# jayleicn/ClipBERT

Measured on NVIDIA H100. Metric: clips/sec fwd+bwd MSRVTT ret (ResNet50+BERT-base), higher is better.
Workload: dtype bf16

## Files before the change

clipbert_b200/_lib.py:

```python
import ctypes
import os

import torch

_HERE = os.path.dirname(os.path.abspath(__file__))
LIB_PATH = os.path.join(_HERE, "lib", "libclipbert_sm90.so")

CB_GEMM_TN, CB_GEMM_WGRAD = 0, 1
ACT_NONE, ACT_RELU, ACT_GELU, ACT_TANH, ACT_GELU_STASH_GRAD = 0, 1, 2, 3, 4
AUX_NONE, AUX_RELU_MASK, AUX_GELU_GRAD, AUX_TANH_GRAD, AUX_MUL = 0, 1, 2, 3, 4
ROWMAP_NONE, ROWMAP_PAD, ROWMAP_UNPAD = 0, 1, 2


class GemmDesc(ctypes.Structure):
    _fields_ = [
        ("mode", ctypes.c_int32),
        ("m", ctypes.c_int32), ("n", ctypes.c_int32), ("k", ctypes.c_int32),
        ("a", ctypes.c_void_p), ("a_rows", ctypes.c_int64), ("a_ld", ctypes.c_int64),
        ("b", ctypes.c_void_p), ("b_rows", ctypes.c_int64), ("b_ld", ctypes.c_int64),
        ("ntaps", ctypes.c_int32), ("tap_w", ctypes.c_int32), ("tap_sign", ctypes.c_int32),
        ("split_k", ctypes.c_int32),
        ("scale", ctypes.c_void_p), ("shift", ctypes.c_void_p),
        ("residual", ctypes.c_void_p), ("res_ld", ctypes.c_int64),
        ("aux", ctypes.c_void_p), ("aux_ld", ctypes.c_int64), ("aux_mode", ctypes.c_int32),
        ("act", ctypes.c_int32),
        ("out", ctypes.c_void_p), ("out_ld", ctypes.c_int64), ("out_fp32", ctypes.c_int32),
        ("out2", ctypes.c_void_p), ("out2_ld", ctypes.c_int64),
        ("rowmap", ctypes.c_int32), ("map_h", ctypes.c_int32), ("map_w", ctypes.c_int32),
        ("dropout_p", ctypes.c_float), ("dropout_seed", ctypes.c_uint64),
        ("block_n", ctypes.c_int32), ("reserved", ctypes.c_int32),
        ("workspace", ctypes.c_void_p), ("workspace_bytes", ctypes.c_int64),
    ]


class NativeLibraryMissing(RuntimeError):
    pass


_lib = None


def lib():
    global _lib
    if _lib is not None:
        return _lib
    if not os.path.exists(LIB_PATH):
        raise NativeLibraryMissing(
            "%s not found: run `python -c 'import __graft_entry__ as g; g.build()'` "
            "(there is no CPU / eager fallback for the ClipBERT hot path)" % LIB_PATH)
    L = ctypes.CDLL(LIB_PATH)
    L.cb_last_error.restype = ctypes.c_char_p
    L.cb_version.restype = ctypes.c_int
    L.cb_sm_arch.restype = ctypes.c_int
    L.cb_launch_count.restype = ctypes.c_int64
    L.cb_gemm.argtypes = [ctypes.POINTER(GemmDesc), ctypes.c_void_p]
    L.cb_gemm.restype = ctypes.c_int
    L.cb_gemm_wgrad_group.argtypes = [ctypes.POINTER(GemmDesc), ctypes.c_int, ctypes.c_void_p]
    L.cb_gemm_wgrad_group.restype = ctypes.c_int
    L.cb_gemm_workspace_bytes.argtypes = [ctypes.POINTER(GemmDesc)]
    L.cb_gemm_workspace_bytes.restype = ctypes.c_int64
    L.cb_gemm_wgrad_group_workspace_bytes.argtypes = [ctypes.POINTER(GemmDesc), ctypes.c_int]
    L.cb_gemm_wgrad_group_workspace_bytes.restype = ctypes.c_int64
    L.cb_set_deterministic.argtypes = [ctypes.c_int]
    L.cb_set_deterministic.restype = ctypes.c_int
    _lib = L
    return L


def check(rc, what="cb call"):
    if rc != 0:
        raise RuntimeError("%s failed (%d): %s" % (what, rc, lib().cb_last_error().decode()))


def stream_ptr():
    return ctypes.c_void_p(torch.cuda.current_stream().cuda_stream)


def ptr(t):
    return None if t is None else t.data_ptr()
```

clipbert_b200/csrc/api.cu:

```cuda
#include <cstdlib>
#include <cstring>
#include <mutex>
#include <unordered_map>
#include <vector>

#include "common.cuh"
#include "host_util.h"

namespace cb {

static thread_local char t_err[512] = "";
std::atomic<int64_t> g_launches{0};
static int pdl_default() {
  const char* e = getenv("CB_PDL");
  return (e && e[0] == '1') ? 1 : ((e && e[0] == '2') ? 2 : 0);
}
std::atomic<int> g_pdl{pdl_default()};
std::atomic<int> g_det{0};
static std::atomic<const uint64_t*> g_drop_offset{nullptr};
const uint64_t* drop_offset_ptr() { return g_drop_offset.load(std::memory_order_relaxed); }

__global__ void drop_offset_advance_kernel(unsigned long long* counter, unsigned long long* snapshot) {
  pdl_wait();
  pdl_trigger();
  const unsigned long long v = *counter + 1ull;
  *counter = v;
  if (snapshot) *snapshot = v;
}

void set_error(const char* fmt, ...) {
  va_list ap;
  va_start(ap, fmt);
  vsnprintf(t_err, sizeof(t_err), fmt, ap);
  va_end(ap);
}

typedef CUresult (*EncodeTiledFn)(CUtensorMap*, CUtensorMapDataType, cuuint32_t, void*,
                                  const cuuint64_t*, const cuuint64_t*, const cuuint32_t*,
                                  const cuuint32_t*, CUtensorMapInterleave, CUtensorMapSwizzle,
                                  CUtensorMapL2promotion, CUtensorMapFloatOOBfill);

static EncodeTiledFn get_encode_fn() {
  static EncodeTiledFn fn = nullptr;
  static std::once_flag once;
  std::call_once(once, [] {
    void* p = nullptr;
    cudaDriverEntryPointQueryResult q;
    cudaError_t e = cudaGetDriverEntryPoint("cuTensorMapEncodeTiled", &p, cudaEnableDefault, &q);
    if (e == cudaSuccess && q == cudaDriverEntryPointSuccess) fn = reinterpret_cast<EncodeTiledFn>(p);
  });
  return fn;
}

struct TmapKey {
  uint64_t base, inner, rows, ld;
  uint32_t box_inner, box_rows;
  bool operator==(const TmapKey& o) const {
    return base == o.base && inner == o.inner && rows == o.rows && ld == o.ld &&
           box_inner == o.box_inner && box_rows == o.box_rows;
  }
};
struct TmapKeyHash {
  size_t operator()(const TmapKey& k) const {
    uint64_t h = k.base * 0x9E3779B97F4A7C15ull;
    h ^= (k.inner + 0x9E3779B97F4A7C15ull + (h << 6) + (h >> 2));
    h ^= (k.rows + 0x9E3779B97F4A7C15ull + (h << 6) + (h >> 2));
    h ^= (k.ld + 0x9E3779B97F4A7C15ull + (h << 6) + (h >> 2));
    h ^= ((static_cast<uint64_t>(k.box_inner) << 32 | k.box_rows) + (h << 6) + (h >> 2));
    return static_cast<size_t>(h);
  }
};

bool get_tmap_2d(CUtensorMap* out, const void* base, uint64_t inner, uint64_t rows, uint64_t ld,
                 uint32_t box_inner, uint32_t box_rows) {
  static std::mutex mu;
  static std::unordered_map<TmapKey, CUtensorMap, TmapKeyHash> cache;
  TmapKey key{reinterpret_cast<uint64_t>(base), inner, rows, ld, box_inner, box_rows};
  std::lock_guard<std::mutex> lock(mu);
  auto it = cache.find(key);
  if (it != cache.end()) {
    *out = it->second;
    return true;
  }

  EncodeTiledFn enc = get_encode_fn();
  if (!enc) {
    set_error("cuTensorMapEncodeTiled driver entry point not available");
    return false;
  }
  if ((reinterpret_cast<uint64_t>(base) & 15) != 0 || ((ld * 2) & 15) != 0) {
    set_error("TMA operand must be 16-byte aligned (base %p, row pitch %llu elements)", base,
              (unsigned long long)ld);
    return false;
  }
  alignas(64) CUtensorMap tm;
  CUtensorMap* m = &tm;
  cuuint64_t dims[2] = {inner, rows};
  cuuint64_t strides[1] = {ld * 2};
  cuuint32_t box[2] = {box_inner, box_rows};
  cuuint32_t estr[2] = {1, 1};
  CUresult r = enc(m, CU_TENSOR_MAP_DATA_TYPE_BFLOAT16, 2, const_cast<void*>(base), dims, strides,
                   box, estr, CU_TENSOR_MAP_INTERLEAVE_NONE, CU_TENSOR_MAP_SWIZZLE_128B,
                   CU_TENSOR_MAP_L2_PROMOTION_L2_256B, CU_TENSOR_MAP_FLOAT_OOB_FILL_NONE);
  if (r != CUDA_SUCCESS) {
    set_error("cuTensorMapEncodeTiled failed (%d) inner=%llu rows=%llu ld=%llu box=%ux%u", (int)r,
              (unsigned long long)inner, (unsigned long long)rows, (unsigned long long)ld, box_inner,
              box_rows);
    return false;
  }
  if (cache.size() > 65536) cache.clear();
  cache.emplace(key, tm);
  *out = tm;
  return true;
}

bool get_tmap_3d_mn(CUtensorMap* out, const void* base, uint64_t cols, uint64_t rows, uint64_t ld, uint32_t box_rows, uint32_t nblk) {
  static std::mutex mu;
  static std::unordered_map<TmapKey, CUtensorMap, TmapKeyHash> cache;
  TmapKey key{reinterpret_cast<uint64_t>(base), cols, rows, ld, 0x80000000u | (nblk << 16) | 64u, box_rows};
  std::lock_guard<std::mutex> lock(mu);
  auto it = cache.find(key);
  if (it != cache.end()) {
    *out = it->second;
    return true;
  }
  EncodeTiledFn enc = get_encode_fn();
  if (!enc) {
    set_error("cuTensorMapEncodeTiled driver entry point not available");
    return false;
  }
  if ((reinterpret_cast<uint64_t>(base) & 15) != 0 || ((ld * 2) & 15) != 0 || (cols & 63) != 0 || nblk == 0 || nblk > 8) {
    set_error("3-D MN-major tensor map: base %p, row pitch %llu, cols %llu (must be a multiple of 64), %u blocks", base,
              (unsigned long long)ld, (unsigned long long)cols, nblk);
    return false;
  }
  alignas(64) CUtensorMap tm;
  CUtensorMap* m = &tm;
  cuuint64_t dims[3] = {64, rows, cols / 64};
  cuuint64_t strides[2] = {ld * 2, 128};
  cuuint32_t box[3] = {64, box_rows, nblk};
  cuuint32_t estr[3] = {1, 1, 1};
  CUresult r = enc(m, CU_TENSOR_MAP_DATA_TYPE_BFLOAT16, 3, const_cast<void*>(base), dims, strides, box, estr,
                   CU_TENSOR_MAP_INTERLEAVE_NONE, CU_TENSOR_MAP_SWIZZLE_128B, CU_TENSOR_MAP_L2_PROMOTION_L2_256B,
                   CU_TENSOR_MAP_FLOAT_OOB_FILL_NONE);
  if (r != CUDA_SUCCESS) {
    set_error("cuTensorMapEncodeTiled (3-D) failed (%d) cols=%llu rows=%llu ld=%llu box=64x%ux%u", (int)r, (unsigned long long)cols,
              (unsigned long long)rows, (unsigned long long)ld, box_rows, nblk);
    return false;
  }
  if (cache.size() > 65536) cache.clear();
  cache.emplace(key, tm);
  *out = tm;
  return true;
}

}

extern "C" {
const char* cb_last_error(void) { return cb::t_err; }
int cb_version(void) { return 100; }
int cb_sm_arch(void) { return 90; }
int64_t cb_launch_count(void) { return cb::g_launches.load(std::memory_order_relaxed); }
int cb_set_pdl(int enable) { return cb::g_pdl.exchange(enable == 2 ? 2 : (enable ? 1 : 0), std::memory_order_relaxed); }
int cb_set_deterministic(int enable) { return cb::g_det.exchange(enable ? 1 : 0, std::memory_order_relaxed); }
int cb_dropout_offset_bind(const uint64_t* device_word) {
  cb::g_drop_offset.store(device_word, std::memory_order_relaxed);
  return CB_OK;
}
int cb_dropout_offset_advance(uint64_t* counter, uint64_t* snapshot, void* stream) {
  CB_REQUIRE(counter != nullptr, "cb_dropout_offset_advance: null counter");
  cb::launch_k(cb::drop_offset_advance_kernel, dim3(1), dim3(1), 0, static_cast<cudaStream_t>(stream),
               reinterpret_cast<unsigned long long*>(counter), reinterpret_cast<unsigned long long*>(snapshot));
  return cb::check_launch("cb_dropout_offset_advance");
}
}
```

clipbert_b200/csrc/common.cuh:

```cuda
#pragma once
#include <cuda.h>
#include <cuda_bf16.h>
#include <cuda_runtime.h>
#include <stdint.h>

#include "drop_cfg.h"

namespace cb {

#ifndef CB_SPIN_LIMIT
#define CB_SPIN_LIMIT (1u << 24)
#endif

__device__ __forceinline__ uint32_t smem_u32(const void* p) {
  return static_cast<uint32_t>(__cvta_generic_to_shared(p));
}

__device__ __forceinline__ void pdl_wait() { asm volatile("griddepcontrol.wait;" ::: "memory"); }
__device__ __forceinline__ void pdl_trigger() { asm volatile("griddepcontrol.launch_dependents;" ::: "memory"); }

__device__ __forceinline__ void mbar_init(uint64_t* bar, uint32_t count) {
  asm volatile("mbarrier.init.shared::cta.b64 [%0], %1;" ::"r"(smem_u32(bar)), "r"(count));
}
__device__ __forceinline__ void fence_mbar_init() {
  asm volatile("fence.mbarrier_init.release.cluster;" ::: "memory");
}
__device__ __forceinline__ void fence_proxy_async_smem() {
  asm volatile("fence.proxy.async.shared::cta;" ::: "memory");
}
__device__ __forceinline__ void mbar_expect_tx(uint64_t* bar, uint32_t bytes) {
  asm volatile("mbarrier.arrive.expect_tx.shared::cta.b64 _, [%0], %1;" ::"r"(smem_u32(bar)),
               "r"(bytes)
               : "memory");
}
__device__ __forceinline__ void mbar_arrive(uint64_t* bar) {
  asm volatile("mbarrier.arrive.shared::cta.b64 _, [%0];" ::"r"(smem_u32(bar)) : "memory");
}
__device__ __forceinline__ void mbar_arrive_if(uint64_t* bar, bool pred) {
  asm volatile("{\n\t.reg .pred p;\n\tsetp.ne.b32 p, %1, 0;\n\t@p mbarrier.arrive.shared::cta.b64 _, [%0];\n\t}" ::"r"(smem_u32(bar)),
               "r"(static_cast<uint32_t>(pred))
               : "memory");
}
__device__ __forceinline__ bool mbar_try_wait(uint64_t* bar, uint32_t parity) {
  uint32_t ok;
  asm volatile(
      "{\n\t.reg .pred p;\n\t"
      "mbarrier.try_wait.parity.shared::cta.b64 p, [%1], %2, %3;\n\t"
      "selp.u32 %0, 1, 0, p;\n\t}"
      : "=r"(ok)
      : "r"(smem_u32(bar)), "r"(parity), "r"(2000u)
      : "memory");
  return ok != 0;
}
__device__ __forceinline__ void mbar_wait(uint64_t* bar, uint32_t parity) {
  uint32_t spins = 0;
  while (!mbar_try_wait(bar, parity)) {
    if (++spins > CB_SPIN_LIMIT) __trap();
  }
}
__device__ __forceinline__ void mbar_wait_unguarded(uint64_t* bar, uint32_t parity) {
  while (!mbar_try_wait(bar, parity)) {
  }
}

__device__ __forceinline__ void tma_prefetch_desc(const CUtensorMap* map) {
  asm volatile("prefetch.tensormap [%0];" ::"l"(map) : "memory");
}
__device__ __forceinline__ void tma_load_2d(void* smem_dst, const CUtensorMap* map, uint64_t* bar,
                                            int c0, int c1) {
  asm volatile(
      "cp.async.bulk.tensor.2d.shared::cluster.global.mbarrier::complete_tx::bytes "
      "[%0], [%1, {%3, %4}], [%2];" ::"r"(smem_u32(smem_dst)),
      "l"(map), "r"(smem_u32(bar)), "r"(c0), "r"(c1)
      : "memory");
}

__device__ __forceinline__ void bulk_load_1d(uint32_t smem_dst, const void* gsrc, uint32_t bytes, uint64_t* bar) {
  asm volatile("cp.async.bulk.shared::cluster.global.mbarrier::complete_tx::bytes [%0], [%1], %2, [%3];" ::"r"(smem_dst), "l"(gsrc),
               "r"(bytes), "r"(smem_u32(bar))
               : "memory");
}

__device__ __forceinline__ void tma_load_2d_s32(uint32_t smem_dst, const CUtensorMap* map, uint64_t* bar, int c0, int c1) {
  asm volatile(
      "cp.async.bulk.tensor.2d.shared::cluster.global.mbarrier::complete_tx::bytes "
      "[%0], [%1, {%3, %4}], [%2];" ::"r"(smem_dst),
      "l"(map), "r"(smem_u32(bar)), "r"(c0), "r"(c1)
      : "memory");
}

__device__ __forceinline__ void tma_load_3d(void* smem_dst, const CUtensorMap* map, uint64_t* bar, int c0, int c1, int c2) {
  asm volatile(
      "cp.async.bulk.tensor.3d.shared::cluster.global.mbarrier::complete_tx::bytes "
      "[%0], [%1, {%3, %4, %5}], [%2];" ::"r"(smem_u32(smem_dst)),
      "l"(map), "r"(smem_u32(bar)), "r"(c0), "r"(c1), "r"(c2)
      : "memory");
}

__device__ __forceinline__ void tma_store_2d(const CUtensorMap* map, const void* smem_src, int c0, int c1) {
  asm volatile("cp.async.bulk.tensor.2d.global.shared::cta.bulk_group [%0, {%2, %3}], [%1];" ::"l"(map),
               "r"(smem_u32(smem_src)), "r"(c0), "r"(c1)
               : "memory");
}
__device__ __forceinline__ void tma_store_2d_s32(const CUtensorMap* map, uint32_t smem_src, int c0, int c1) {
  asm volatile("cp.async.bulk.tensor.2d.global.shared::cta.bulk_group [%0, {%2, %3}], [%1];" ::"l"(map), "r"(smem_src), "r"(c0), "r"(c1)
               : "memory");
}
__device__ __forceinline__ uint4 lds128(uint32_t saddr) {
  uint4 v;
  asm volatile("ld.shared.v4.u32 {%0, %1, %2, %3}, [%4];" : "=r"(v.x), "=r"(v.y), "=r"(v.z), "=r"(v.w) : "r"(saddr));
  return v;
}
__device__ __forceinline__ void sts128(uint32_t saddr, uint4 v) {
  asm volatile("st.shared.v4.u32 [%0], {%1, %2, %3, %4};" ::"r"(saddr), "r"(v.x), "r"(v.y), "r"(v.z), "r"(v.w) : "memory");
}
__device__ __forceinline__ void tma_store_commit() { asm volatile("cp.async.bulk.commit_group;" ::: "memory"); }
template <int N>
__device__ __forceinline__ void tma_store_wait_read() {
  asm volatile("cp.async.bulk.wait_group.read %0;" ::"n"(N) : "memory");
}
template <int N>
__device__ __forceinline__ void tma_store_wait_all() {
  asm volatile("cp.async.bulk.wait_group %0;" ::"n"(N) : "memory");
}
__device__ __forceinline__ void named_bar_sync(uint32_t id, uint32_t nthreads) {
  asm volatile("bar.sync %0, %1;" ::"r"(id), "r"(nthreads) : "memory");
}
__device__ __forceinline__ void named_bar_arrive(uint32_t id, uint32_t nthreads) {
  asm volatile("bar.arrive %0, %1;" ::"r"(id), "r"(nthreads) : "memory");
}
template <uint32_t NREG>
__device__ __forceinline__ void setmaxnreg_dec() {
  asm volatile("setmaxnreg.dec.sync.aligned.u32 %0;" ::"n"(NREG));
}
template <uint32_t NREG>
__device__ __forceinline__ void setmaxnreg_inc() {
  asm volatile("setmaxnreg.inc.sync.aligned.u32 %0;" ::"n"(NREG));
}

__device__ __forceinline__ void wgmma_fence() { asm volatile("wgmma.fence.sync.aligned;" ::: "memory"); }
__device__ __forceinline__ void wgmma_commit() { asm volatile("wgmma.commit_group.sync.aligned;" ::: "memory"); }
template <int N>
__device__ __forceinline__ void wgmma_wait() {
  asm volatile("wgmma.wait_group.sync.aligned %0;" ::"n"(N) : "memory");
}
template <int R>
__device__ __forceinline__ void wgmma_fence_acc(float (&d)[R]) {
#pragma unroll
  for (int i = 0; i < R; ++i) asm volatile("" : "+f"(d[i])::"memory");
}

__device__ __forceinline__ uint64_t gmma_desc(uint32_t smem_addr, uint32_t lbo, uint32_t sbo) {
  uint64_t d = 0;
  d |= static_cast<uint64_t>((smem_addr & 0x3FFFFu) >> 4);
  d |= static_cast<uint64_t>((lbo >> 4) & 0x3FFFu) << 16;
  d |= static_cast<uint64_t>((sbo >> 4) & 0x3FFFu) << 32;
  d |= 1ull << 62;
  return d;
}

template <int TA, int TB>
__device__ __forceinline__ void wgmma_bf16_n64(float (&d)[32], uint64_t adesc, uint64_t bdesc, uint32_t accumulate) {
  asm volatile(
      "{\n\t.reg .pred p;\n\t"
      "setp.ne.b32 p, %34, 0;\n\t"
      "wgmma.mma_async.sync.aligned.m64n64k16.f32.bf16.bf16 "
      "{"
      "%0, %1, %2, %3, %4, %5, %6, %7, %8, %9, %10, %11, %12, %13, %14, %15, "
      "%16, %17, %18, %19, %20, %21, %22, %23, %24, %25, %26, %27, %28, %29, %30, %31"
      "}, %32, %33, p, 1, 1, %35, %36;\n\t}"
      : "+f"(d[0]), "+f"(d[1]), "+f"(d[2]), "+f"(d[3]), "+f"(d[4]), "+f"(d[5]), "+f"(d[6]), "+f"(d[7]),
        "+f"(d[8]), "+f"(d[9]), "+f"(d[10]), "+f"(d[11]), "+f"(d[12]), "+f"(d[13]), "+f"(d[14]), "+f"(d[15]),
        "+f"(d[16]), "+f"(d[17]), "+f"(d[18]), "+f"(d[19]), "+f"(d[20]), "+f"(d[21]), "+f"(d[22]), "+f"(d[23]),
        "+f"(d[24]), "+f"(d[25]), "+f"(d[26]), "+f"(d[27]), "+f"(d[28]), "+f"(d[29]), "+f"(d[30]), "+f"(d[31])
      : "l"(adesc), "l"(bdesc), "r"(accumulate), "n"(TA), "n"(TB));
}
template <int TA, int TB>
__device__ __forceinline__ void wgmma_bf16_n128(float (&d)[64], uint64_t adesc, uint64_t bdesc, uint32_t accumulate) {
  asm volatile(
      "{\n\t.reg .pred p;\n\t"
      "setp.ne.b32 p, %66, 0;\n\t"
      "wgmma.mma_async.sync.aligned.m64n128k16.f32.bf16.bf16 "
      "{"
      "%0, %1, %2, %3, %4, %5, %6, %7, %8, %9, %10, %11, %12, %13, %14, %15, "
      "%16, %17, %18, %19, %20, %21, %22, %23, %24, %25, %26, %27, %28, %29, %30, %31, "
      "%32, %33, %34, %35, %36, %37, %38, %39, %40, %41, %42, %43, %44, %45, %46, %47, "
      "%48, %49, %50, %51, %52, %53, %54, %55, %56, %57, %58, %59, %60, %61, %62, %63"
      "}, %64, %65, p, 1, 1, %67, %68;\n\t}"
      : "+f"(d[0]), "+f"(d[1]), "+f"(d[2]), "+f"(d[3]), "+f"(d[4]), "+f"(d[5]), "+f"(d[6]), "+f"(d[7]),
        "+f"(d[8]), "+f"(d[9]), "+f"(d[10]), "+f"(d[11]), "+f"(d[12]), "+f"(d[13]), "+f"(d[14]), "+f"(d[15]),
        "+f"(d[16]), "+f"(d[17]), "+f"(d[18]), "+f"(d[19]), "+f"(d[20]), "+f"(d[21]), "+f"(d[22]), "+f"(d[23]),
        "+f"(d[24]), "+f"(d[25]), "+f"(d[26]), "+f"(d[27]), "+f"(d[28]), "+f"(d[29]), "+f"(d[30]), "+f"(d[31]),
        "+f"(d[32]), "+f"(d[33]), "+f"(d[34]), "+f"(d[35]), "+f"(d[36]), "+f"(d[37]), "+f"(d[38]), "+f"(d[39]),
        "+f"(d[40]), "+f"(d[41]), "+f"(d[42]), "+f"(d[43]), "+f"(d[44]), "+f"(d[45]), "+f"(d[46]), "+f"(d[47]),
        "+f"(d[48]), "+f"(d[49]), "+f"(d[50]), "+f"(d[51]), "+f"(d[52]), "+f"(d[53]), "+f"(d[54]), "+f"(d[55]),
        "+f"(d[56]), "+f"(d[57]), "+f"(d[58]), "+f"(d[59]), "+f"(d[60]), "+f"(d[61]), "+f"(d[62]), "+f"(d[63])
      : "l"(adesc), "l"(bdesc), "r"(accumulate), "n"(TA), "n"(TB));
}
template <int TA, int TB>
__device__ __forceinline__ void wgmma_bf16_n256(float (&d)[128], uint64_t adesc, uint64_t bdesc, uint32_t accumulate) {
  asm volatile(
      "{\n\t.reg .pred p;\n\t"
      "setp.ne.b32 p, %130, 0;\n\t"
      "wgmma.mma_async.sync.aligned.m64n256k16.f32.bf16.bf16 "
      "{"
      "%0, %1, %2, %3, %4, %5, %6, %7, %8, %9, %10, %11, %12, %13, %14, %15, "
      "%16, %17, %18, %19, %20, %21, %22, %23, %24, %25, %26, %27, %28, %29, %30, %31, "
      "%32, %33, %34, %35, %36, %37, %38, %39, %40, %41, %42, %43, %44, %45, %46, %47, "
      "%48, %49, %50, %51, %52, %53, %54, %55, %56, %57, %58, %59, %60, %61, %62, %63, "
      "%64, %65, %66, %67, %68, %69, %70, %71, %72, %73, %74, %75, %76, %77, %78, %79, "
      "%80, %81, %82, %83, %84, %85, %86, %87, %88, %89, %90, %91, %92, %93, %94, %95, "
      "%96, %97, %98, %99, %100, %101, %102, %103, %104, %105, %106, %107, %108, %109, %110, %111, "
      "%112, %113, %114, %115, %116, %117, %118, %119, %120, %121, %122, %123, %124, %125, %126, %127"
      "}, %128, %129, p, 1, 1, %131, %132;\n\t}"
      : "+f"(d[0]), "+f"(d[1]), "+f"(d[2]), "+f"(d[3]), "+f"(d[4]), "+f"(d[5]), "+f"(d[6]), "+f"(d[7]),
        "+f"(d[8]), "+f"(d[9]), "+f"(d[10]), "+f"(d[11]), "+f"(d[12]), "+f"(d[13]), "+f"(d[14]), "+f"(d[15]),
        "+f"(d[16]), "+f"(d[17]), "+f"(d[18]), "+f"(d[19]), "+f"(d[20]), "+f"(d[21]), "+f"(d[22]), "+f"(d[23]),
        "+f"(d[24]), "+f"(d[25]), "+f"(d[26]), "+f"(d[27]), "+f"(d[28]), "+f"(d[29]), "+f"(d[30]), "+f"(d[31]),
        "+f"(d[32]), "+f"(d[33]), "+f"(d[34]), "+f"(d[35]), "+f"(d[36]), "+f"(d[37]), "+f"(d[38]), "+f"(d[39]),
        "+f"(d[40]), "+f"(d[41]), "+f"(d[42]), "+f"(d[43]), "+f"(d[44]), "+f"(d[45]), "+f"(d[46]), "+f"(d[47]),
        "+f"(d[48]), "+f"(d[49]), "+f"(d[50]), "+f"(d[51]), "+f"(d[52]), "+f"(d[53]), "+f"(d[54]), "+f"(d[55]),
        "+f"(d[56]), "+f"(d[57]), "+f"(d[58]), "+f"(d[59]), "+f"(d[60]), "+f"(d[61]), "+f"(d[62]), "+f"(d[63]),
        "+f"(d[64]), "+f"(d[65]), "+f"(d[66]), "+f"(d[67]), "+f"(d[68]), "+f"(d[69]), "+f"(d[70]), "+f"(d[71]),
        "+f"(d[72]), "+f"(d[73]), "+f"(d[74]), "+f"(d[75]), "+f"(d[76]), "+f"(d[77]), "+f"(d[78]), "+f"(d[79]),
        "+f"(d[80]), "+f"(d[81]), "+f"(d[82]), "+f"(d[83]), "+f"(d[84]), "+f"(d[85]), "+f"(d[86]), "+f"(d[87]),
        "+f"(d[88]), "+f"(d[89]), "+f"(d[90]), "+f"(d[91]), "+f"(d[92]), "+f"(d[93]), "+f"(d[94]), "+f"(d[95]),
        "+f"(d[96]), "+f"(d[97]), "+f"(d[98]), "+f"(d[99]), "+f"(d[100]), "+f"(d[101]), "+f"(d[102]), "+f"(d[103]),
        "+f"(d[104]), "+f"(d[105]), "+f"(d[106]), "+f"(d[107]), "+f"(d[108]), "+f"(d[109]), "+f"(d[110]), "+f"(d[111]),
        "+f"(d[112]), "+f"(d[113]), "+f"(d[114]), "+f"(d[115]), "+f"(d[116]), "+f"(d[117]), "+f"(d[118]), "+f"(d[119]),
        "+f"(d[120]), "+f"(d[121]), "+f"(d[122]), "+f"(d[123]), "+f"(d[124]), "+f"(d[125]), "+f"(d[126]), "+f"(d[127])
      : "l"(adesc), "l"(bdesc), "r"(accumulate), "n"(TA), "n"(TB));
}

template <int N, int TA, int TB>
__device__ __forceinline__ void wgmma_bf16(float (&d)[N / 2], uint64_t adesc, uint64_t bdesc, uint32_t accumulate) {
  if constexpr (N == 64) wgmma_bf16_n64<TA, TB>(d, adesc, bdesc, accumulate);
  else if constexpr (N == 128) wgmma_bf16_n128<TA, TB>(d, adesc, bdesc, accumulate);
  else wgmma_bf16_n256<TA, TB>(d, adesc, bdesc, accumulate);
}

__device__ __forceinline__ float warp_sum(float v) {
#pragma unroll
  for (int o = 16; o > 0; o >>= 1) v += __shfl_xor_sync(0xffffffffu, v, o);
  return v;
}
__device__ __forceinline__ float warp_max(float v) {
#pragma unroll
  for (int o = 16; o > 0; o >>= 1) v = fmaxf(v, __shfl_xor_sync(0xffffffffu, v, o));
  return v;
}

__device__ __forceinline__ void red_add_f32x4(float* addr, float4 v) {
  asm volatile("red.global.add.v4.f32 [%0], {%1, %2, %3, %4};" ::"l"(addr), "f"(v.x), "f"(v.y), "f"(v.z),
               "f"(v.w)
               : "memory");
}

__device__ __forceinline__ void red_add_f32x2(float* addr, float x, float y) {
  asm volatile("red.global.add.v2.f32 [%0], {%1, %2};" ::"l"(addr), "f"(x), "f"(y) : "memory");
}

__device__ __forceinline__ float fast_rcp(float x) {
  float r;
  asm("rcp.approx.ftz.f32 %0, %1;" : "=f"(r) : "f"(x));
  return r;
}

__device__ __forceinline__ float fast_erf(float x) {
  const float ax = fabsf(x);
  const float t = fast_rcp(fmaf(0.3275911f, ax, 1.0f));
  float p = fmaf(1.061405429f, t, -1.453152027f);
  p = fmaf(p, t, 1.421413741f);
  p = fmaf(p, t, -0.284496736f);
  p = fmaf(p, t, 0.254829592f);
  const float r = 1.0f - p * t * __expf(-ax * ax);
  return copysignf(r, x);
}
__device__ __forceinline__ float gelu_erf(float x) {
  return 0.5f * x * (1.0f + fast_erf(x * 0.70710678118654752f));
}
__device__ __forceinline__ void gelu_erf_and_grad(float x, float& y, float& g) {
  const float az = fabsf(x) * 0.70710678118654752f;
  const float t = fast_rcp(fmaf(0.3275911f, az, 1.0f));
  float p = fmaf(1.061405429f, t, -1.453152027f);
  p = fmaf(p, t, 1.421413741f);
  p = fmaf(p, t, -0.284496736f);
  p = fmaf(p, t, 0.254829592f);
  const float e = __expf(-az * az);
  const float cdf = 0.5f * (1.0f + copysignf(1.0f - p * t * e, x));
  y = x * cdf;
  g = fmaf(x * 0.3989422804014327f, e, cdf);
}
__device__ __forceinline__ float gelu_erf_grad(float x) {
  const float cdf = 0.5f * (1.0f + fast_erf(x * 0.70710678118654752f));
  const float pdf = 0.3989422804014327f * __expf(-0.5f * x * x);
  return cdf + x * pdf;
}

__device__ __forceinline__ uint64_t drop_seed(uint64_t seed, const uint64_t* offset) {
  return offset ? seed + __ldg(reinterpret_cast<const unsigned long long*>(offset)) * 0xD1342543DE82EF95ull : seed;
}
__device__ __forceinline__ DropCfg drop_resolve(DropCfg dc) {
  if (dc.thresh) dc.seed = drop_seed(dc.seed, dc.offset);
  dc.offset = nullptr;
  return dc;
}
__device__ __forceinline__ uint64_t drop_hash(uint64_t seed, uint64_t group) {
  uint64_t z = group * 0x9E3779B97F4A7C15ull + seed;
  z = (z ^ (z >> 30)) * 0xBF58476D1CE4E5B9ull;
  z = (z ^ (z >> 27)) * 0x94D049BB133111EBull;
  return z ^ (z >> 31);
}
__device__ __forceinline__ float drop_lane(uint64_t h, int lane, uint32_t thresh, float inv_keep) {
  return (static_cast<uint32_t>(h >> (16 * lane)) & 0xFFFFu) >= thresh ? inv_keep : 0.0f;
}
__device__ __forceinline__ float dropout_mult(uint64_t seed, uint64_t idx, uint32_t thresh, float inv_keep) {
  return drop_lane(drop_hash(seed, idx >> 2), static_cast<int>(idx & 3), thresh, inv_keep);
}
__device__ __forceinline__ void dropout_mult4(uint64_t seed, uint64_t idx, uint32_t thresh, float inv_keep, float (&m)[4]) {
  const uint64_t h = drop_hash(seed, idx >> 2);
#pragma unroll
  for (int j = 0; j < 4; ++j) m[j] = drop_lane(h, j, thresh, inv_keep);
}
__device__ __forceinline__ void dropout_mult2(uint64_t seed, uint64_t idx, uint32_t thresh, float inv_keep, float& m0, float& m1) {
  const uint64_t h0 = drop_hash(seed, idx >> 2);
  const int l0 = static_cast<int>(idx & 3);
  m0 = drop_lane(h0, l0, thresh, inv_keep);
  m1 = l0 == 3 ? drop_lane(drop_hash(seed, (idx >> 2) + 1), 0, thresh, inv_keep) : drop_lane(h0, l0 + 1, thresh, inv_keep);
}

__device__ __forceinline__ uint32_t pack_bf16x2(float lo, float hi) {
  __nv_bfloat162 h = __floats2bfloat162_rn(lo, hi);
  return *reinterpret_cast<uint32_t*>(&h);
}
__device__ __forceinline__ float2 unpack_bf16x2(uint32_t u) {
  __nv_bfloat162 h = *reinterpret_cast<__nv_bfloat162*>(&u);
  return __bfloat1622float2(h);
}

}
```

clipbert_b200/csrc/gemm.cu:

```cuda
#include <algorithm>

#include "common.cuh"
#include "host_util.h"

namespace cb {

constexpr int BM = 128;
constexpr int BK = 64;
constexpr int CONSUMER_WARPS = 8;
constexpr int GEMM_THREADS = (CONSUMER_WARPS + 1) * 32;
constexpr int PP_THREADS = 3 * 128;
constexpr int PP_PRODUCER_REGS = 40;
constexpr int PP_CONSUMER_REGS = 232;
constexpr int PP_BAR_TURN = 1;
constexpr int MAX_STAGES = 8;
constexpr int SMEM_LIMIT = 232448;
constexpr int STG_PITCH = 36;
constexpr int STG_WARP_FLOATS = 16 * STG_PITCH;
constexpr int EPI_BYTES = CONSUMER_WARPS * STG_WARP_FLOATS * 4;
constexpr int IN_BOX_BYTES = BM * 64 * 2;

struct GemmEpi {
  const float* scale;
  const float* shift;
  const __nv_bfloat16* residual;
  const __nv_bfloat16* aux;
  int aux_mode;
  int act;
  void* out;
  int64_t out_ld;
  int out_fp32;
  __nv_bfloat16* out2;
  int64_t out2_ld;
  int rowmap, H, W;
  uint32_t drop_thresh;
  float drop_inv_keep;
  uint64_t seed;
  const uint64_t* seed_off;
  int mn3d;
  long long* dbg;
};

__device__ __forceinline__ void dbg_stamp(const GemmEpi& epi, int slot) {
  if (epi.dbg) {
    epi.dbg[blockIdx.x * 32 + slot] = clock64();
    if (slot == 0 || slot == 11) {
      unsigned long long ns;
      asm volatile("mov.u64 %0, %%globaltimer;" : "=l"(ns));
      epi.dbg[blockIdx.x * 32 + (slot == 0 ? 12 : 13)] = static_cast<long long>(ns);
    }
  }
}

template <int BN>
struct GemmCfg {
  static constexpr int A_BYTES = BM * BK * 2;
  static constexpr int B_BYTES = BN * BK * 2;
  static constexpr int STAGE_BYTES = A_BYTES + B_BYTES;
  static constexpr int BAR_BYTES = 256;
};

enum { EK_GENERIC = 0, EK_SHIFT_ACT = 1, EK_RELU_MASK = 2, EK_DROP_RES = 3, EK_GELU_STASH = 4, EK_AUX_MUL = 5 };

__device__ __forceinline__ float relu_nan(float v) { return !(v <= 0.0f) ? v : 0.0f; }
__device__ __forceinline__ bool bf16_relu_pos(uint32_t x, bool lo) {
  const uint32_t b = lo ? (x & 0xffffu) : (x >> 16);
  return b - 0x0080u <= 0x7f80u - 0x0080u;
}

template <int NC>
__device__ __forceinline__ void add_shift(float (&f)[NC], const float (&shv)[NC]) {
#pragma unroll
  for (int j = 0; j < NC; ++j) f[j] += shv[j];
}
template <int NC>
__device__ __forceinline__ void add_residual(float (&f)[NC], const uint32_t (&res16)[NC / 2]) {
#pragma unroll
  for (int j = 0; j < NC / 2; ++j) {
    const float2 r2 = unpack_bf16x2(res16[j]);
    f[2 * j] += r2.x;
    f[2 * j + 1] += r2.y;
  }
}
template <int NC>
__device__ __forceinline__ void epilogue_shift_act(float (&f)[NC], const float (&shv)[NC], bool has_shift, const uint32_t (&res16)[NC / 2], bool has_res,
                                                   bool relu) {
  if (has_shift) add_shift<NC>(f, shv);
  if (has_res) add_residual<NC>(f, res16);
  if (relu) {
#pragma unroll
    for (int j = 0; j < NC; ++j) f[j] = relu_nan(f[j]);
  }
}
template <int NC>
__device__ __forceinline__ void epilogue_relu_mask(float (&f)[NC], const uint32_t (&res16)[NC / 2], bool has_res, const uint32_t (&aux16)[NC / 2]) {
  if (has_res) add_residual<NC>(f, res16);
#pragma unroll
  for (int j = 0; j < NC / 2; ++j) {
    f[2 * j] = bf16_relu_pos(aux16[j], true) ? f[2 * j] : 0.0f;
    f[2 * j + 1] = bf16_relu_pos(aux16[j], false) ? f[2 * j + 1] : 0.0f;
  }
}
template <int NC>
__device__ __forceinline__ void epilogue_drop_res(float (&f)[NC], const float (&shv)[NC], bool has_shift, const uint32_t (&res16)[NC / 2], bool has_res,
                                                  uint64_t dseed, uint64_t didx, uint32_t thresh, float inv_keep) {
  if (has_shift) add_shift<NC>(f, shv);
#pragma unroll
  for (int j = 0; j < NC; j += 4) {
    float m[4];
    dropout_mult4(dseed, didx + j, thresh, inv_keep, m);
    f[j] *= m[0]; f[j + 1] *= m[1]; f[j + 2] *= m[2]; f[j + 3] *= m[3];
  }
  if (has_res) add_residual<NC>(f, res16);
}
template <int NC>
__device__ __forceinline__ void epilogue_gelu_stash(float (&f)[NC], const float (&shv)[NC], bool has_shift, uint32_t (&o2_16)[NC / 2]) {
  if (has_shift) add_shift<NC>(f, shv);
#pragma unroll
  for (int j = 0; j < NC / 2; ++j) {
    float y0, g0, y1, g1;
    gelu_erf_and_grad(f[2 * j], y0, g0);
    gelu_erf_and_grad(f[2 * j + 1], y1, g1);
    f[2 * j] = y0;
    f[2 * j + 1] = y1;
    o2_16[j] = pack_bf16x2(g0, g1);
  }
}
template <int NC>
__device__ __forceinline__ void epilogue_aux_mul(float (&f)[NC], const uint32_t (&res16)[NC / 2], bool has_res, const uint32_t (&aux16)[NC / 2]) {
  if (has_res) add_residual<NC>(f, res16);
#pragma unroll
  for (int j = 0; j < NC / 2; ++j) {
    const float2 a2 = unpack_bf16x2(aux16[j]);
    f[2 * j] *= a2.x;
    f[2 * j + 1] *= a2.y;
  }
}
template <int NC, bool GUARD>
__device__ __forceinline__ void epilogue_math(float (&f)[NC], const GemmEpi& epi, const float (&shv)[NC], bool has_shift, uint64_t dseed, int nb, int N,
                                              int64_t orow, const uint32_t (&res16)[NC / 2], bool has_res, const uint32_t (&aux16)[NC / 2], bool has_aux,
                                              uint32_t (&o2_16)[NC / 2], bool has_out2) {
  if (GUARD && nb >= N) return;
  if (epi.scale) {
#pragma unroll
    for (int j = 0; j < NC; j += 4) {
      if (!GUARD || nb + j + 4 <= N) {
        const float4 s4 = __ldg(reinterpret_cast<const float4*>(epi.scale + nb + j));
        f[j] *= s4.x; f[j + 1] *= s4.y; f[j + 2] *= s4.z; f[j + 3] *= s4.w;
      }
    }
  }
  if (has_shift) add_shift<NC>(f, shv);
  if (epi.drop_thresh) {
    const uint64_t base = static_cast<uint64_t>(orow) * static_cast<uint64_t>(N) + nb;
#pragma unroll
    for (int j = 0; j < NC; j += 4) {
      float m[4];
      dropout_mult4(dseed, base + j, epi.drop_thresh, epi.drop_inv_keep, m);
      f[j] *= m[0]; f[j + 1] *= m[1]; f[j + 2] *= m[2]; f[j + 3] *= m[3];
    }
  }
  if (has_res) add_residual<NC>(f, res16);
  if (epi.act == CB_ACT_GELU_STASH_GRAD) {
#pragma unroll
    for (int j = 0; j < NC / 2; ++j) {
      float y0, g0, y1, g1;
      gelu_erf_and_grad(f[2 * j], y0, g0);
      gelu_erf_and_grad(f[2 * j + 1], y1, g1);
      f[2 * j] = y0;
      f[2 * j + 1] = y1;
      if (has_out2) o2_16[j] = pack_bf16x2(g0, g1);
    }
  } else if (has_out2) {
#pragma unroll
    for (int j = 0; j < NC / 2; ++j) o2_16[j] = pack_bf16x2(f[2 * j], f[2 * j + 1]);
  }
  switch (epi.act) {
    case CB_ACT_RELU:
#pragma unroll
      for (int j = 0; j < NC; ++j) f[j] = relu_nan(f[j]);
      break;
    case CB_ACT_GELU:
#pragma unroll
      for (int j = 0; j < NC; ++j) f[j] = gelu_erf(f[j]);
      break;
    case CB_ACT_TANH:
#pragma unroll
      for (int j = 0; j < NC; ++j) f[j] = tanhf(f[j]);
      break;
    default: break;
  }
  if (has_aux) {
    switch (epi.aux_mode) {
      case CB_AUX_RELU_MASK:
#pragma unroll
        for (int j = 0; j < NC / 2; ++j) {
          f[2 * j] = bf16_relu_pos(aux16[j], true) ? f[2 * j] : 0.0f;
          f[2 * j + 1] = bf16_relu_pos(aux16[j], false) ? f[2 * j + 1] : 0.0f;
        }
        break;
      case CB_AUX_GELU_GRAD:
#pragma unroll
        for (int j = 0; j < NC / 2; ++j) {
          const float2 a2 = unpack_bf16x2(aux16[j]);
          f[2 * j] *= gelu_erf_grad(a2.x);
          f[2 * j + 1] *= gelu_erf_grad(a2.y);
        }
        break;
      case CB_AUX_TANH_GRAD:
#pragma unroll
        for (int j = 0; j < NC / 2; ++j) {
          const float2 a2 = unpack_bf16x2(aux16[j]);
          f[2 * j] *= (1.0f - a2.x * a2.x);
          f[2 * j + 1] *= (1.0f - a2.y * a2.y);
        }
        break;
      case CB_AUX_MUL:
#pragma unroll
        for (int j = 0; j < NC / 2; ++j) {
          const float2 a2 = unpack_bf16x2(aux16[j]);
          f[2 * j] *= a2.x;
          f[2 * j + 1] *= a2.y;
        }
        break;
      default: break;
    }
  }
}

struct TileInfo {
  int m0, n0;
};

template <int BN>
__device__ __forceinline__ TileInfo decode_tile(int tile, int tiles_m, int tiles_n) {
  TileInfo t;
  t.m0 = (tile / tiles_n) % tiles_m * BM;
  t.n0 = tile % tiles_n * BN;
  return t;
}

template <int BN, int TA, int TB>
__device__ __forceinline__ void mma_tile(float (&acc)[BN / 2], uint32_t smem0, int stage_bytes, int KCH, int STAGES, int n_iters, int wg,
                                         int lane, int& s, uint32_t& ph, uint64_t* full_bar, uint64_t* empty_bar) {
  using Cfg = GemmCfg<BN>;
  int prev = -1;
  for (int i = 0; i < n_iters; i += KCH) {
    const int nch = min(KCH, n_iters - i);
    mbar_wait(&full_bar[s], ph);
    __syncwarp();
    wgmma_fence();
    wgmma_fence_acc(acc);
    for (int ch = 0; ch < nch; ++ch) {
      const uint32_t a_addr = smem0 + s * stage_bytes + ch * Cfg::STAGE_BYTES + wg * (64 * 128);
      const uint32_t b_addr = smem0 + s * stage_bytes + ch * Cfg::STAGE_BYTES + Cfg::A_BYTES;
#pragma unroll
      for (int k = 0; k < BK / 16; ++k) {
        const uint64_t ad = TA ? gmma_desc(a_addr + k * 2048, BK * 128, 1024) : gmma_desc(a_addr + k * 32, 16, 1024);
        const uint64_t bd = TB ? gmma_desc(b_addr + k * 2048, BK * 128, 1024) : gmma_desc(b_addr + k * 32, 16, 1024);
        wgmma_bf16<BN, TA, TB>(acc, ad, bd, (i > 0 || ch > 0 || k > 0) ? 1u : 0u);
      }
    }
    wgmma_commit();
    wgmma_wait<1>();
    wgmma_fence_acc(acc);
    if (prev >= 0) {
      __syncwarp();
      if (lane == 0) mbar_arrive(&empty_bar[prev]);
    }
    prev = s;
    if (++s == STAGES) { s = 0; ph ^= 1; }
  }
  wgmma_wait<0>();
  wgmma_fence_acc(acc);
  if (prev >= 0) {
    __syncwarp();
    if (lane == 0) mbar_arrive(&empty_bar[prev]);
  }
}

template <int BN, int TB>
__device__ __forceinline__ void mma_tile_pp(float (&acc)[2][BN / 2], uint32_t smem0, int stage_bytes, int KCH, int STAGES, int n_iters,
                                            int lane, int& s, uint32_t& ph, uint64_t* full_bar, uint64_t* empty_bar, int pass_bar,
                                            bool in_stage) {
  using Cfg = GemmCfg<BN>;
  int prev = -1;
  for (int i = 0; i < n_iters; i += KCH) {
    const int nch = min(KCH, n_iters - i);
    mbar_wait_unguarded(&full_bar[s], ph);
    __syncwarp();
    wgmma_fence();
    wgmma_fence_acc(acc[0]);
    wgmma_fence_acc(acc[1]);
    for (int ch = 0; ch < nch; ++ch) {
      const uint32_t a_addr = smem0 + s * stage_bytes + ch * Cfg::STAGE_BYTES;
      const uint32_t b_addr = a_addr + Cfg::A_BYTES;
#pragma unroll
      for (int k = 0; k < BK / 16; ++k) {
        const uint64_t bd = TB ? gmma_desc(b_addr + k * 2048, BK * 128, 1024) : gmma_desc(b_addr + k * 32, 16, 1024);
        const uint32_t accum = (i > 0 || ch > 0 || k > 0) ? 1u : 0u;
#pragma unroll
        for (int h = 0; h < 2; ++h) wgmma_bf16<BN, 0, TB>(acc[h], gmma_desc(a_addr + h * (64 * 128) + k * 32, 16, 1024), bd, accum);
      }
    }
    wgmma_commit();
    wgmma_wait<1>();
    wgmma_fence_acc(acc[0]);
    wgmma_fence_acc(acc[1]);
    if (prev >= 0) {
      __syncwarp();
      mbar_arrive_if(&empty_bar[prev], lane == 0);
    }
    prev = s;
    if (++s == STAGES) { s = 0; ph ^= 1; }
    if (pass_bar && i + KCH >= n_iters) {
      if (in_stage) mbar_wait_unguarded(&full_bar[s], ph);
      named_bar_arrive(pass_bar, 2 * 128);
    }
  }
  wgmma_wait<0>();
  wgmma_fence_acc(acc[0]);
  wgmma_fence_acc(acc[1]);
  if (prev >= 0) {
    __syncwarp();
    mbar_arrive_if(&empty_bar[prev], lane == 0);
  }
}

template <int BN, bool STORE = false>
__device__ __forceinline__ void wgrad_epilogue(const float (&acc)[BN / 2], float* obase, int64_t out_ld, const float* scale, int M, int N, int r0,
                                               int n0, int lane) {
  const int r1 = r0 + 8;
  const float rs0 = (r0 < M && scale) ? scale[r0] : 1.0f;
  const float rs1 = (r1 < M && scale) ? scale[r1] : 1.0f;
#pragma unroll
  for (int j = 0; j < BN / 8; ++j) {
    const int n = n0 + j * 8 + 2 * (lane & 3);
    if (n < N) {
      if constexpr (STORE) {
        if (r0 < M) *reinterpret_cast<float2*>(obase + static_cast<int64_t>(r0) * out_ld + n) = make_float2(acc[4 * j] * rs0, acc[4 * j + 1] * rs0);
        if (r1 < M) *reinterpret_cast<float2*>(obase + static_cast<int64_t>(r1) * out_ld + n) = make_float2(acc[4 * j + 2] * rs1, acc[4 * j + 3] * rs1);
      } else {
        if (r0 < M) red_add_f32x2(obase + static_cast<int64_t>(r0) * out_ld + n, acc[4 * j] * rs0, acc[4 * j + 1] * rs0);
        if (r1 < M) red_add_f32x2(obase + static_cast<int64_t>(r1) * out_ld + n, acc[4 * j + 2] * rs1, acc[4 * j + 3] * rs1);
      }
    }
  }
}

__device__ __forceinline__ uint32_t swz128(uint32_t box, int r, int q) { return box + r * 128 + ((q ^ (r & 7)) << 4); }

template <int BN, int MODE>
__global__ void __launch_bounds__(PP_THREADS, 1)
    gemm_pingpong_kernel(const __grid_constant__ CUtensorMap tmA, const __grid_constant__ CUtensorMap tmB, const __grid_constant__ CUtensorMap tmR,
                         const __grid_constant__ CUtensorMap tmX, int M, int N, int K, int ntaps, int tap_w, int tap_sign, int tiles_m,
                         int tiles_n, int total_tiles, int STAGES, int KCH, int N_IN, GemmEpi epi) {
  static_assert(MODE != 1 && BN <= 128, "TN / NN tiles of 128 x 64 or 128 x 128");
  using Cfg = GemmCfg<BN>;
  extern __shared__ uint8_t smem_raw[];
  uint8_t* smem = reinterpret_cast<uint8_t*>((reinterpret_cast<uintptr_t>(smem_raw) + 1023) & ~static_cast<uintptr_t>(1023));
  const int stage_bytes = KCH * Cfg::STAGE_BYTES;
  const bool has_res = epi.residual != nullptr, has_aux = epi.aux != nullptr;
  constexpr int IN_TILE_BYTES = (BN / 64) * IN_BOX_BYTES;
  const int in_bytes = (has_res + has_aux) * IN_TILE_BYTES;
  uint8_t* in_base = smem + STAGES * stage_bytes;
  uint8_t* stg_base = in_base + N_IN * in_bytes;
  uint64_t* full_bar = reinterpret_cast<uint64_t*>(stg_base + EPI_BYTES);
  uint64_t* empty_bar = full_bar + MAX_STAGES;
  uint64_t* in_full = empty_bar + MAX_STAGES;
  uint64_t* in_empty = in_full + 2;

  const int warp = __shfl_sync(0xffffffffu, static_cast<int>(threadIdx.x >> 5), 0);
  const int lane = threadIdx.x & 31;
  const int unit = blockIdx.x;
  const int n_units = gridDim.x;
  if (threadIdx.x == 0) dbg_stamp(epi, 0);
  pdl_trigger();
  if (threadIdx.x == 0) {
    tma_prefetch_desc(&tmA);
    tma_prefetch_desc(&tmB);
    if (has_res) tma_prefetch_desc(&tmR);
    if (has_aux) tma_prefetch_desc(&tmX);
    for (int s = 0; s < STAGES; ++s) {
      mbar_init(&full_bar[s], 1);
      mbar_init(&empty_bar[s], 4);
    }
    for (int b = 0; b < 2; ++b) {
      mbar_init(&in_full[b], 1);
      mbar_init(&in_empty[b], 4);
    }
    fence_mbar_init();
  }
  __syncthreads();
  const int kc_per_tap = (K + BK - 1) / BK;
  const int n_iters = ntaps * kc_per_tap;
  const bool in_stage = in_bytes && !N_IN;
  const int tile_stages = (n_iters + KCH - 1) / KCH + (in_stage ? 1 : 0);
  pdl_wait();
  if (threadIdx.x == 0) dbg_stamp(epi, 1);

  if (warp < 4) {
    setmaxnreg_dec<PP_PRODUCER_REGS>();
    if (warp == 0 && lane == 0) {
      constexpr int B_BOXES = (MODE == 0) ? 1 : BN / 64;
      int s = 0;
      uint32_t ph = 0;
      auto load_inputs = [&](int tile) {
        const TileInfo t = decode_tile<BN>(tile, tiles_m, tiles_n);
        uint64_t* bar;
        uint8_t* dst;
        if (N_IN) {
          const int local = (tile - unit) / n_units;
          const int b = N_IN == 2 ? (local & 1) : 0;
          const int uses = N_IN == 2 ? (local >> 1) : local;
          mbar_wait(&in_empty[b], (static_cast<uint32_t>(uses) & 1u) ^ 1u);
          bar = &in_full[local & 1];
          dst = in_base + b * in_bytes;
        } else {
          mbar_wait(&empty_bar[s], ph ^ 1);
          bar = &full_bar[s];
          dst = smem + s * stage_bytes;
          if (++s == STAGES) { s = 0; ph ^= 1; }
        }
        mbar_expect_tx(bar, in_bytes);
        if (has_res) {
#pragma unroll
          for (int j = 0; j < BN / 64; ++j) tma_load_2d(dst + j * IN_BOX_BYTES, &tmR, bar, t.n0 + j * 64, t.m0);
          dst += IN_TILE_BYTES;
        }
        if (has_aux) {
#pragma unroll
          for (int j = 0; j < BN / 64; ++j) tma_load_2d(dst + j * IN_BOX_BYTES, &tmX, bar, t.n0 + j * 64, t.m0);
        }
      };
      int pend = -1;
      for (int tile = unit; tile < total_tiles; tile += n_units) {
        const TileInfo t = decode_tile<BN>(tile, tiles_m, tiles_n);
        const bool inputs_first = tile < unit + N_IN * n_units;
        if (in_bytes && N_IN && inputs_first) load_inputs(tile);
        for (int i = 0; i < n_iters; i += KCH) {
          const int nch = min(KCH, n_iters - i);
          mbar_wait(&empty_bar[s], ph ^ 1);
          mbar_expect_tx(&full_bar[s], nch * Cfg::STAGE_BYTES);
          int tp = 0, kc = i;
          if (ntaps > 1) { tp = i / kc_per_tap; kc = i - tp * kc_per_tap; }
          for (int ch = 0; ch < nch; ++ch) {
            uint8_t* sa = smem + s * stage_bytes + ch * Cfg::STAGE_BYTES;
            uint8_t* sb = sa + Cfg::A_BYTES;
            int shift = 0;
            if (ntaps == 9) shift = tap_sign * ((tp / 3 - 1) * tap_w + (tp % 3 - 1));
            else if (ntaps > 1) shift = tap_sign * tp * tap_w;
            tma_load_2d(sa, &tmA, &full_bar[s], kc * BK, t.m0 + shift);
            if (MODE == 0) {
              tma_load_2d(sb, &tmB, &full_bar[s], tp * K + kc * BK, t.n0);
            } else if (epi.mn3d) {
              tma_load_3d(sb, &tmB, &full_bar[s], 0, kc * BK, (tp * N + t.n0) >> 6);
            } else {
#pragma unroll
              for (int j = 0; j < B_BOXES; ++j) tma_load_2d(sb + j * (BK * 128), &tmB, &full_bar[s], tp * N + t.n0 + j * 64, kc * BK);
            }
            if (++kc == kc_per_tap) { kc = 0; ++tp; }
          }
          if (++s == STAGES) { s = 0; ph ^= 1; }
          if (i == 0 && tile == unit) dbg_stamp(epi, 2);
        }
        if (in_stage) load_inputs(tile);
        if (pend >= 0) load_inputs(pend);
        pend = (in_bytes && N_IN && !inputs_first) ? tile : -1;
      }
      if (pend >= 0) load_inputs(pend);
      dbg_stamp(epi, 3);
    }
    return;
  }

  setmaxnreg_inc<PP_CONSUMER_REGS>();
  const int wg = (warp >> 2) - 1;
  const int wq = warp & 3;
  const uint32_t smem0 = smem_u32(smem);
  const uint64_t dseed = epi.drop_thresh ? drop_seed(epi.seed, epi.seed_off) : 0ull;
  float acc[2][BN / 2];
  int s = 0;
  uint32_t ph = 0;
  auto ring_skip = [&](int n) {
    s += n;
    while (s >= STAGES) { s -= STAGES; ph ^= 1; }
  };
  if (wg == 1) ring_skip(tile_stages);

  const int er = lane & 15, eh = lane >> 4;
  float* stg = reinterpret_cast<float*>(stg_base) + (warp - 4) * STG_WARP_FLOATS;
  const bool has_out2 = epi.out2 != nullptr;
  const bool has_shift = epi.shift != nullptr;
  const bool full = (N & 15) == 0 && epi.scale == nullptr;
  const bool drop = epi.drop_thresh != 0;
  int kind = EK_GENERIC;
  if (full) {
    if (!drop && !has_out2 && !has_aux && (epi.act == CB_ACT_NONE || epi.act == CB_ACT_RELU)) kind = EK_SHIFT_ACT;
    else if (!drop && !has_out2 && !has_shift && has_aux && epi.aux_mode == CB_AUX_RELU_MASK && epi.act == CB_ACT_NONE) kind = EK_RELU_MASK;
    else if (drop && !has_out2 && !has_aux && epi.act == CB_ACT_NONE) kind = EK_DROP_RES;
    else if (!drop && has_out2 && !has_aux && !has_res && epi.act == CB_ACT_GELU_STASH_GRAD) kind = EK_GELU_STASH;
    else if (!drop && !has_out2 && !has_shift && has_aux && epi.aux_mode == CB_AUX_MUL && epi.act == CB_ACT_NONE) kind = EK_AUX_MUL;
  }
  const bool kind_relu = epi.act == CB_ACT_RELU;
  const bool guard = (N & 15) != 0;

  for (int local = wg, tile = unit + wg * n_units; tile < total_tiles; local += 2, tile += 2 * n_units) {
    const TileInfo t = decode_tile<BN>(tile, tiles_m, tiles_n);
    if (local > 0) named_bar_sync(PP_BAR_TURN + wg, 2 * 128);
    const int pass = tile + n_units < total_tiles ? PP_BAR_TURN + (wg ^ 1) : 0;
    mma_tile_pp<BN, MODE != 0>(acc, smem0, stage_bytes, KCH, STAGES, n_iters, lane, s, ph, full_bar, empty_bar, pass, in_stage);

    const uint32_t in_buf = N_IN ? smem_u32(in_base) + (N_IN == 2 ? wg : 0) * in_bytes : smem0 + s * stage_bytes;
    if (in_bytes) {
      if (N_IN) mbar_wait_unguarded(&in_full[wg], static_cast<uint32_t>(local >> 1) & 1u);
      else mbar_wait_unguarded(&full_bar[s], ph);
    }
    int orow_half[2];
#pragma unroll
    for (int h = 0; h < 2; ++h) {
      const int m = t.m0 + h * 64 + wq * 16 + er;
      bool row_ok = m < M;
      int64_t orow = m;
      if (epi.rowmap == CB_ROWMAP_PAD) {
        const int hw = epi.H * epi.W;
        const int img = m / hw;
        const int r = m - img * hw;
        const int y = r / epi.W, x = r - y * epi.W;
        orow = (static_cast<int64_t>(img) * (epi.H + 2) + y + 1) * (epi.W + 2) + x + 1;
      } else if (epi.rowmap == CB_ROWMAP_UNPAD) {
        const int wp = epi.W + 2, hp = epi.H + 2;
        const int img = m / (hp * wp);
        const int r = m - img * (hp * wp);
        const int y = r / wp, x = r - y * wp;
        row_ok = row_ok && y >= 1 && y <= epi.H && x >= 1 && x <= epi.W;
        orow = (static_cast<int64_t>(img) * epi.H + (y - 1)) * epi.W + (x - 1);
      }
      orow_half[h] = row_ok ? static_cast<int>(orow) : -1;
    }
#pragma unroll
    for (int sc = 0; sc < BN / 32; ++sc) {
#pragma unroll 1
      for (int h = 0; h < 2; ++h) {
        const int wrow = h * 64 + wq * 16;
        __syncwarp();
#pragma unroll
        for (int jj = 0; jj < 4; ++jj) {
          const int j = sc * 4 + jj;
          float* p = stg + (lane >> 2) * STG_PITCH + jj * 8 + 2 * (lane & 3);
          const bool h1 = h != 0;
          *reinterpret_cast<float2*>(p) = make_float2(h1 ? acc[1][4 * j] : acc[0][4 * j], h1 ? acc[1][4 * j + 1] : acc[0][4 * j + 1]);
          *reinterpret_cast<float2*>(p + 8 * STG_PITCH) =
              make_float2(h1 ? acc[1][4 * j + 2] : acc[0][4 * j + 2], h1 ? acc[1][4 * j + 3] : acc[0][4 * j + 3]);
        }
        __syncwarp();
        const int nb = t.n0 + sc * 32 + eh * 16;
        const int64_t orow = h ? orow_half[1] : orow_half[0];
        if (orow < 0 || nb >= N) continue;
        constexpr int NC = 16;
        float f[NC];
        const uint32_t srow = smem_u32(stg + er * STG_PITCH + eh * 16);
#pragma unroll
        for (int j = 0; j < NC / 4; ++j) {
          const uint4 u = lds128(srow + j * 16);
          f[4 * j] = __uint_as_float(u.x); f[4 * j + 1] = __uint_as_float(u.y);
          f[4 * j + 2] = __uint_as_float(u.z); f[4 * j + 3] = __uint_as_float(u.w);
        }
        uint32_t res16[NC / 2], aux16[NC / 2];
        const int tc = sc * 32 + eh * 16;
        const int q = (tc & 63) >> 3;
        if (has_res) {
#pragma unroll
          for (int j = 0; j < 2; ++j) {
            const uint4 u = lds128(swz128(in_buf + (tc >> 6) * IN_BOX_BYTES, wrow + er, q + j));
            res16[4 * j] = u.x; res16[4 * j + 1] = u.y; res16[4 * j + 2] = u.z; res16[4 * j + 3] = u.w;
          }
        }
        if (has_aux) {
#pragma unroll
          for (int j = 0; j < 2; ++j) {
            const uint4 u = lds128(swz128(in_buf + (has_res ? IN_TILE_BYTES : 0) + (tc >> 6) * IN_BOX_BYTES, wrow + er, q + j));
            aux16[4 * j] = u.x; aux16[4 * j + 1] = u.y; aux16[4 * j + 2] = u.z; aux16[4 * j + 3] = u.w;
          }
        }
        float shv[NC];
        if (has_shift) {
#pragma unroll
          for (int j = 0; j < NC; j += 4) {
            float4 s4 = make_float4(0.f, 0.f, 0.f, 0.f);
            if (nb + j + 4 <= N) s4 = __ldg(reinterpret_cast<const float4*>(epi.shift + nb + j));
            shv[j] = s4.x; shv[j + 1] = s4.y; shv[j + 2] = s4.z; shv[j + 3] = s4.w;
          }
        }
        uint32_t o2_16[NC / 2];
        switch (kind) {
          case EK_SHIFT_ACT: epilogue_shift_act<NC>(f, shv, has_shift, res16, has_res, kind_relu); break;
          case EK_RELU_MASK: epilogue_relu_mask<NC>(f, res16, has_res, aux16); break;
          case EK_DROP_RES:
            epilogue_drop_res<NC>(f, shv, has_shift, res16, has_res, dseed, static_cast<uint64_t>(orow) * static_cast<uint64_t>(N) + nb,
                                  epi.drop_thresh, epi.drop_inv_keep);
            break;
          case EK_GELU_STASH: epilogue_gelu_stash<NC>(f, shv, has_shift, o2_16); break;
          case EK_AUX_MUL: epilogue_aux_mul<NC>(f, res16, has_res, aux16); break;
          default:
            if (guard) epilogue_math<NC, true>(f, epi, shv, has_shift, dseed, nb, N, orow, res16, has_res, aux16, has_aux, o2_16, has_out2);
            else epilogue_math<NC, false>(f, epi, shv, has_shift, dseed, nb, N, orow, res16, has_res, aux16, has_aux, o2_16, has_out2);
        }
        if (epi.out_fp32) {
          float* o = reinterpret_cast<float*>(epi.out) + orow * epi.out_ld + nb;
#pragma unroll
          for (int j = 0; j < NC; j += 4)
            if (nb + j + 4 <= N) *reinterpret_cast<float4*>(o + j) = make_float4(f[j], f[j + 1], f[j + 2], f[j + 3]);
        } else {
          __nv_bfloat16* o = reinterpret_cast<__nv_bfloat16*>(epi.out) + orow * epi.out_ld + nb;
#pragma unroll
          for (int j = 0; j < 2; ++j)
            if (nb + 8 * j + 8 <= N)
              *reinterpret_cast<uint4*>(o + 8 * j) = make_uint4(pack_bf16x2(f[8 * j], f[8 * j + 1]), pack_bf16x2(f[8 * j + 2], f[8 * j + 3]),
                                                                pack_bf16x2(f[8 * j + 4], f[8 * j + 5]), pack_bf16x2(f[8 * j + 6], f[8 * j + 7]));
        }
        if (has_out2) {
          __nv_bfloat16* o = epi.out2 + orow * epi.out2_ld + nb;
#pragma unroll
          for (int j = 0; j < 2; ++j)
            if (nb + 8 * j + 8 <= N) *reinterpret_cast<uint4*>(o + 8 * j) = make_uint4(o2_16[4 * j], o2_16[4 * j + 1], o2_16[4 * j + 2], o2_16[4 * j + 3]);
        }
      }
    }
    if (in_bytes) {
      __syncwarp();
      if (lane == 0) mbar_arrive(N_IN ? &in_empty[N_IN == 2 ? wg : 0] : &empty_bar[s]);
      if (!N_IN && ++s == STAGES) { s = 0; ph ^= 1; }
    }
    ring_skip(tile_stages);
  }
  if (threadIdx.x == 4 * 32) dbg_stamp(epi, 11);
}

static int g_sm_limit = 0;
static int sm_count_device() {
  static int n = 0;
  if (n == 0) {
    int dev = 0;
    cudaGetDevice(&dev);
    cudaDeviceGetAttribute(&n, cudaDevAttrMultiProcessorCount, dev);
    if (n <= 0) n = 132;
  }
  return n;
}
static int sm_count() {
  const int n = sm_count_device();
  return (g_sm_limit > 0 && g_sm_limit < n) ? g_sm_limit : n;
}
static int plan_sm_count() { return g_det.load(std::memory_order_relaxed) ? sm_count_device() : sm_count(); }

static long long* g_gemm_timeline = nullptr;
static int g_mn3d = 1;


struct SmemPlan {
  int epi_bytes, kch, stages, chunk_bytes, n_in;
};
static SmemPlan plan_ring(int bn, bool staging, int kiters, int force_kch, int in_bytes, int n_in) {
  SmemPlan p;
  const int limit = SMEM_LIMIT;
  p.chunk_bytes = BM * BK * 2 + bn * BK * 2;
  p.epi_bytes = staging ? EPI_BYTES : 0;
  p.n_in = n_in;
  const int chunks_fit = (limit - 1024 - GemmCfg<64>::BAR_BYTES - p.epi_bytes - n_in * in_bytes) / p.chunk_bytes;
  const int min_stages = kiters > chunks_fit ? 3 : 2;
  p.kch = 1;
  if (force_kch > 0) p.kch = force_kch;
  else if (kiters >= 4 && chunks_fit >= 4 * min_stages) p.kch = 4;
  else if (kiters >= 2 && chunks_fit >= 2 * min_stages) p.kch = 2;
  if (p.kch > kiters) p.kch = kiters;
  if (p.kch > 1 && chunks_fit / p.kch < 2) p.kch = 1;
  p.stages = chunks_fit / p.kch;
  if (p.stages > MAX_STAGES) p.stages = MAX_STAGES;
  const int stage_iters = ceil_div(kiters, p.kch);
  const int cap = staging ? 2 * stage_iters + 1 : (stage_iters + 1 > 2 ? stage_iters + 1 : 2);
  if (p.stages > cap) p.stages = cap;
  return p;
}
static SmemPlan plan_smem(int bn, bool staging, int kiters, int force_kch = 0, int in_bytes = 0) {
  const SmemPlan none = plan_ring(bn, staging, kiters, force_kch, 0, 0);
  if (in_bytes == 0) return none;
  const SmemPlan two = plan_ring(bn, staging, kiters, force_kch, in_bytes, 2);
  if (two.stages >= 2 && two.stages * two.kch >= kiters) return two;
  if (kiters > 4 && none.stages >= 2 && none.kch * none.chunk_bytes >= in_bytes) return none;
  return plan_ring(bn, staging, kiters, force_kch, in_bytes, 1);
}
static int epi_in_bytes(const cb_gemm_desc& d, int bn) {
  return d.mode == CB_GEMM_WGRAD ? 0 : ((d.residual != nullptr) + (d.aux != nullptr)) * (bn / 64) * IN_BOX_BYTES;
}

static int real_splits(int kc, int want) {
  const int sp = want < 1 ? 1 : (want > kc ? kc : want);
  return ceil_div(kc, ceil_div(kc, sp));
}

struct SplitReduceJob {
  float* out;
  const float* ws;
  int64_t out_ld;
  int M, W, S;
};
struct SplitReduce {
  int njobs;
  SplitReduceJob j[8];
};
__global__ void __launch_bounds__(256) wgrad_split_reduce_kernel(const __grid_constant__ SplitReduce r) {
  pdl_wait();
  pdl_trigger();
  const SplitReduceJob& J = r.j[blockIdx.y];
  const int w4 = J.W / 4;
  const int64_t total = static_cast<int64_t>(J.M) * w4, plane = static_cast<int64_t>(J.M) * J.W;
  for (int64_t i = static_cast<int64_t>(blockIdx.x) * 256 + threadIdx.x; i < total; i += static_cast<int64_t>(gridDim.x) * 256) {
    const int64_t m = i / w4;
    const int c = static_cast<int>(i - m * w4) * 4;
    float4* o = reinterpret_cast<float4*>(J.out + m * J.out_ld + c);
    float4 v = *o;
    const float* p = J.ws + m * J.W + c;
    for (int s = 0; s < J.S; ++s) {
      const float4 a = *reinterpret_cast<const float4*>(p + s * plane);
      v.x += a.x; v.y += a.y; v.z += a.z; v.w += a.w;
    }
    *o = v;
  }
}
static int launch_split_reduce(const SplitReduce& r, cudaStream_t stream, const char* what) {
  int64_t most = 0;
  for (int i = 0; i < r.njobs; ++i) most = std::max(most, static_cast<int64_t>(r.j[i].M) * (r.j[i].W / 4));
  const int gx = static_cast<int>(std::min<int64_t>(1024, (most + 255) / 256));
  launch_k(wgrad_split_reduce_kernel, dim3(gx, r.njobs), 256, 0, stream, r);
  return check_launch(what);
}

template <int BN, int MODE>
static int launch_gemm(const cb_gemm_desc& d, const GemmEpi& epi_in, cudaStream_t stream) {
  GemmEpi epi = epi_in;
  using Cfg = GemmCfg<BN>;
  static bool attr_set = false;
  auto kern = gemm_pingpong_kernel<BN, MODE>;
  if (!attr_set) {
    cudaError_t e = cudaFuncSetAttribute(kern, cudaFuncAttributeMaxDynamicSharedMemorySize, SMEM_LIMIT);
    if (e != cudaSuccess) {
      set_error("cudaFuncSetAttribute(smem=%d): %s", SMEM_LIMIT, cudaGetErrorString(e));
      return CB_ERR_CUDA;
    }
    attr_set = true;
  }
  alignas(64) CUtensorMap ta, tb, tr, tx;
  bool mn3d = false;
  const int tiles_m = ceil_div(d.m, BM), tiles_n = ceil_div(d.n, BN);
  const int total = tiles_m * tiles_n;
  const int kiters = ceil_div(d.k, BK) * d.ntaps;
  bool ok = get_tmap_2d(&ta, d.a, d.k, d.a_rows, d.a_ld, BK, BM);
  if (MODE == 0) {
    ok = ok && get_tmap_2d(&tb, d.b, static_cast<uint64_t>(d.k) * d.ntaps, d.b_rows, d.b_ld, BK, BN);
  } else {
    mn3d = g_mn3d && d.n % 64 == 0 &&
           get_tmap_3d_mn(&tb, d.b, static_cast<uint64_t>(d.n) * d.ntaps, d.b_rows, d.b_ld, BK, BN / 64);
    if (!mn3d) ok = ok && get_tmap_2d(&tb, d.b, static_cast<uint64_t>(d.n) * d.ntaps, d.b_rows, d.b_ld, 64, BK);
  }
  tr = ta;
  tx = ta;
  if (d.residual) ok = ok && get_tmap_2d(&tr, d.residual, d.n, d.m, d.res_ld, 64, BM);
  if (d.aux) ok = ok && get_tmap_2d(&tx, d.aux, d.n, d.m, d.aux_ld, 64, BM);
  if (!ok) return CB_ERR_CUDA;
  epi.mn3d = mn3d ? 1 : 0;
  const int units = sm_count();
  const int grid = total < units ? total : units;
  const int in_bytes = epi_in_bytes(d, BN);
  const SmemPlan sp = plan_smem(BN, true, kiters, (d.reserved >> 8) & 15, in_bytes);
  const int kch = sp.kch, stages = sp.stages;
  if (stages < 2) {
    set_error("cb_gemm: not enough shared memory for a 2-stage pipeline (BN=%d, epilogue %d B + inputs %d B)", BN, sp.epi_bytes,
              in_bytes);
    return CB_ERR_INVALID;
  }
  const int smem_bytes = stages * kch * Cfg::STAGE_BYTES + sp.n_in * in_bytes + sp.epi_bytes + Cfg::BAR_BYTES + 1024;
  launch_gemm_k(kern, grid, PP_THREADS, smem_bytes, stream, ta, tb, tr, tx, d.m, d.n, d.k, d.ntaps, d.tap_w, d.tap_sign, tiles_m,
                tiles_n, total, stages, kch, sp.n_in, epi);
  return check_launch("cb_gemm");
}

struct LaunchCfg {
  int bn, splits;
};

static LaunchCfg choose_config(const cb_gemm_desc& d, int units) {
  const int kc = ceil_div(d.k, BK);
  const bool wgrad = d.mode == CB_GEMM_WGRAD;
  const int block_n = (!wgrad && d.block_n == 256) ? 128 : d.block_n;
  static const int cand[3] = {64, 128, 256};
  LaunchCfg best = {64, 1};
  double best_cost = 1e30;
  for (int c = 0; c < 3; ++c) {
    const int bn = cand[c];
    if (block_n && bn != block_n) continue;
    if (!wgrad && bn == 256) continue;
    if (bn > 64 && d.n <= bn / 2) continue;
    const int64_t base = static_cast<int64_t>(ceil_div(d.m, BM)) * ceil_div(d.n, bn) * (wgrad ? d.ntaps : 1);
    const int max_split = wgrad ? (d.split_k > 0 ? d.split_k : (kc < 32 ? kc : 32)) : 1;
    for (int sp = (wgrad && d.split_k > 0) ? d.split_k : 1; sp <= max_split; ++sp) {
      const int ips = ceil_div(wgrad ? kc : kc * d.ntaps, sp);
      const int real_sp = wgrad ? ceil_div(kc, ips) : 1;
      const int64_t tiles = base * real_sp;
      const double rounds = static_cast<double>((tiles + units - 1) / units);
      const SmemPlan pl = plan_smem(bn, !wgrad, ips, (d.reserved >> 8) & 15, epi_in_bytes(d, bn));
      if (pl.stages < 2) continue;
      const double shallow = (pl.stages * pl.kch < 3 && ips > 2) ? 3.0 : 1.0;
      const double stage_cost = 450.0 + pl.kch * pl.chunk_bytes / 60.0;
      const double main_loop = ceil_div(ips, pl.kch) * stage_cost * shallow;
      double cost;
      if (wgrad) {
        cost = rounds * (main_loop + bn * 24.0) + 2500.0;
      } else {
        const double epi = bn * 30.0;
        const double per_tile = main_loop > 0.5 * (main_loop + epi) ? main_loop : 0.5 * (main_loop + epi);
        cost = rounds * per_tile + 0.5 * epi + 2500.0;
      }
      if (cost < best_cost) {
        best_cost = cost;
        best = {bn, real_sp};
      }
    }
  }
  return best;
}

constexpr int WG_MAX_PROBLEMS = 8;
struct WgradProblem {
  CUtensorMap tmA, tmB;
  float* out;
  const float* scale;
  int64_t out_ld;
  int M, N, K;
  int ntaps, tap_w, tap_sign;
  int iters_per_split, tiles_m, tiles_n;
  int tile_begin;
  int mn3d;
};
struct WgradGroup {
  int nprob, total_tiles;
  WgradProblem p[WG_MAX_PROBLEMS];
};
struct WgradWorkspace {
  float* p[WG_MAX_PROBLEMS];
};
struct WgTile {
  int pi, m0, n0, tap, it_begin, n_iters;
};
__device__ __forceinline__ WgTile wg_decode(const WgradGroup& g, int tile) {
  WgTile t;
  int pi = 0;
  while (pi + 1 < g.nprob && tile >= g.p[pi + 1].tile_begin) ++pi;
  const WgradProblem& P = g.p[pi];
  int r = tile - P.tile_begin;
  const int nt = r % P.tiles_n;
  r /= P.tiles_n;
  const int mt = r % P.tiles_m;
  r /= P.tiles_m;
  t.pi = pi;
  t.m0 = mt * BM;
  t.tap = r % P.ntaps;
  const int split = r / P.ntaps;
  const int kc = (P.K + BK - 1) / BK;
  t.it_begin = split * P.iters_per_split;
  t.n_iters = min(kc, t.it_begin + P.iters_per_split) - t.it_begin;
  t.n0 = nt;
  return t;
}

template <int BN, bool DET = false>
__global__ void __launch_bounds__(GEMM_THREADS, 1)
    wgrad_group_kernel(const __grid_constant__ WgradGroup g, int STAGES, int KCH, const __grid_constant__ WgradWorkspace ws) {
  using Cfg = GemmCfg<BN>;
  extern __shared__ uint8_t smem_raw[];
  uint8_t* smem = reinterpret_cast<uint8_t*>((reinterpret_cast<uintptr_t>(smem_raw) + 1023) & ~static_cast<uintptr_t>(1023));
  const int stage_bytes = KCH * Cfg::STAGE_BYTES;
  uint64_t* full_bar = reinterpret_cast<uint64_t*>(smem + STAGES * stage_bytes);
  uint64_t* empty_bar = full_bar + MAX_STAGES;
  const int warp = __shfl_sync(0xffffffffu, static_cast<int>(threadIdx.x >> 5), 0);
  const int lane = threadIdx.x & 31;
  const int unit = blockIdx.x, n_units = gridDim.x;
  pdl_trigger();
  if (threadIdx.x == 0) {
    for (int i = 0; i < g.nprob; ++i) {
      tma_prefetch_desc(&g.p[i].tmA);
      tma_prefetch_desc(&g.p[i].tmB);
    }
    for (int s = 0; s < STAGES; ++s) {
      mbar_init(&full_bar[s], 1);
      mbar_init(&empty_bar[s], CONSUMER_WARPS);
    }
    fence_mbar_init();
  }
  __syncthreads();
  pdl_wait();

  if (warp >= CONSUMER_WARPS) {
    if (warp == CONSUMER_WARPS && lane == 0) {
      int s = 0;
      uint32_t ph = 0;
      for (int tile = unit; tile < g.total_tiles; tile += n_units) {
        const WgTile t = wg_decode(g, tile);
        const WgradProblem& P = g.p[t.pi];
        const int n0 = t.n0 * BN;
        int shift = 0;
        if (P.ntaps == 9) shift = P.tap_sign * ((t.tap / 3 - 1) * P.tap_w + (t.tap % 3 - 1));
        for (int i = 0; i < t.n_iters; i += KCH) {
          const int nch = min(KCH, t.n_iters - i);
          mbar_wait(&empty_bar[s], ph ^ 1);
          mbar_expect_tx(&full_bar[s], nch * Cfg::STAGE_BYTES);
          int kit = t.it_begin + i;
          for (int ch = 0; ch < nch; ++ch, ++kit) {
            uint8_t* sa = smem + s * stage_bytes + ch * Cfg::STAGE_BYTES;
            uint8_t* sb = sa + Cfg::A_BYTES;
            const int p = kit * BK;
            if (P.mn3d) {
              tma_load_3d(sa, &P.tmA, &full_bar[s], 0, p, t.m0 >> 6);
              tma_load_3d(sb, &P.tmB, &full_bar[s], 0, p + shift, n0 >> 6);
            } else {
#pragma unroll
              for (int j = 0; j < BM / 64; ++j) tma_load_2d(sa + j * (BK * 128), &P.tmA, &full_bar[s], t.m0 + j * 64, p);
#pragma unroll
              for (int j = 0; j < BN / 64; ++j) tma_load_2d(sb + j * (BK * 128), &P.tmB, &full_bar[s], n0 + j * 64, p + shift);
            }
          }
          if (++s == STAGES) { s = 0; ph ^= 1; }
        }
      }
    }
    return;
  }

  const int wg = warp >> 2;
  const int wrow = wg * 64 + (warp & 3) * 16;
  const uint32_t smem0 = smem_u32(smem);
  float acc[BN / 2];
  int s = 0;
  uint32_t ph = 0;
  for (int tile = unit; tile < g.total_tiles; tile += n_units) {
    const WgTile t = wg_decode(g, tile);
    const WgradProblem& P = g.p[t.pi];
    mma_tile<BN, 1, 1>(acc, smem0, stage_bytes, KCH, STAGES, t.n_iters, wg, lane, s, ph, full_bar, empty_bar);
    if (DET && ws.p[t.pi] != nullptr)
      wgrad_epilogue<BN, true>(acc, ws.p[t.pi] + static_cast<int64_t>(t.it_begin / P.iters_per_split) * P.M * P.ntaps * P.N +
                                        static_cast<int64_t>(t.tap) * P.N,
                               static_cast<int64_t>(P.ntaps) * P.N, P.scale, P.M, P.N, t.m0 + wrow + (lane >> 2), t.n0 * BN, lane);
    else
      wgrad_epilogue<BN>(acc, P.out + static_cast<int64_t>(t.tap) * P.N, P.out_ld, P.scale, P.M, P.N, t.m0 + wrow + (lane >> 2), t.n0 * BN, lane);
  }
}

template <int BN, bool DET>
static int launch_wgrad_group(const cb_gemm_desc* descs, int n, int splits, float* ws, cudaStream_t stream, const char* what) {
  using Cfg = GemmCfg<BN>;
  static bool attr_set = false;
  auto kern = wgrad_group_kernel<BN, DET>;
  if (!attr_set) {
    cudaError_t e = cudaFuncSetAttribute(kern, cudaFuncAttributeMaxDynamicSharedMemorySize, SMEM_LIMIT);
    if (e != cudaSuccess) {
      set_error("cudaFuncSetAttribute(smem=%d): %s", SMEM_LIMIT, cudaGetErrorString(e));
      return CB_ERR_CUDA;
    }
    attr_set = true;
  }
  alignas(64) WgradGroup g;
  g.nprob = n;
  SplitReduce red;
  red.njobs = 0;
  WgradWorkspace wsp;
  int total = 0, max_iters = 0;
  for (int i = 0; i < n; ++i) {
    const cb_gemm_desc& d = descs[i];
    WgradProblem& P = g.p[i];
    const bool mn3d = g_mn3d && d.m % 64 == 0 && d.n % 64 == 0 && get_tmap_3d_mn(&P.tmA, d.a, d.m, d.a_rows, d.a_ld, BK, BM / 64) &&
                      get_tmap_3d_mn(&P.tmB, d.b, d.n, d.b_rows, d.b_ld, BK, BN / 64);
    if (!mn3d && !(get_tmap_2d(&P.tmA, d.a, d.m, d.a_rows, d.a_ld, 64, BK) && get_tmap_2d(&P.tmB, d.b, d.n, d.b_rows, d.b_ld, 64, BK)))
      return CB_ERR_CUDA;
    P.mn3d = mn3d ? 1 : 0;
    P.out = static_cast<float*>(d.out);
    P.scale = d.scale;
    P.out_ld = d.out_ld;
    P.M = d.m; P.N = d.n; P.K = d.k;
    P.ntaps = d.ntaps; P.tap_w = d.tap_w; P.tap_sign = d.tap_sign;
    const int kc = ceil_div(d.k, BK);
    const int sp = real_splits(kc, splits);
    P.iters_per_split = ceil_div(kc, sp);
    wsp.p[i] = nullptr;
    if (DET && sp > 1) {
      wsp.p[i] = ws;
      red.j[red.njobs++] = {static_cast<float*>(d.out), ws, d.out_ld, d.m, d.ntaps * d.n, sp};
      ws += static_cast<int64_t>(sp) * d.m * d.ntaps * d.n;
    }
    P.tiles_m = ceil_div(d.m, BM);
    P.tiles_n = ceil_div(d.n, BN);
    P.tile_begin = total;
    total += P.tiles_m * P.tiles_n * d.ntaps * sp;
    if (P.iters_per_split > max_iters) max_iters = P.iters_per_split;
  }
  g.total_tiles = total;
  const SmemPlan sp = plan_smem(BN, false, max_iters, (descs[0].reserved >> 8) & 15);
  if (sp.stages < 2) {
    set_error("%s: not enough shared memory for a 2-stage pipeline (BN=%d)", what, BN);
    return CB_ERR_INVALID;
  }
  const int smem_bytes = sp.stages * sp.kch * Cfg::STAGE_BYTES + Cfg::BAR_BYTES + 1024;
  const int units = sm_count();
  launch_gemm_k(kern, total < units ? total : units, GEMM_THREADS, smem_bytes, stream, g, sp.stages, sp.kch, wsp);
  const int rc = check_launch(what);
  if (rc != CB_OK || red.njobs == 0) return rc;
  return launch_split_reduce(red, stream, what);
}

struct GroupPlan {
  bool groupable;
  int bn, split;
};
static GroupPlan group_plan(const cb_gemm_desc* descs, int n, int sms) {
  GroupPlan gp = {n >= 2 && n <= WG_MAX_PROBLEMS, 64, 1};
  for (int i = 0; i < n; ++i)
    if (descs[i].k * 2 < descs[0].k || descs[0].k * 2 < descs[i].k) gp.groupable = false;
  if (!gp.groupable) return gp;
  int min_n = descs[0].n;
  for (int i = 1; i < n; ++i) min_n = descs[i].n < min_n ? descs[i].n : min_n;
  gp.bn = descs[0].block_n ? descs[0].block_n : (min_n >= 192 ? 256 : (min_n >= 96 ? 128 : 64));
  int64_t base = 0;
  int kc_min = 1 << 30, kc_max = 0;
  for (int i = 0; i < n; ++i) {
    base += static_cast<int64_t>(ceil_div(descs[i].m, BM)) * ceil_div(descs[i].n, gp.bn) * descs[i].ntaps;
    const int kc = ceil_div(descs[i].k, BK);
    kc_min = kc < kc_min ? kc : kc_min;
    kc_max = kc > kc_max ? kc : kc_max;
  }
  double best_cost = 1e30;
  for (int sp = 1; sp <= 8 && sp <= kc_min; ++sp) {
    const double waves = static_cast<double>((base * sp + sms - 1) / sms);
    const double cost = waves * (ceil_div(kc_max, sp) + 8.0);
    if (cost < best_cost) { best_cost = cost; gp.split = sp; }
  }
  if (descs[0].split_k > 0) gp.split = descs[0].split_k;
  return gp;
}

static int64_t wgrad_ws_bytes(const cb_gemm_desc& d, int splits) {
  return splits > 1 ? static_cast<int64_t>(splits) * d.m * d.ntaps * d.n * 4 : 0;
}
static int64_t group_ws_bytes(const cb_gemm_desc* descs, int n) {
  const GroupPlan gp = group_plan(descs, n, sm_count_device());
  int64_t bytes = 0;
  for (int i = 0; i < n; ++i) {
    const int64_t b = gp.groupable ? wgrad_ws_bytes(descs[i], real_splits(ceil_div(descs[i].k, BK), gp.split))
                                   : wgrad_ws_bytes(descs[i], choose_config(descs[i], sm_count_device()).splits);
    bytes = gp.groupable ? bytes + b : std::max(bytes, b);
  }
  return bytes;
}

static int check_wgrad_desc(const cb_gemm_desc& d, const char* who) {
  CB_REQUIRE(d.mode == CB_GEMM_WGRAD && d.out_fp32 == 1, "%s: not an fp32 WGRAD descriptor", who);
  CB_REQUIRE(d.a && d.b && d.out && d.m > 0 && d.n > 0 && d.k > 0, "%s: null operand / empty shape", who);
  CB_REQUIRE(d.m % 8 == 0 && d.n % 8 == 0, "%s: m, n must be multiples of 8 (got %d, %d)", who, d.m, d.n);
  CB_REQUIRE(d.out_ld % 4 == 0, "%s: out_ld must be a multiple of 4", who);
  CB_REQUIRE((reinterpret_cast<uintptr_t>(d.out) & 15) == 0, "%s: out must be 16-byte aligned", who);
  CB_REQUIRE((reinterpret_cast<uintptr_t>(d.a) & 15) == 0 && (reinterpret_cast<uintptr_t>(d.b) & 15) == 0,
             "%s: a and b must be 16-byte aligned (TMA)", who);
  CB_REQUIRE(d.ntaps == 1 || d.ntaps == 9, "%s: ntaps must be 1 or 9 (got %d)", who, d.ntaps);
  return CB_OK;
}

static int launch_wgrad(const cb_gemm_desc* descs, int n, int bn, int splits, cudaStream_t stream, const char* what) {
  int64_t need = 0;
  if (g_det.load(std::memory_order_relaxed))
    for (int i = 0; i < n; ++i) need += wgrad_ws_bytes(descs[i], real_splits(ceil_div(descs[i].k, BK), splits));
  const cb_gemm_desc& d0 = descs[0];
  CB_REQUIRE(need == 0 || (d0.workspace != nullptr && d0.workspace_bytes >= need && (reinterpret_cast<uintptr_t>(d0.workspace) & 15) == 0),
             "%s: deterministic mode needs a 16-byte aligned workspace of %lld bytes in descs[0] (%s_workspace_bytes), got %lld", what,
             static_cast<long long>(need), what, static_cast<long long>(d0.workspace ? d0.workspace_bytes : 0));
  float* ws = static_cast<float*>(d0.workspace);
  switch (bn) {
    case 64: return need ? launch_wgrad_group<64, true>(descs, n, splits, ws, stream, what)
                         : launch_wgrad_group<64, false>(descs, n, splits, ws, stream, what);
    case 128: return need ? launch_wgrad_group<128, true>(descs, n, splits, ws, stream, what)
                          : launch_wgrad_group<128, false>(descs, n, splits, ws, stream, what);
    case 256: return need ? launch_wgrad_group<256, true>(descs, n, splits, ws, stream, what)
                          : launch_wgrad_group<256, false>(descs, n, splits, ws, stream, what);
    default: set_error("%s: block_n must be 0, 64, 128 or 256 (got %d)", what, bn); return CB_ERR_INVALID;
  }
}

}

extern "C" void cb_debug_gemm_timeline(void* device_buf) { cb::g_gemm_timeline = static_cast<long long*>(device_buf); }
extern "C" void cb_debug_gemm_mn3d(int on) { cb::g_mn3d = on ? 1 : 0; }
extern "C" void cb_debug_gemm_occ2(int, double) {}
extern "C" void cb_debug_gemm_sm_limit(int n) { cb::g_sm_limit = n > 0 ? n : 0; }

extern "C" int cb_gemm(const cb_gemm_desc* dp, void* stream_v) {
  using namespace cb;
  CB_REQUIRE(dp != nullptr, "cb_gemm: null descriptor");
  const cb_gemm_desc& d = *dp;
  cudaStream_t stream = static_cast<cudaStream_t>(stream_v);
  CB_REQUIRE(d.a && d.b && d.out, "cb_gemm: null operand pointer");
  CB_REQUIRE(d.m > 0 && d.n > 0 && d.k > 0, "cb_gemm: empty problem m=%d n=%d k=%d", d.m, d.n, d.k);
  CB_REQUIRE(d.ntaps == 1 || d.ntaps == 9 || (d.ntaps == 4 && d.mode == CB_GEMM_TN),
             "cb_gemm: ntaps must be 1, 9 (3x3 conv) or 4 (row taps, TN only) (got %d)", d.ntaps);
  CB_REQUIRE(d.mode == CB_GEMM_TN || d.mode == CB_GEMM_WGRAD || d.mode == CB_GEMM_NN, "cb_gemm: bad mode %d", d.mode);
  CB_REQUIRE(d.dropout_p >= 0.0f && d.dropout_p <= 1.0f, "cb_gemm: dropout_p %g outside [0, 1]", d.dropout_p);

  GemmEpi epi;
  epi.scale = d.scale;
  epi.shift = d.shift;
  epi.residual = static_cast<const __nv_bfloat16*>(d.residual);
  epi.aux = static_cast<const __nv_bfloat16*>(d.aux);
  epi.aux_mode = d.aux ? d.aux_mode : CB_AUX_NONE;
  epi.act = d.act;
  epi.out = d.out;
  epi.out_ld = d.out_ld;
  epi.out_fp32 = d.out_fp32;
  epi.out2 = static_cast<__nv_bfloat16*>(d.out2);
  epi.out2_ld = d.out2_ld;
  epi.rowmap = d.rowmap;
  epi.H = d.map_h;
  epi.W = d.map_w;
  epi.seed = d.dropout_seed;
  epi.dbg = g_gemm_timeline;
  epi.mn3d = 0;
  {
    const DropCfg dc = make_drop(d.dropout_p, d.dropout_seed);
    epi.drop_thresh = dc.thresh;
    epi.drop_inv_keep = dc.inv_keep;
    epi.seed_off = dc.offset;
  }

  if (d.mode == CB_GEMM_TN || d.mode == CB_GEMM_NN) {
    const bool nn = d.mode == CB_GEMM_NN;
    CB_REQUIRE(d.n % 8 == 0, "cb_gemm(TN): n must be a multiple of 8 (got %d)", d.n);
    CB_REQUIRE(d.k % 8 == 0, "cb_gemm(TN): k must be a multiple of 8 (got %d)", d.k);
    CB_REQUIRE(d.out_ld % 8 == 0, "cb_gemm(TN): out_ld must be a multiple of 8");
    CB_REQUIRE(!d.residual || d.res_ld % 8 == 0, "cb_gemm(TN): res_ld must be a multiple of 8");
    CB_REQUIRE(!d.aux || d.aux_ld % 8 == 0, "cb_gemm(TN): aux_ld must be a multiple of 8");
    CB_REQUIRE((reinterpret_cast<uintptr_t>(d.residual) & 15) == 0, "cb_gemm(TN): residual must be 16-byte aligned");
    CB_REQUIRE((reinterpret_cast<uintptr_t>(d.aux) & 15) == 0, "cb_gemm(TN): aux must be 16-byte aligned");
    CB_REQUIRE((reinterpret_cast<uintptr_t>(d.a) & 15) == 0, "cb_gemm(TN): a must be 16-byte aligned");
    CB_REQUIRE((reinterpret_cast<uintptr_t>(d.b) & 15) == 0, "cb_gemm(TN): b must be 16-byte aligned");
    CB_REQUIRE((reinterpret_cast<uintptr_t>(d.out) & 15) == 0, "cb_gemm(TN): out must be 16-byte aligned");
    CB_REQUIRE((reinterpret_cast<uintptr_t>(d.out2) & 15) == 0, "cb_gemm(TN): out2 must be 16-byte aligned");
    CB_REQUIRE(!d.out2 || d.out2_ld % 8 == 0, "cb_gemm(TN): out2_ld must be a multiple of 8");
    CB_REQUIRE(!(d.out2 && d.out_fp32), "cb_gemm(TN): out2 requires a bf16 primary output");
    CB_REQUIRE(d.rowmap == CB_ROWMAP_NONE || (d.map_h > 0 && d.map_w > 0), "cb_gemm: rowmap needs map_h/map_w");
    CB_REQUIRE(d.ntaps == 1 || d.tap_w > 2, "cb_gemm: tap modes need tap_w (padded row pitch in pixels)");
    CB_REQUIRE(d.block_n == 0 || d.block_n == 64 || d.block_n == 128 || d.block_n == 256, "cb_gemm: block_n must be 0, 64, 128 or 256 (got %d)",
               d.block_n);
    const LaunchCfg lc = choose_config(d, sm_count());
    switch (lc.bn) {
      case 64: return nn ? launch_gemm<64, 2>(d, epi, stream) : launch_gemm<64, 0>(d, epi, stream);
      case 128: return nn ? launch_gemm<128, 2>(d, epi, stream) : launch_gemm<128, 0>(d, epi, stream);
      default: CB_REQUIRE(false, "cb_gemm: no tile width for block_n %d", d.block_n);
    }
  } else {
    const int rc = check_wgrad_desc(d, "cb_gemm(WGRAD)");
    if (rc != CB_OK) return rc;
    const LaunchCfg lc = choose_config(d, plan_sm_count());
    return launch_wgrad(&d, 1, lc.bn, lc.splits, stream, "cb_gemm");
  }
  return CB_ERR_INVALID;
}

extern "C" int cb_gemm_wgrad_group(const cb_gemm_desc* descs, int n, void* stream_v) {
  using namespace cb;
  CB_REQUIRE(descs != nullptr && n >= 1, "cb_gemm_wgrad_group: no problems");
  for (int i = 0; i < n; ++i) {
    char who[48];
    snprintf(who, sizeof(who), "cb_gemm_wgrad_group: problem %d", i);
    const int rc = check_wgrad_desc(descs[i], who);
    if (rc != CB_OK) return rc;
  }
  const GroupPlan gp = group_plan(descs, n, plan_sm_count());
  if (!gp.groupable) {
    for (int i = 0; i < n; ++i) {
      cb_gemm_desc d = descs[i];
      d.workspace = descs[0].workspace;
      d.workspace_bytes = descs[0].workspace_bytes;
      const int rc = cb_gemm(&d, stream_v);
      if (rc != CB_OK) return rc;
    }
    return CB_OK;
  }
  return launch_wgrad(descs, n, gp.bn, gp.split, static_cast<cudaStream_t>(stream_v), "cb_gemm_wgrad_group");
}

extern "C" int64_t cb_gemm_workspace_bytes(const cb_gemm_desc* d) {
  using namespace cb;
  if (d == nullptr || d->mode != CB_GEMM_WGRAD || d->m <= 0 || d->n <= 0 || d->k <= 0) return 0;
  return wgrad_ws_bytes(*d, choose_config(*d, sm_count_device()).splits);
}

extern "C" int64_t cb_gemm_wgrad_group_workspace_bytes(const cb_gemm_desc* descs, int n) {
  using namespace cb;
  if (descs == nullptr || n < 1) return 0;
  for (int i = 0; i < n; ++i)
    if (descs[i].mode != CB_GEMM_WGRAD || descs[i].m <= 0 || descs[i].n <= 0 || descs[i].k <= 0) return 0;
  return group_ws_bytes(descs, n);
}
```

clipbert_b200/csrc/host_util.h:

```cpp
#pragma once
#include <cuda.h>
#include <cuda_runtime.h>
#include <stdint.h>

#include <atomic>
#include <cstdarg>
#include <cstdio>
#include <utility>

#include "../../include/clipbert_b200.h"

namespace cb {

void set_error(const char* fmt, ...);
extern std::atomic<int64_t> g_launches;

inline int check_launch(const char* what) {
  cudaError_t e = cudaGetLastError();
  if (e != cudaSuccess) {
    set_error("%s: launch failed: %s", what, cudaGetErrorString(e));
    return CB_ERR_CUDA;
  }
  g_launches.fetch_add(1, std::memory_order_relaxed);
  return CB_OK;
}

extern std::atomic<int> g_pdl;

extern std::atomic<int> g_det;
int launch_ordered_sum(const float* part, int n, float* out, cudaStream_t stream, const char* what);

template <bool kGemm, typename... KArgs, typename... Args>
inline void launch_k_impl(void (*kern)(KArgs...), dim3 grid, dim3 block, size_t smem, cudaStream_t stream, Args&&... args) {
  cudaLaunchConfig_t cfg = {};
  cfg.gridDim = grid;
  cfg.blockDim = block;
  cfg.dynamicSmemBytes = smem;
  cfg.stream = stream;
  cudaLaunchAttribute attr[1];
  attr[0].id = cudaLaunchAttributeProgrammaticStreamSerialization;
  attr[0].val.programmaticStreamSerializationAllowed = 1;
  cfg.attrs = attr;
  const int mode = g_pdl.load(std::memory_order_relaxed);
  cfg.numAttrs = (mode == 1 || (mode == 2 && !kGemm)) ? 1 : 0;
  (void)cudaLaunchKernelEx(&cfg, kern, std::forward<Args>(args)...);
}
template <typename... KArgs, typename... Args>
inline void launch_k(void (*kern)(KArgs...), dim3 grid, dim3 block, size_t smem, cudaStream_t stream, Args&&... args) {
  launch_k_impl<false>(kern, grid, block, smem, stream, std::forward<Args>(args)...);
}
template <typename... KArgs, typename... Args>
inline void launch_gemm_k(void (*kern)(KArgs...), dim3 grid, dim3 block, size_t smem, cudaStream_t stream, Args&&... args) {
  launch_k_impl<true>(kern, grid, block, smem, stream, std::forward<Args>(args)...);
}

bool get_tmap_2d(CUtensorMap* out, const void* base, uint64_t inner, uint64_t rows, uint64_t ld,
                 uint32_t box_inner, uint32_t box_rows);

bool get_tmap_3d_mn(CUtensorMap* out, const void* base, uint64_t cols, uint64_t rows, uint64_t ld, uint32_t box_rows, uint32_t nblk);

#define CB_REQUIRE(cond, ...)        \
  do {                               \
    if (!(cond)) {                   \
      cb::set_error(__VA_ARGS__);    \
      return CB_ERR_INVALID;         \
    }                                \
  } while (0)

inline int ceil_div(int64_t a, int64_t b) { return static_cast<int>((a + b - 1) / b); }

}
```

clipbert_b200/grid_feat.py:

```python
import math

import torch
from torch import nn

from . import ops
from .params import FlatGroup

RESNET50_STAGES = (("res2", 3, 64, 256, 1), ("res3", 4, 128, 512, 2), ("res4", 6, 256, 1024, 2), ("res5", 3, 512, 2048, 2))
FROZEN_BN_EPS = 1e-5
STEM_KP = 152

_D2_CONFIG_TEXT = """MODEL:
  META_ARCHITECTURE: GeneralizedRCNN
  BACKBONE: {NAME: build_resnet_backbone, FREEZE_AT: %d}
  RESNETS: {DEPTH: 50, OUT_FEATURES: [res5], RES5_DILATION: 1, STRIDE_IN_1X1: true, NORM: FrozenBN}
  WEIGHTS: detectron2://ImageNetPretrained/MSRA/R-50.pkl
"""


def _require_cuda(t):
    assert t.is_cuda, "GridFeatBackbone runs on CUDA only (no CPU fallback)"


class FrozenBatchNorm2d(nn.Module):

    def __init__(self, c):
        super().__init__()
        self.register_buffer("weight", torch.ones(c))
        self.register_buffer("bias", torch.zeros(c))
        self.register_buffer("running_mean", torch.zeros(c))
        self.register_buffer("running_var", torch.ones(c))


class ConvBN(nn.Module):

    def __init__(self, cin, cout, k, norm=True):
        super().__init__()
        self.weight = nn.Parameter(torch.empty(cout, cin, k, k))
        nn.init.kaiming_normal_(self.weight, mode="fan_out", nonlinearity="relu")
        if norm:
            self.norm = FrozenBatchNorm2d(cout)
        self.cin, self.cout, self.k = cin, cout, k


class BottleneckBlock(nn.Module):
    def __init__(self, cin, mid, cout, stride, has_shortcut):
        super().__init__()
        if has_shortcut:
            self.shortcut = ConvBN(cin, cout, 1)
        self.conv1 = ConvBN(cin, mid, 1)
        self.conv2 = ConvBN(mid, mid, 3)
        self.conv3 = ConvBN(mid, cout, 1)
        self.stride, self.has_shortcut = stride, has_shortcut
        self.cin, self.mid, self.cout = cin, mid, cout


class _Stem(nn.Module):
    def __init__(self):
        super().__init__()
        self.conv1 = ConvBN(3, 64, 7)


class _Backbone(nn.Module):
    def __init__(self):
        super().__init__()
        self.stem = _Stem()
        cin = 64
        for name, nblocks, mid, cout, stride in RESNET50_STAGES:
            blocks = []
            for b in range(nblocks):
                blocks.append(BottleneckBlock(cin, mid, cout, stride if b == 0 else 1, b == 0))
                cin = cout
            setattr(self, name, nn.Sequential(*blocks))


class _Feature(nn.Module):

    def __init__(self):
        super().__init__()
        self.backbone = _Backbone()


class _GridEncoderConv(nn.Module):
    def __init__(self, cin, cout):
        super().__init__()
        self.weight = nn.Parameter(torch.empty(cout, cin, 3, 3))
        nn.init.kaiming_uniform_(self.weight, a=math.sqrt(5))
        self.cin, self.cout, self.k = cin, cout, 3


class _CnnFn(torch.autograd.Function):
    @staticmethod
    def forward(ctx, module, images, anchor):
        grid, stash = module._forward_impl(images, need_backward=True)
        module._pending_backward += 1
        ctx.module = module
        ctx.stash = stash
        return grid

    @staticmethod
    def backward(ctx, dgrid):
        stash, ctx.stash = ctx.stash, None
        m = ctx.module
        m._pending_backward = max(0, m._pending_backward - 1)
        if stash is not None:
            m._backward_impl(stash, dgrid, last=m._pending_backward == 0)
        return None, None, None


class GridFeatBackbone(nn.Module):
    def __init__(self, detectron2_model_cfg=None, config=None, input_format="BGR", freeze_at=2):
        super().__init__()
        assert input_format == "BGR", "detectron 2 image input format should be BGR"
        hidden = getattr(config, "hidden_size", 768) if config is not None else 768
        cin = getattr(config, "backbone_channel_in_size", 2048) if config is not None else 2048
        self.feature = _Feature()
        self.grid_encoder = nn.Sequential(_GridEncoderConv(cin, hidden))
        self.input_format = input_format
        self.config = config
        self.freeze_at = freeze_at
        self.detectron2_model_cfg = detectron2_model_cfg
        self._flat = None
        self._bn = None
        self._dirty = True
        self._capture = None
        self._inject = None
        self._pending_backward = 0
        self._bucket_hook = None
        self._segments = None
        self._pad_pool = {}
        self.pixel_mean = None
        self.raw_float_inputs = False
        self.pixel_std = None
        self.stem_mode = "s2d"
        self._s2d_ld = 16
        self._optimizer_emits_packed = False
        if freeze_at < 1:
            raise NotImplementedError("GridFeatBackbone: FREEZE_AT = 0 (trainable stem) is not supported on the H100 path")
        bb = self.feature.backbone
        if freeze_at >= 1:
            for p in bb.stem.parameters():
                p.requires_grad = False
        for si, (name, *_r) in enumerate(RESNET50_STAGES):
            if freeze_at >= si + 2:
                for p in getattr(bb, name).parameters():
                    p.requires_grad = False

    @property
    def config_file(self):
        return _D2_CONFIG_TEXT % self.freeze_at

    def load_state_dict(self, state_dict, strict=False, **kw):
        import os

        from . import load_save
        if isinstance(state_dict, (str, bytes, os.PathLike)):
            if not os.path.exists(state_dict):
                raise FileNotFoundError("GridFeatBackbone.load_state_dict: checkpoint %r does not exist (the reference falls back to the d2 "
                                        "config's MODEL.WEIGHTS URL, which this offline path cannot download)" % (state_dict,))
        loaded, ignored = load_save.load_detectron2_checkpoint(self, state_dict)
        self._dirty = True
        missing = sorted(k for k in self.state_dict() if k not in loaded)
        if strict and missing:
            raise RuntimeError("GridFeatBackbone.load_state_dict: missing keys %s" % missing[:8])
        return torch.nn.modules.module._IncompatibleKeys(missing, ignored)

    def mark_weights_updated(self):
        self._dirty = True

    def _convs(self):
        bb = self.feature.backbone
        out = [("stem.conv1", bb.stem.conv1)]
        for name, *_r in RESNET50_STAGES:
            for bi, blk in enumerate(getattr(bb, name)):
                if blk.has_shortcut:
                    out.append(("%s.%d.shortcut" % (name, bi), blk.shortcut))
                out.append(("%s.%d.conv1" % (name, bi), blk.conv1))
                out.append(("%s.%d.conv2" % (name, bi), blk.conv2))
                out.append(("%s.%d.conv3" % (name, bi), blk.conv3))
        out.append(("grid_encoder.0", self.grid_encoder[0]))
        return out

    def _any_trainable(self):
        return any(m.weight.requires_grad for _, m in self._convs())

    def _ensure_ready(self, device):
        if self._flat is None or not self._flat.is_current() or self._flat.device != device:
            flat = FlatGroup(device)
            for name, m in self._convs():
                m._e = flat.add(name, m.weight, kind="conv")
            flat.materialize()
            self._flat = flat
            convs = [m for _, m in self._convs() if hasattr(m, "norm")]
            ctot = sum(m.cout for m in convs)
            bufs = {k: torch.empty(ctot, dtype=torch.float32, device=device) for k in ("weight", "bias", "running_mean", "running_var")}
            off = 0
            for m in convs:
                for k in bufs:
                    v = bufs[k][off: off + m.cout]
                    v.copy_(getattr(m.norm, k).to(device))
                    setattr(m.norm, k, v)
                m._bn_off = off
                off += m.cout
            self._bn = bufs
            self._bn_scale = torch.empty(ctot, dtype=torch.float32, device=device)
            self._bn_shift = torch.empty(ctot, dtype=torch.float32, device=device)
            self._stem_w = torch.zeros(64, STEM_KP, dtype=torch.bfloat16, device=device)
            self._stem_w_s2d = torch.zeros(64, 256, dtype=torch.bfloat16, device=device)
            self._segments = None
            self._pad_pool = {}
            self._dirty = True
        if self._dirty or self._flat.needs_repack():
            self._repack()
            self._dirty = False
            self._flat.needs_repack()

    @torch.no_grad()
    def _repack(self):
        b = self._bn
        torch.rsqrt(b["running_var"] + FROZEN_BN_EPS, out=self._bn_scale)
        self._bn_scale.mul_(b["weight"])
        torch.addcmul(b["bias"], b["running_mean"], self._bn_scale, value=-1.0, out=self._bn_shift)
        flat = self._flat
        if self._segments is None:
            rows = []
            for name, m in self._convs():
                e = m._e
                rows.append([e["offset"], e["numel"], m.k * m.k * m.cin, m._bn_off if hasattr(m, "norm") else -1])
            self._segments = torch.tensor(rows, dtype=torch.int64, device=flat.master.device)
        ops.cast_scale_segments(flat.master, flat.packed, self._segments, self._bn_scale)
        for name, m in self._convs():
            e = m._e
            n = e["numel"]
            row_len = m.k * m.k * m.cin
            if hasattr(m, "norm"):
                m._scale, m._shift = self._bn_scale[m._bn_off: m._bn_off + m.cout], self._bn_shift[m._bn_off: m._bn_off + m.cout]
            else:
                m._scale = m._shift = None
            m._w = flat.packed[e["offset"]: e["offset"] + n].view(m.cout, row_len)
            m._gw = flat.grad[e["offset"]: e["offset"] + n].view(m.cout, row_len)
        stem = self.feature.backbone.stem.conv1
        if self.pixel_std is not None and any(float(v) != 1.0 for v in self.pixel_std):
            e = stem._e
            w32 = flat.master[e["offset"]: e["offset"] + e["numel"]].view(64, 49, 3) * self._bn_scale[stem._bn_off: stem._bn_off + 64].view(64, 1, 1)
            r, g, b_ = (float(v) for v in self.pixel_std)
            inv = torch.tensor([1.0 / b_, 1.0 / g, 1.0 / r], dtype=torch.float32, device=w32.device)
            stem._w.copy_((w32 * inv).reshape(64, 147))
        self._stem_w[:, :147] = stem._w
        self._pack_stem_s2d(stem._w)
        stem._w = self._stem_w

    def optimizer_segments(self):
        return [dict(param=m.weight, row_len=m.k * m.k * m.cin, scale_off=m._bn_off if hasattr(m, "norm") else -1, emit=True)
                for _, m in self._convs()]

    def optimizer_scales(self):
        return self._bn_scale

    def packed_written_by_optimizer(self):
        stem = self.feature.backbone.stem.conv1
        if stem.weight.requires_grad:
            e = stem._e
            self._stem_w[:, :147] = self._flat.packed[e["offset"]: e["offset"] + e["numel"]].view(64, 147)
            self._pack_stem_s2d(self._stem_w[:, :147])
        self._dirty = False
        self._flat.needs_repack()

    def _pack_stem_s2d(self, w147):
        w = torch.zeros(64, 8, 8, 4, dtype=w147.dtype, device=w147.device)
        w[:, :7, :7, :3] = w147.reshape(64, 7, 7, 3)
        self._stem_w_s2d.copy_(w.view(64, 4, 2, 4, 2, 4).permute(0, 1, 3, 2, 4, 5).reshape(64, 256))

    def _pad_get(self, rows, ch, device):
        lst = self._pad_pool.setdefault((rows, ch), [])
        return lst.pop() if lst else torch.zeros(rows, ch, dtype=torch.bfloat16, device=device)

    def _pad_put(self, t):
        if t is not None:
            self._pad_pool.setdefault((t.shape[0], t.shape[1]), []).append(t)

    def forward(self, x):
        _require_cuda(x)
        self._ensure_ready(x.device)
        if not (torch.is_grad_enabled() and self._any_trainable()):
            return self._forward_impl(x, need_backward=False)[0]
        anchor = next(m.weight for _, m in self._convs() if m.weight.requires_grad)
        return _CnnFn.apply(self, x, anchor)

    def _conv1x1(self, m, x, rows, act, residual=None, rowmap=ops.ROWMAP_NONE, hw=None, out=None):
        if out is None:
            out = torch.empty(rows, m.cout, dtype=torch.bfloat16, device=x.device)
        kw = dict(mode=ops.CB_GEMM_TN, m=rows, n=m.cout, k=m.cin, a=x, a_rows=rows, a_ld=m.cin, b=m._w, b_rows=m.cout,
                  b_ld=m.cin, shift=m._shift, act=act, out=out, out_ld=m.cout, rowmap=rowmap)
        if residual is not None:
            kw.update(residual=residual, res_ld=m.cout)
        if hw is not None:
            kw.update(map_h=hw[0], map_w=hw[1])
        ops.gemm(**kw)
        return out

    def _conv3x3(self, m, x_pad, n, h, w, act):
        p = n * (h + 2) * (w + 2)
        out = torch.empty(n * h * w, m.cout, dtype=torch.bfloat16, device=x_pad.device)
        ops.gemm(mode=ops.CB_GEMM_TN, m=p, n=m.cout, k=m.cin, a=x_pad, a_rows=p, a_ld=m.cin, b=m._w, b_rows=m.cout,
                 b_ld=9 * m.cin, ntaps=9, tap_w=w + 2, tap_sign=1, shift=m._shift, act=act, out=out, out_ld=m.cout,
                 rowmap=ops.ROWMAP_UNPAD, map_h=h, map_w=w)
        return out

    def _forward_impl(self, images, need_backward):
        dev = images.device
        bsz, n_frms, c, h, w = images.shape
        assert c == 3
        n = bsz * n_frms
        x = images.reshape(n, c, h, w)
        if x.dtype == torch.uint8 or self.raw_float_inputs:
            assert self.pixel_mean is not None, "raw frames need pixel_mean (fused ImageNorm)"
            mean = tuple(float(v) for v in self.pixel_mean)
            x = x if x.dtype in (torch.uint8, torch.float32) else x.float()
        else:
            x = x.float() if x.dtype != torch.float32 else x
            mean = (0.0, 0.0, 0.0)
        x = x.contiguous()
        bb = self.feature.backbone
        bf16 = torch.bfloat16
        ho, wo = (h - 1) // 2 + 1, (w - 1) // 2 + 1
        hh, ww = (ho - 1) // 2 + 1, (wo - 1) // 2 + 1
        stem = bb.stem.conv1
        cur = torch.empty(n * hh * ww, 64, dtype=bf16, device=dev)
        mode = self.stem_mode
        if mode == "s2d":
            hs, ws = ho + 3, wo + 3
            rows = n * hs * ws
            ld = self._s2d_ld
            s2d = torch.empty((rows + 4) * ld, dtype=bf16, device=dev)
            ops.stem_s2d(x, s2d, n, h, w, ld, mean)
            c1 = torch.empty(rows, 64, dtype=bf16, device=dev)
            kw = dict(mode=ops.CB_GEMM_TN, m=rows, n=64, k=64, a=s2d, a_rows=rows, a_ld=ld, b=self._stem_w_s2d, b_rows=64, b_ld=256,
                      ntaps=4, tap_w=ws, tap_sign=1, shift=stem._shift, act=ops.ACT_RELU, out=c1, out_ld=64)
            try:
                ops.gemm(**kw)
            except RuntimeError as e:
                if ld == 64 or "cuTensorMapEncodeTiled" not in str(e):
                    raise
                self._s2d_ld = ld = 64
                s2d = torch.empty((rows + 4) * ld, dtype=bf16, device=dev)
                ops.stem_s2d(x, s2d, n, h, w, ld, mean)
                ops.gemm(**dict(kw, a=s2d, a_ld=ld))
            del s2d
            ops.maxpool3x3s2(c1, cur, n, ho, wo, 64, row_pitch=ws, img_pitch=hs * ws)
        else:
            col = torch.empty(n * ho * wo, STEM_KP, dtype=bf16, device=dev)
            ops.stem_im2col(x, col, n, h, w, STEM_KP, mean)
            c1 = torch.empty(n * ho * wo, 64, dtype=bf16, device=dev)
            ops.gemm(mode=ops.CB_GEMM_TN, m=n * ho * wo, n=64, k=STEM_KP, a=col, a_rows=n * ho * wo, a_ld=STEM_KP, b=stem._w,
                     b_rows=64, b_ld=STEM_KP, shift=stem._shift, act=ops.ACT_RELU, out=c1, out_ld=64)
            del col
            ops.maxpool3x3s2(c1, cur, n, ho, wo, 64)
        del c1
        if self._capture is not None:
            self._capture["stem"] = cur.view(n, hh, ww, 64)
        blocks = []
        stage_names = [s[0] for s in RESNET50_STAGES]
        for si, name in enumerate(stage_names):
            stage = getattr(bb, name)
            for bi, blk in enumerate(stage):
                last = (si == len(stage_names) - 1) and (bi == len(stage) - 1)
                if self._inject is not None and ("%s.%d" % (name, bi)) in self._inject:
                    cur = self._inject["%s.%d" % (name, bi)].to(device=dev, dtype=bf16).reshape(n * hh * ww, -1).contiguous()
                x_in, h_in, w_in = cur, hh, ww
                if blk.stride == 2:
                    hh, ww = (hh - 1) // 2 + 1, (ww - 1) // 2 + 1
                    xs = torch.empty(n * hh * ww, blk.cin, dtype=bf16, device=dev)
                    ops.subsample2(x_in, xs, n, h_in, w_in, blk.cin)
                else:
                    xs = x_in
                rows = n * hh * ww
                sc = self._conv1x1(blk.shortcut, xs, rows, ops.ACT_NONE) if blk.has_shortcut else xs
                a_pad = self._pad_get(n * (hh + 2) * (ww + 2), blk.mid, dev)
                self._conv1x1(blk.conv1, xs, rows, ops.ACT_RELU, rowmap=ops.ROWMAP_PAD, hw=(hh, ww), out=a_pad)
                b = self._conv3x3(blk.conv2, a_pad, n, hh, ww, ops.ACT_RELU)
                if last:
                    y = self._pad_get(n * (hh + 2) * (ww + 2), blk.cout, dev)
                    self._conv1x1(blk.conv3, b, rows, ops.ACT_RELU, residual=sc, rowmap=ops.ROWMAP_PAD, hw=(hh, ww), out=y)
                else:
                    y = self._conv1x1(blk.conv3, b, rows, ops.ACT_RELU, residual=sc)
                trainable = blk.conv1.weight.requires_grad
                if not (need_backward and trainable):
                    self._pad_put(a_pad)
                if need_backward and trainable:
                    blocks.append(dict(name="%s.%d" % (name, bi), blk=blk, x_in=x_in, xs=xs, a_pad=a_pad, b=b, y=y, h=hh, w=ww, h_in=h_in, w_in=w_in,
                                       first_trainable=not blocks))
                cur = y
            if self._capture is not None:
                self._capture[name] = (cur.view(n, hh + 2, ww + 2, -1)[:, 1:-1, 1:-1] if name == "res5" else cur.view(n, hh, ww, -1))
        ge = self.grid_encoder[0]
        gconv = self._conv3x3(ge, cur, n, hh, ww, ops.ACT_NONE)
        gh, gw = hh // 2, ww // 2
        grid = torch.empty(bsz, n_frms, gh, gw, ge.cout, dtype=bf16, device=dev)
        ops.maxpool2x2_relu_fwd(gconv, grid, n, hh, ww, ge.cout)
        stash = None
        if not need_backward:
            self._pad_put(cur)
        if need_backward:
            stash = dict(n=n, h=hh, w=ww, res5_pad=cur, gconv=gconv, blocks=blocks)
            if self._capture is not None:
                self._capture["stash"] = stash
        return grid, stash

    def _wgrad_kw(self, m, dy, x, p, ntaps=1, tap_w=0):
        return dict(mode=ops.CB_GEMM_WGRAD, m=m.cout, n=m.cin, k=p, a=dy, a_rows=p, a_ld=m.cout, b=x, b_rows=p, b_ld=m.cin,
                    ntaps=ntaps, tap_w=tap_w, tap_sign=1, scale=m._scale, out=m._gw, out_ld=ntaps * m.cin, out_fp32=1)

    def _wgrad(self, m, dy, x, p, ntaps=1, tap_w=0):
        ops.gemm(**self._wgrad_kw(m, dy, x, p, ntaps, tap_w))

    def _dgrad1x1(self, m, dy, rows, residual=None, aux=None, rowmap=ops.ROWMAP_NONE, hw=None, out=None):
        if out is None:
            out = torch.empty(rows, m.cin, dtype=torch.bfloat16, device=dy.device)
        kw = dict(mode=ops.CB_GEMM_NN, m=rows, n=m.cin, k=m.cout, a=dy, a_rows=rows, a_ld=m.cout, b=m._w, b_rows=m.cout,
                  b_ld=m.cin, out=out, out_ld=m.cin, rowmap=rowmap)
        if residual is not None:
            kw.update(residual=residual, res_ld=m.cin)
        if aux is not None:
            kw.update(aux=aux, aux_ld=m.cin, aux_mode=ops.AUX_RELU_MASK)
        if hw is not None:
            kw.update(map_h=hw[0], map_w=hw[1])
        ops.gemm(**kw)
        return out

    def _dgrad3x3(self, m, dy_pad, n, h, w, aux_pad):
        p = n * (h + 2) * (w + 2)
        out = torch.empty(n * h * w, m.cin, dtype=torch.bfloat16, device=dy_pad.device)
        ops.gemm(mode=ops.CB_GEMM_NN, m=p, n=m.cin, k=m.cout, a=dy_pad, a_rows=p, a_ld=m.cout, b=m._w, b_rows=m.cout,
                 b_ld=9 * m.cin, ntaps=9, tap_w=w + 2, tap_sign=-1, aux=aux_pad, aux_ld=m.cin, aux_mode=ops.AUX_RELU_MASK,
                 out=out, out_ld=m.cin, rowmap=ops.ROWMAP_UNPAD, map_h=h, map_w=w)
        return out

    def _backward_impl(self, stash, dgrid, last=True):
        self._flat.attach_grads()
        dev = dgrid.device
        bf16 = torch.bfloat16
        n, h, w = stash["n"], stash["h"], stash["w"]
        ge = self.grid_encoder[0]
        dgrid = dgrid.to(bf16).contiguous()
        p = n * (h + 2) * (w + 2)
        sq = ops.SideQueue()
        recycle = []
        dg_pad = torch.empty(p, ge.cout, dtype=bf16, device=dev)
        ops.maxpool2x2_relu_bwd(dgrid, stash["gconv"], dg_pad, n, h, w, ge.cout)
        res5_pad = stash["res5_pad"]
        recycle.append(res5_pad)
        if ge.weight.requires_grad:
            sq.run(lambda: self._wgrad(ge, dg_pad, res5_pad, p, ntaps=9, tap_w=w + 2), dg_pad, res5_pad)
        blocks = stash["blocks"]
        if blocks:
            g = self._dgrad3x3(ge, dg_pad, n, h, w, res5_pad)
        del dg_pad
        for st in (reversed(blocks) if blocks else ()):
            blk, hh, ww = st["blk"], st["h"], st["w"]
            rows = n * hh * ww
            pp = n * (hh + 2) * (ww + 2)
            wg = [self._wgrad_kw(blk.conv3, g, st["b"], rows)]
            db_pad = self._pad_get(pp, blk.mid, dev)
            recycle += [db_pad, st["a_pad"]]
            self._dgrad1x1(blk.conv3, g, rows, aux=st["b"], rowmap=ops.ROWMAP_PAD, hw=(hh, ww), out=db_pad)
            wg.append(self._wgrad_kw(blk.conv2, db_pad, st["a_pad"], pp, ntaps=9, tap_w=ww + 2))
            da = self._dgrad3x3(blk.conv2, db_pad, n, hh, ww, st["a_pad"])
            wg.append(self._wgrad_kw(blk.conv1, da, st["xs"], rows))
            if blk.has_shortcut:
                wg.append(self._wgrad_kw(blk.shortcut, g, st["xs"], rows))
            if ops.group_wgrad in (1, 2, 4):
                sq.run(lambda: ops.gemm_wgrad_group(wg), g, st["b"], db_pad, st["a_pad"], da, st["xs"])
            else:
                sq.run(lambda: [ops.gemm(**kw) for kw in wg], g, st["b"], db_pad, st["a_pad"], da, st["xs"])
            if blk.has_shortcut:
                if last and self._bucket_hook is not None and st["name"] == "res5.0":
                    self._bucket_hook(self._flat.grad, blk.shortcut._e["offset"], sq.side if sq.forked else None)
                if st["first_trainable"]:
                    break
                dxs = self._dgrad1x1(blk.shortcut, g, rows)
                dxs = self._dgrad1x1(blk.conv1, da, rows, residual=dxs)
                g = torch.empty(n * st["h_in"] * st["w_in"], blk.cin, dtype=bf16, device=dev)
                if blk.stride == 2:
                    ops.unsubsample2_mask(dxs, st["x_in"], g, n, st["h_in"], st["w_in"], blk.cin)
                else:
                    ops.relu_mask(dxs, st["x_in"], g)
            else:
                if st["first_trainable"]:
                    break
                g = self._dgrad1x1(blk.conv1, da, rows, residual=g, aux=st["x_in"])
        sq.join()
        for t in recycle:
            self._pad_put(t)
        if not self._optimizer_emits_packed:
            self._dirty = True
```

clipbert_b200/ops.py:

```python
import ctypes

import torch

from . import _lib as L
from ._lib import (ACT_GELU, ACT_GELU_STASH_GRAD, ACT_NONE, ACT_RELU, ACT_TANH, AUX_GELU_GRAD, AUX_MUL, AUX_NONE,
                   AUX_RELU_MASK, AUX_TANH_GRAD, CB_GEMM_TN, CB_GEMM_WGRAD, ROWMAP_NONE, ROWMAP_PAD, ROWMAP_UNPAD)

CB_GEMM_NN = 2
_c = ctypes
_vp, _i, _i64, _f, _u64 = _c.c_void_p, _c.c_int, _c.c_int64, _c.c_float, _c.c_uint64

_SIGS = {
    "cb_layernorm_fwd": [_vp, _vp, _vp, _vp, _vp, _i, _i, _f, _vp],
    "cb_layernorm_bwd": [_vp, _vp, _vp, _vp, _vp, _vp, _vp, _vp, _vp, _i, _i, _f, _u64, _vp],
    "cb_embed_text_fwd": [_vp, _vp, _vp, _vp, _vp, _vp, _vp, _vp, _i, _i, _i, _i, _i, _f, _f, _u64, _vp],
    "cb_embed_text_bwd": [_vp] * 12 + [_i, _i, _i, _i, _i, _f, _u64, _vp],
    "cb_embed_visual_fwd": [_vp, _vp, _i, _vp, _vp, _vp, _vp, _vp, _vp, _vp, _i, _i, _i, _i, _i, _i, _i, _f, _f, _u64, _vp],
    "cb_embed_visual_bwd": [_vp, _vp, _vp, _vp, _i] + [_vp] * 12 + [_i, _i, _i, _i, _i, _i, _i, _i, _f, _u64, _vp],
    "cb_colsum": [_vp, _i64, _vp, _i, _i, _vp],
    "cb_dropout": [_vp, _vp, _i64, _f, _u64, _vp],
    "cb_dropout_offset_advance": [_vp, _vp, _vp],
    "cb_gelu_bwd": [_vp, _vp, _vp, _i64, _vp],
    "cb_pad_cast": [_vp, _i64, _vp, _i, _i, _i, _vp],
    "cb_cast_scale": [_vp, _vp, _i64, _vp, _i64, _vp],
    "cb_cast_bf16_f32": [_vp, _vp, _i64, _vp],
    "cb_cast_scale_segments": [_vp, _vp, _vp, _i, _vp, _vp],
    "cb_nvls_allreduce_f32": [_vp, _i64, _i, _i, _f, _i, _vp],
    "cb_clip_lse_loss": [_vp, _vp, _vp, _vp, _i, _i, _i, _f, _vp],
    "cb_clip_pool_ce_loss": [_vp, _vp, _vp, _vp, _i, _i, _i, _i, _f, _vp],
    "cb_cross_entropy_fwd": [_vp, _i64, _vp, _vp, _vp, _i64, _i, _i64, _vp],
    "cb_cross_entropy_bwd": [_vp, _i64, _vp, _vp, _vp, _vp, _i64, _i64, _i, _i64, _vp],
    "cb_attention_fwd": [_vp, _i64, _vp, _vp, _i64, _vp, _i, _i, _i, _i, _i, _f, _u64, _vp],
    "cb_attention_bwd": [_vp, _i64, _vp, _vp, _vp, _i64, _vp, _vp, _i64, _i, _i, _i, _i, _i, _f, _u64, _vp],
    "cb_attention_probs": [_vp, _i64, _vp, _vp, _vp, _i, _i, _i, _i, _i, _f, _u64, _vp],
    "cb_stem_im2col": [_vp, _i, _vp, _i, _i, _i, _i, _f, _f, _f, _vp],
    "cb_maxpool3x3s2": [_vp, _vp, _i, _i, _i, _i, _vp],
    "cb_maxpool3x3s2_strided": [_vp, _vp, _i, _i, _i, _i, _i64, _i64, _vp],
    "cb_stem_s2d": [_vp, _i, _vp, _i, _i, _i, _i, _f, _f, _f, _vp],
    "cb_resize_pad": [_vp, _i, _vp, _i, _i, _i, _i, _i, _i, _vp],
    "cb_subsample2": [_vp, _vp, _i, _i, _i, _i, _vp],
    "cb_unsubsample2_mask": [_vp, _vp, _vp, _i, _i, _i, _i, _vp],
    "cb_maxpool2x2_relu_fwd": [_vp, _vp, _i, _i, _i, _i, _vp],
    "cb_maxpool2x2_relu_bwd": [_vp, _vp, _vp, _i, _i, _i, _i, _vp],
    "cb_relu_mask": [_vp, _vp, _vp, _i64, _vp],
    "cb_layernorm_bwd_det": [_vp, _vp, _vp, _vp, _vp, _vp, _vp, _vp, _vp, _i, _i, _f, _u64, _vp, _i64, _vp],
    "cb_embed_text_bwd_det": [_vp] * 12 + [_i, _i, _i, _i, _i, _f, _u64, _vp, _i64, _vp],
    "cb_embed_visual_bwd_det": [_vp, _vp, _vp, _vp, _i] + [_vp] * 12 + [_i, _i, _i, _i, _i, _i, _i, _i, _f, _u64, _vp, _i64, _vp],
    "cb_colsum_det": [_vp, _i64, _vp, _i, _i, _vp, _i64, _vp],
    "cb_clip_lse_loss_det": [_vp, _vp, _vp, _vp, _i, _i, _i, _f, _vp, _i64, _vp],
    "cb_clip_pool_ce_loss_det": [_vp, _vp, _vp, _vp, _i, _i, _i, _i, _f, _vp, _i64, _vp],
    "cb_sumsq_det": [_vp, _i64, _vp, _i, _vp, _vp, _i64, _vp],
    "cb_layernorm_bwd_scratch_bytes": [_i],
    "cb_embed_text_bwd_scratch_bytes": [_i, _i],
    "cb_embed_visual_bwd_scratch_bytes": [_i, _i, _i],
    "cb_colsum_scratch_bytes": [_i, _i],
    "cb_clip_loss_scratch_bytes": [_i],
    "cb_sumsq_scratch_bytes": [_i64, _vp, _i],
}
_bound = {}


def _fn(name):
    f = _bound.get(name)
    if f is None:
        f = getattr(L.lib(), name)
        f.argtypes = _SIGS[name]
        f.restype = _c.c_int64 if name.endswith("_scratch_bytes") else _c.c_int
        _bound[name] = f
    return f


def _p(t):
    return None if t is None else t.data_ptr()


def _s():
    return torch.cuda.current_stream().cuda_stream


_op_timing = None


def set_op_timing(events):
    global _op_timing
    _op_timing = events


def _call(name, *args):
    if _op_timing is not None:
        e0, e1 = torch.cuda.Event(enable_timing=True), torch.cuda.Event(enable_timing=True)
        e0.record()
    rc = _fn(name)(*args)
    if rc != 0:
        raise RuntimeError("%s failed (%d): %s" % (name, rc, L.lib().cb_last_error().decode()))
    if _op_timing is not None:
        e1.record()
        _op_timing.append((name, e0, e1))


def launch_count():
    return int(L.lib().cb_launch_count())


def set_attention_flash(on):
    L.lib().cb_debug_attention_flash(int(bool(on)))


def set_attention_flash_pipe(on):
    L.lib().cb_debug_attention_flash_pipe(int(bool(on)))


def set_attention_rows48(on):
    L.lib().cb_debug_attention_rows48(int(bool(on)))


def set_mn3d(on):
    L.lib().cb_debug_gemm_mn3d(int(bool(on)))


def set_occ2(mode, max_gflop=0.0):
    f = L.lib().cb_debug_gemm_occ2
    f.argtypes = [ctypes.c_int, ctypes.c_double]
    f.restype = None
    f(int(mode), float(max_gflop))


def dropout_offset_bind(word):
    f = L.lib().cb_dropout_offset_bind
    f.argtypes = [_vp]
    f.restype = _c.c_int
    f(None if word is None else word.data_ptr())


def dropout_offset_advance(counter, snapshot=None):
    _call("cb_dropout_offset_advance", _p(counter), _p(snapshot), _s())


def set_sm_limit(n):
    L.lib().cb_debug_gemm_sm_limit(int(n))


def set_pdl(enable):
    return int(L.lib().cb_set_pdl(2 if int(enable) == 2 else int(bool(enable))))


_lib_deterministic = False


def set_deterministic(on):
    return bool(L.lib().cb_set_deterministic(int(bool(on))))


def deterministic():
    global _lib_deterministic
    on = torch.are_deterministic_algorithms_enabled()
    if on != _lib_deterministic:
        set_deterministic(on)
        _lib_deterministic = on
    return on


def _scratch(nbytes, like):
    return torch.empty(max(4, (int(nbytes) + 3) // 4), dtype=torch.float32, device=like.device)


def _scratch_args(nbytes, like):
    t = _scratch(nbytes, like)
    return t, t.numel() * 4


class SideQueue:
    _streams = {}

    def __init__(self, enabled=True):
        self.enabled = bool(enabled) and overlap_wgrad
        self.keep = []
        self.side = None
        self.forked = False

    def _side_stream(self):
        dev = torch.cuda.current_device()
        st = SideQueue._streams.get(dev)
        if st is None:
            st = SideQueue._streams[dev] = torch.cuda.Stream(device=dev)
        return st

    def run(self, fn, *keep):
        if not self.enabled:
            fn()
            return
        if self.side is None:
            self.side = self._side_stream()
        main = torch.cuda.current_stream()
        ev = torch.cuda.Event()
        ev.record(main)
        self.side.wait_event(ev)
        with torch.cuda.stream(self.side):
            fn()
        self.keep.extend(keep)
        self.forked = True

    def join(self):
        if self.forked:
            torch.cuda.current_stream().wait_stream(self.side)
            self.forked = False
        self.keep.clear()


overlap_wgrad = True


_GEMM_PTR_FIELDS = ("a", "b", "scale", "shift", "residual", "aux", "out", "out2", "workspace")
_gemm_timing = None


def set_gemm_timing(events):
    global _gemm_timing
    _gemm_timing = events


_tuning = None
_gemm_record = None


def gemm_key(kw):
    return "m%d n%d k%d mode%d t%d r%d a%d o%d f%d rm%d act%d" % (
        kw["m"], kw["n"], kw["k"], kw.get("mode", 0), kw.get("ntaps", 1), kw.get("residual") is not None, kw.get("aux") is not None,
        kw.get("out2") is not None, kw.get("out_fp32", 0), kw.get("rowmap", 0), kw.get("act", 0))


def _load_tuning():
    global _tuning
    import json
    import os
    path = os.path.join(os.path.dirname(os.path.abspath(__file__)), "gemm_tuning.json")
    _tuning = {}
    if os.path.exists(path) and not os.environ.get("CB_NO_TUNING"):
        try:
            _tuning = json.load(open(path)).get("configs", {})
        except Exception:
            _tuning = {}


def _gemm_descs(kws):
    arr = (L.GemmDesc * len(kws))()
    for d, kw in zip(arr, kws):
        d.ntaps = 1
        d.tap_sign = 1
        d.split_k = 0
        for k, v in kw.items():
            if k in _GEMM_PTR_FIELDS:
                v = _p(v) if isinstance(v, torch.Tensor) else v
            setattr(d, k, v)
    return arr


def gemm_workspace_bytes(kw):
    return int(L.lib().cb_gemm_workspace_bytes(_gemm_descs([kw])))


def gemm_wgrad_group_workspace_bytes(kws):
    return int(L.lib().cb_gemm_wgrad_group_workspace_bytes(_gemm_descs(kws), len(kws)))


def _with_workspace(kw, nbytes):
    if nbytes <= 0:
        return kw
    ws, nb = _scratch_args(nbytes, kw["out"])
    return dict(kw, workspace=ws, workspace_bytes=nb)


def _launch_gemm(name, kws):
    arr = _gemm_descs(kws)
    timing = _gemm_timing is not None or _op_timing is not None
    if timing:
        e0, e1 = torch.cuda.Event(enable_timing=True), torch.cuda.Event(enable_timing=True)
        e0.record()
    if name == "cb_gemm":
        rc = L.lib().cb_gemm(arr, _s())
    else:
        rc = L.lib().cb_gemm_wgrad_group(arr, len(kws), _s())
    if rc != 0:
        raise RuntimeError("%s failed (%d): %s" % (name, rc, L.lib().cb_last_error().decode()))
    if timing:
        e1.record()
        if _gemm_timing is not None:
            _gemm_timing.append((e0, e1))
        if _op_timing is not None:
            d = arr[0]
            label = ("gemm mode=%d m=%d n=%d k=%d taps=%d res=%d aux=%d o2=%d f32=%d rm=%d" % (
                d.mode, d.m, d.n, d.k, d.ntaps, bool(d.residual), bool(d.aux), bool(d.out2), d.out_fp32, d.rowmap)
                if name == "cb_gemm" else "gemm wgrad group x%d" % len(kws))
            _op_timing.append((label, e0, e1))


def gemm(**kw):
    if _tuning is None:
        _load_tuning()
    if _gemm_record is not None:
        _gemm_record.append(dict(kw))
    if _tuning and "block_n" not in kw and "reserved" not in kw:
        t = _tuning.get(gemm_key(kw))
        if t is not None:
            kw = dict(kw, block_n=t[0], split_k=t[1], reserved=(t[2] << 8) | (32 if (len(t) > 3 and t[3]) else 0))
    if kw.get("mode", CB_GEMM_TN) == CB_GEMM_WGRAD and deterministic():
        kw = _with_workspace(kw, gemm_workspace_bytes(kw))
    _launch_gemm("cb_gemm", [kw])


group_wgrad = 3


def gemm_wgrad_group(kws):
    if not kws:
        return
    if len(kws) == 1:
        for kw in kws:
            gemm(**kw)
        return
    if _gemm_record is not None:
        _gemm_record.append(dict(group=[dict(kw) for kw in kws]))
    kws = list(kws)
    if deterministic():
        kws[0] = _with_workspace(kws[0], gemm_wgrad_group_workspace_bytes(kws))
    _launch_gemm("cb_gemm_wgrad_group", kws)


def layernorm_fwd(x, gamma, beta, y, stats, eps):
    _call("cb_layernorm_fwd", _p(x), _p(gamma), _p(beta), _p(y), _p(stats), x.shape[0], x.shape[1], eps, _s())


def layernorm_bwd(dy, x, stats, gamma, dx, dx_drop, dgamma, dbeta, dbias_drop, p, seed):
    if (dgamma is not None or dbeta is not None or dbias_drop is not None) and deterministic():
        layernorm_bwd_det(dy, x, stats, gamma, dx, dx_drop, dgamma, dbeta, dbias_drop, p, seed,
                          _scratch(layernorm_bwd_scratch_bytes(x.shape[0]), x))
        return
    _call("cb_layernorm_bwd", _p(dy), _p(x), _p(stats), _p(gamma), _p(dx), _p(dx_drop), _p(dgamma), _p(dbeta),
          _p(dbias_drop), x.shape[0], x.shape[1], p, seed, _s())


def layernorm_bwd_scratch_bytes(m):
    return int(_fn("cb_layernorm_bwd_scratch_bytes")(m))


def layernorm_bwd_det(dy, x, stats, gamma, dx, dx_drop, dgamma, dbeta, dbias_drop, p, seed, scratch):
    _call("cb_layernorm_bwd_det", _p(dy), _p(x), _p(stats), _p(gamma), _p(dx), _p(dx_drop), _p(dgamma), _p(dbeta),
          _p(dbias_drop), x.shape[0], x.shape[1], p, seed, _p(scratch), scratch.numel() * 4, _s())


def embed_text_fwd(ids, word, pos, type0, gamma, beta, out, stats, nseq, lt, l, eps, p, seed):
    _call("cb_embed_text_fwd", _p(ids), _p(word), _p(pos), _p(type0), _p(gamma), _p(beta), _p(out), _p(stats), nseq, lt, l,
          word.shape[0], word.shape[1], eps, p, seed, _s())


def embed_text_bwd(dh, ids, word, pos, type0, gamma, stats, dword, dpos, dtype0, dgamma, dbeta, nseq, lt, l, p, seed):
    if deterministic():
        embed_text_bwd_det(dh, ids, word, pos, type0, gamma, stats, dword, dpos, dtype0, dgamma, dbeta, nseq, lt, l, p, seed,
                           _scratch(embed_text_bwd_scratch_bytes(nseq, lt), dh))
        return
    _call("cb_embed_text_bwd", _p(dh), _p(ids), _p(word), _p(pos), _p(type0), _p(gamma), _p(stats), _p(dword), _p(dpos),
          _p(dtype0), _p(dgamma), _p(dbeta), nseq, lt, l, word.shape[0], word.shape[1], p, seed, _s())


def embed_text_bwd_scratch_bytes(nseq, lt):
    return int(_fn("cb_embed_text_bwd_scratch_bytes")(nseq, lt))


def embed_text_bwd_det(dh, ids, word, pos, type0, gamma, stats, dword, dpos, dtype0, dgamma, dbeta, nseq, lt, l, p, seed, scratch):
    _call("cb_embed_text_bwd_det", _p(dh), _p(ids), _p(word), _p(pos), _p(type0), _p(gamma), _p(stats), _p(dword), _p(dpos),
          _p(dtype0), _p(dgamma), _p(dbeta), nseq, lt, l, word.shape[0], word.shape[1], p, seed, _p(scratch), scratch.numel() * 4,
          _s())


def embed_visual_fwd(grid, seq2vid, n_ex, rowemb, colemb, type0, gamma, beta, out, stats, nseq, t, gh, gw, lt, l, eps, p,
                     seed):
    _call("cb_embed_visual_fwd", _p(grid), _p(seq2vid), n_ex, _p(rowemb), _p(colemb), _p(type0), _p(gamma), _p(beta), _p(out),
          _p(stats), nseq, t, gh, gw, lt, l, rowemb.shape[1], eps, p, seed, _s())


def embed_visual_bwd(dh, grid, seq2vid, vid_start, n_ex, rowemb, colemb, type0, gamma, stats, dv_tmp, dgrid, drow, dcol,
                     dtype0, dgamma, dbeta, nseq, nvid, t, gh, gw, lt, l, p, seed):
    if deterministic():
        embed_visual_bwd_det(dh, grid, seq2vid, vid_start, n_ex, rowemb, colemb, type0, gamma, stats, dv_tmp, dgrid, drow, dcol,
                             dtype0, dgamma, dbeta, nseq, nvid, t, gh, gw, lt, l, p, seed,
                             _scratch(embed_visual_bwd_scratch_bytes(nseq, gh, gw), dh))
        return
    _call("cb_embed_visual_bwd", _p(dh), _p(grid), _p(seq2vid), _p(vid_start), n_ex, _p(rowemb), _p(colemb), _p(type0),
          _p(gamma), _p(stats), _p(dv_tmp), _p(dgrid), _p(drow), _p(dcol), _p(dtype0), _p(dgamma), _p(dbeta), nseq, nvid, t,
          gh, gw, lt, l, rowemb.shape[1], p, seed, _s())


def embed_visual_bwd_scratch_bytes(nseq, gh, gw):
    return int(_fn("cb_embed_visual_bwd_scratch_bytes")(nseq, gh, gw))


def embed_visual_bwd_det(dh, grid, seq2vid, vid_start, n_ex, rowemb, colemb, type0, gamma, stats, dv_tmp, dgrid, drow, dcol,
                         dtype0, dgamma, dbeta, nseq, nvid, t, gh, gw, lt, l, p, seed, scratch):
    _call("cb_embed_visual_bwd_det", _p(dh), _p(grid), _p(seq2vid), _p(vid_start), n_ex, _p(rowemb), _p(colemb), _p(type0),
          _p(gamma), _p(stats), _p(dv_tmp), _p(dgrid), _p(drow), _p(dcol), _p(dtype0), _p(dgamma), _p(dbeta), nseq, nvid, t,
          gh, gw, lt, l, rowemb.shape[1], p, seed, _p(scratch), scratch.numel() * 4, _s())


def nvls_allreduce(multicast_ptr, n, rank, world, scale, max_ctas=0):
    _call("cb_nvls_allreduce_f32", multicast_ptr, n, rank, world, scale, max_ctas, _s())


def clip_lse_loss(logits, labels, loss, dlogits, n_clips, nseq, ncls, grad_scale=1.0):
    if deterministic():
        clip_lse_loss_det(logits, labels, loss, dlogits, n_clips, nseq, ncls, grad_scale, _scratch(clip_loss_scratch_bytes(nseq), logits))
        return
    _call("cb_clip_lse_loss", _p(logits), _p(labels), _p(loss), _p(dlogits), n_clips, nseq, ncls, grad_scale, _s())


def clip_pool_ce_loss(logits, labels, loss, dlogits, n_clips, nseq, ncls, pool, grad_scale=1.0):
    if deterministic():
        clip_pool_ce_loss_det(logits, labels, loss, dlogits, n_clips, nseq, ncls, pool, grad_scale,
                              _scratch(clip_loss_scratch_bytes(nseq), logits))
        return
    _call("cb_clip_pool_ce_loss", _p(logits), _p(labels), _p(loss), _p(dlogits), n_clips, nseq, ncls, pool, grad_scale, _s())


def clip_loss_scratch_bytes(nseq):
    return int(_fn("cb_clip_loss_scratch_bytes")(nseq))


def clip_lse_loss_det(logits, labels, loss, dlogits, n_clips, nseq, ncls, grad_scale, scratch):
    _call("cb_clip_lse_loss_det", _p(logits), _p(labels), _p(loss), _p(dlogits), n_clips, nseq, ncls, grad_scale, _p(scratch),
          scratch.numel() * 4, _s())


def clip_pool_ce_loss_det(logits, labels, loss, dlogits, n_clips, nseq, ncls, pool, grad_scale, scratch):
    _call("cb_clip_pool_ce_loss_det", _p(logits), _p(labels), _p(loss), _p(dlogits), n_clips, nseq, ncls, pool, grad_scale,
          _p(scratch), scratch.numel() * 4, _s())


def cross_entropy_fwd(logits, labels, loss, lse, ignore_index=-100):
    _call("cb_cross_entropy_fwd", _p(logits), logits.stride(0), _p(labels), _p(loss), _p(lse), logits.shape[0], logits.shape[1], ignore_index, _s())


def cross_entropy_bwd(logits, labels, lse, grad_loss, dlogits, ignore_index=-100):
    _call("cb_cross_entropy_bwd", _p(logits), logits.stride(0), _p(labels), _p(lse), _p(grad_loss), _p(dlogits), dlogits.stride(0), logits.shape[0],
          logits.shape[1], ignore_index, _s())


def colsum(x, out, m, n, ld=None):
    if deterministic():
        colsum_det(x, out, m, n, ld, _scratch(colsum_scratch_bytes(m, n), x))
        return
    _call("cb_colsum", _p(x), n if ld is None else ld, _p(out), m, n, _s())


def colsum_scratch_bytes(m, n):
    return int(_fn("cb_colsum_scratch_bytes")(m, n))


def colsum_det(x, out, m, n, ld, scratch):
    _call("cb_colsum_det", _p(x), n if ld is None else ld, _p(out), m, n, _p(scratch), scratch.numel() * 4, _s())


def sumsq_scratch_bytes(n, chunks, nchunks):
    return int(_fn("cb_sumsq_scratch_bytes")(n, _p(chunks), nchunks))


def sumsq_det(x, n, chunks, nchunks, out, scratch):
    _call("cb_sumsq_det", _p(x), n, _p(chunks), nchunks, _p(out), _p(scratch), scratch.numel() * 4, _s())


def dropout(x, y, p, seed):
    _call("cb_dropout", _p(x), _p(y), x.numel(), p, seed, _s())


def gelu_bwd(dy, u, dx):
    _call("cb_gelu_bwd", _p(dy), _p(u), _p(dx), dy.numel(), _s())


def pad_cast(src, dst):
    _call("cb_pad_cast", _p(src), src.stride(0), _p(dst), src.shape[0], src.shape[1], dst.shape[1], _s())


def cast_scale(src, dst, rowscale=None, row_len=1):
    _call("cb_cast_scale", _p(src), _p(rowscale), row_len, _p(dst), src.numel(), _s())


def cast_bf16_f32(src, dst):
    _call("cb_cast_bf16_f32", _p(src), _p(dst), src.numel(), _s())


def cast_scale_segments(master, packed, segments, scales):
    _call("cb_cast_scale_segments", _p(master), _p(packed), _p(segments), segments.shape[0], _p(scales), _s())


def attention_fwd(qkv, text_mask, ctx, lse, nseq, l, lt, heads, p, seed):
    _call("cb_attention_fwd", _p(qkv), qkv.shape[1], _p(text_mask), _p(ctx), ctx.shape[1], _p(lse), nseq, l, lt, heads, 64, p,
          seed, _s())


def attention_bwd(qkv, text_mask, ctx, dctx, lse, dqkv, nseq, l, lt, heads, p, seed):
    _call("cb_attention_bwd", _p(qkv), qkv.shape[1], _p(text_mask), _p(ctx), _p(dctx), ctx.shape[1], _p(lse), _p(dqkv),
          dqkv.shape[1], nseq, l, lt, heads, 64, p, seed, _s())


def attention_probs(qkv, text_mask, lse, probs, nseq, l, lt, heads, p, seed):
    assert probs.dtype == torch.float32 and probs.is_contiguous() and probs.numel() == nseq * heads * l * l
    _call("cb_attention_probs", _p(qkv), qkv.shape[1], _p(text_mask), _p(lse), _p(probs), nseq, l, lt, heads, 64, p, seed, _s())


def stem_im2col(x, out, n, h, w, kp, mean=(0.0, 0.0, 0.0)):
    dt = 0 if x.dtype == torch.float32 else 1
    _call("cb_stem_im2col", _p(x), dt, _p(out), n, h, w, kp, mean[0], mean[1], mean[2], _s())


def stem_s2d(x, out, n, h, w, ld, mean=(0.0, 0.0, 0.0)):
    dt = 0 if x.dtype == torch.float32 else 1
    _call("cb_stem_s2d", _p(x), dt, _p(out), n, h, w, ld, mean[0], mean[1], mean[2], _s())


def resize_pad(x, y, new_h, new_w):
    dt = 0 if x.dtype == torch.float32 else 1
    _call("cb_resize_pad", _p(x), dt, _p(y), x.numel() // (x.shape[-1] * x.shape[-2]), x.shape[-2], x.shape[-1], new_h, new_w, y.shape[-1], _s())


def maxpool3x3s2(x, y, n, h, w, c, row_pitch=None, img_pitch=None):
    if row_pitch is None:
        _call("cb_maxpool3x3s2", _p(x), _p(y), n, h, w, c, _s())
    else:
        _call("cb_maxpool3x3s2_strided", _p(x), _p(y), n, h, w, c, row_pitch, img_pitch, _s())


def subsample2(x, y, n, h, w, c):
    _call("cb_subsample2", _p(x), _p(y), n, h, w, c, _s())


def unsubsample2_mask(dsub, act, dx, n, h, w, c):
    _call("cb_unsubsample2_mask", _p(dsub), _p(act), _p(dx), n, h, w, c, _s())


def maxpool2x2_relu_fwd(x, y, n, h, w, c):
    _call("cb_maxpool2x2_relu_fwd", _p(x), _p(y), n, h, w, c, _s())


def maxpool2x2_relu_bwd(dy, x, dx_pad, n, h, w, c):
    _call("cb_maxpool2x2_relu_bwd", _p(dy), _p(x), _p(dx_pad), n, h, w, c, _s())


def relu_mask(dy, act, dx):
    _call("cb_relu_mask", _p(dy), _p(act), _p(dx), dy.numel(), _s())
```

include/clipbert_b200.h:

```cpp
#ifndef CLIPBERT_B200_H_
#define CLIPBERT_B200_H_

#include <stddef.h>
#include <stdint.h>

#ifdef __cplusplus
extern "C" {
#endif

typedef enum cb_status {
  CB_OK = 0,
  CB_ERR_INVALID = -1,
  CB_ERR_CUDA = -2,
  CB_ERR_UNSUPPORTED = -3
} cb_status;

const char* cb_last_error(void);
int cb_version(void);
int cb_sm_arch(void);
int64_t cb_launch_count(void);
int cb_set_pdl(int enable);

int cb_set_deterministic(int enable);

int cb_dropout_offset_bind(const uint64_t* device_word);
int cb_dropout_offset_advance(uint64_t* counter, uint64_t* snapshot, void* stream);

enum { CB_GEMM_TN = 0, CB_GEMM_WGRAD = 1, CB_GEMM_NN = 2 };
enum {
  CB_ACT_NONE = 0, CB_ACT_RELU = 1, CB_ACT_GELU = 2, CB_ACT_TANH = 3,
  CB_ACT_GELU_STASH_GRAD = 4
};
enum {
  CB_AUX_NONE = 0,
  CB_AUX_RELU_MASK = 1,
  CB_AUX_GELU_GRAD = 2,
  CB_AUX_TANH_GRAD = 3,
  CB_AUX_MUL = 4
};
enum {
  CB_ROWMAP_NONE = 0,
  CB_ROWMAP_PAD = 1,
  CB_ROWMAP_UNPAD = 2
};

typedef struct cb_gemm_desc {
  int32_t mode;
  int32_t m, n, k;
  const void* a;
  int64_t a_rows, a_ld;
  const void* b;
  int64_t b_rows, b_ld;
  int32_t ntaps, tap_w, tap_sign;
  int32_t split_k;
  const float* scale;
  const float* shift;
  const void* residual;
  int64_t res_ld;
  const void* aux;
  int64_t aux_ld;
  int32_t aux_mode;
  int32_t act;
  void* out;
  int64_t out_ld;
  int32_t out_fp32;
  void* out2;
  int64_t out2_ld;
  int32_t rowmap, map_h, map_w;
  float dropout_p;
  uint64_t dropout_seed;
  int32_t block_n;
  int32_t reserved;
  void* workspace;
  int64_t workspace_bytes;
} cb_gemm_desc;

int cb_gemm(const cb_gemm_desc* desc, void* stream);
int64_t cb_gemm_workspace_bytes(const cb_gemm_desc* desc);
int cb_gemm_wgrad_group(const cb_gemm_desc* descs, int n, void* stream);
int64_t cb_gemm_wgrad_group_workspace_bytes(const cb_gemm_desc* descs, int n);

int cb_layernorm_fwd(const void* x, const float* gamma, const float* beta, void* y, float* stats, int m, int hidden,
                     float eps, void* stream);
int cb_layernorm_bwd(const void* dy, const void* x, const float* stats, const float* gamma, void* dx, void* dx_drop,
                     float* dgamma, float* dbeta, float* dbias_drop, int m, int hidden, float dropout_p,
                     uint64_t dropout_seed, void* stream);
int64_t cb_layernorm_bwd_scratch_bytes(int m);
int cb_layernorm_bwd_det(const void* dy, const void* x, const float* stats, const float* gamma, void* dx, void* dx_drop,
                         float* dgamma, float* dbeta, float* dbias_drop, int m, int hidden, float dropout_p,
                         uint64_t dropout_seed, float* scratch, int64_t scratch_bytes, void* stream);

int cb_embed_text_fwd(const int64_t* ids, const float* word, const float* pos, const float* type0, const float* gamma,
                      const float* beta, void* out, float* stats, int nseq, int lt, int l, int vocab, int hidden,
                      float eps, float dropout_p, uint64_t seed, void* stream);
int cb_embed_text_bwd(const void* dh, const int64_t* ids, const float* word, const float* pos, const float* type0,
                      const float* gamma, const float* stats, float* dword, float* dpos, float* dtype0, float* dgamma,
                      float* dbeta, int nseq, int lt, int l, int vocab, int hidden, float dropout_p, uint64_t seed,
                      void* stream);
int cb_embed_visual_fwd(const void* grid, const int32_t* seq2vid, int n_ex, const float* rowemb, const float* colemb,
                        const float* type0, const float* gamma, const float* beta, void* out, float* stats, int nseq,
                        int t, int gh, int gw, int lt, int l, int hidden, float eps, float dropout_p, uint64_t seed,
                        void* stream);
int cb_embed_visual_bwd(const void* dh, const void* grid, const int32_t* seq2vid, const int32_t* vid_start, int n_ex,
                        const float* rowemb, const float* colemb, const float* type0, const float* gamma,
                        const float* stats, float* dv_tmp, void* dgrid, float* drow, float* dcol, float* dtype0,
                        float* dgamma, float* dbeta, int nseq, int nvid, int t, int gh, int gw, int lt, int l, int hidden,
                        float dropout_p, uint64_t seed, void* stream);
int64_t cb_embed_text_bwd_scratch_bytes(int nseq, int lt);
int cb_embed_text_bwd_det(const void* dh, const int64_t* ids, const float* word, const float* pos, const float* type0,
                          const float* gamma, const float* stats, float* dword, float* dpos, float* dtype0, float* dgamma,
                          float* dbeta, int nseq, int lt, int l, int vocab, int hidden, float dropout_p, uint64_t seed,
                          float* scratch, int64_t scratch_bytes, void* stream);
int64_t cb_embed_visual_bwd_scratch_bytes(int nseq, int gh, int gw);
int cb_embed_visual_bwd_det(const void* dh, const void* grid, const int32_t* seq2vid, const int32_t* vid_start, int n_ex,
                            const float* rowemb, const float* colemb, const float* type0, const float* gamma,
                            const float* stats, float* dv_tmp, void* dgrid, float* drow, float* dcol, float* dtype0,
                            float* dgamma, float* dbeta, int nseq, int nvid, int t, int gh, int gw, int lt, int l, int hidden,
                            float dropout_p, uint64_t seed, float* scratch, int64_t scratch_bytes, void* stream);

int cb_attention_fwd(const void* qkv, int64_t ld_qkv, const int64_t* text_mask, void* ctx, int64_t ld_ctx, float* lse,
                     int nseq, int l, int lt, int heads, int head_dim, float dropout_p, uint64_t seed, void* stream);
int cb_attention_bwd(const void* qkv, int64_t ld_qkv, const int64_t* text_mask, const void* ctx, const void* dctx,
                     int64_t ld_ctx, const float* lse, void* dqkv, int64_t ld_dqkv, int nseq, int l, int lt, int heads,
                     int head_dim, float dropout_p, uint64_t seed, void* stream);
int cb_attention_probs(const void* qkv, int64_t ld_qkv, const int64_t* text_mask, const float* lse, float* probs, int nseq,
                       int l, int lt, int heads, int head_dim, float dropout_p, uint64_t seed, void* stream);

int cb_colsum(const void* x, int64_t ld, float* out, int m, int n, void* stream);
int64_t cb_colsum_scratch_bytes(int m, int n);
int cb_colsum_det(const void* x, int64_t ld, float* out, int m, int n, float* scratch, int64_t scratch_bytes, void* stream);
int cb_dropout(const void* x, void* y, int64_t n, float p, uint64_t seed, void* stream);
int cb_gelu_bwd(const void* dy, const void* u, void* dx, int64_t n, void* stream);
int cb_pad_cast(const float* in, int64_t in_ld, void* out, int rows, int c, int cpad, void* stream);
int cb_cast_scale(const float* in, const float* rowscale, int64_t row_len, void* out, int64_t n, void* stream);
int cb_cast_bf16_f32(const void* in, float* out, int64_t n, void* stream);
int cb_cast_scale_segments(const float* master, void* packed, const int64_t* segments, int nseg, const float* scales, void* stream);

int cb_resize_pad(const void* x, int in_dtype, float* y, int planes, int h, int w, int new_h, int new_w, int max_size, void* stream);
int cb_stem_im2col(const void* x, int in_dtype, void* out, int n, int h, int w, int kp, float mean_r, float mean_g,
                   float mean_b, void* stream);
int cb_stem_s2d(const void* x, int in_dtype, void* out, int n, int h, int w, int ld, float mean_r, float mean_g, float mean_b,
                void* stream);
int cb_maxpool3x3s2(const void* x, void* y, int n, int h, int w, int c, void* stream);
int cb_maxpool3x3s2_strided(const void* x, void* y, int n, int h, int w, int c, int64_t row_pitch, int64_t img_pitch, void* stream);
int cb_subsample2(const void* x, void* y, int n, int h, int w, int c, void* stream);
int cb_unsubsample2_mask(const void* dsub, const void* act, void* dx, int n, int h, int w, int c, void* stream);
int cb_maxpool2x2_relu_fwd(const void* x, void* y, int n, int h, int w, int c, void* stream);
int cb_maxpool2x2_relu_bwd(const void* dy, const void* x, void* dx_pad, int n, int h, int w, int c, void* stream);
int cb_relu_mask(const void* dy, const void* act, void* dx, int64_t n, void* stream);

int cb_clip_lse_loss(const float* logits, const int64_t* labels, float* loss, float* dlogits, int n_clips, int nseq, int ncls,
                     float grad_scale, void* stream);
int cb_clip_pool_ce_loss(const float* logits, const int64_t* labels, float* loss, float* dlogits, int n_clips, int nseq, int ncls, int pool,
                         float grad_scale, void* stream);
int64_t cb_clip_loss_scratch_bytes(int nseq);
int cb_clip_lse_loss_det(const float* logits, const int64_t* labels, float* loss, float* dlogits, int n_clips, int nseq, int ncls,
                         float grad_scale, float* scratch, int64_t scratch_bytes, void* stream);
int cb_clip_pool_ce_loss_det(const float* logits, const int64_t* labels, float* loss, float* dlogits, int n_clips, int nseq, int ncls,
                             int pool, float grad_scale, float* scratch, int64_t scratch_bytes, void* stream);
int cb_cross_entropy_fwd(const float* logits, int64_t ld, const int64_t* labels, float* loss, float* lse, int64_t rows, int ncls,
                         int64_t ignore_index, void* stream);
int cb_cross_entropy_bwd(const float* logits, int64_t ld, const int64_t* labels, const float* lse, const float* grad_loss, float* dlogits,
                         int64_t dld, int64_t rows, int ncls, int64_t ignore_index, void* stream);

int cb_nvls_allreduce_f32(void* multicast_ptr, int64_t n, int rank, int world, float scale, int max_ctas, void* stream);

int cb_sumsq(const float* x, int64_t n, const int64_t* chunks, int nchunks, float* out, void* stream);
int64_t cb_sumsq_scratch_bytes(int64_t n, const int64_t* chunks, int nchunks);
int cb_sumsq_det(const float* x, int64_t n, const int64_t* chunks, int nchunks, float* out, float* scratch, int64_t scratch_bytes,
                 void* stream);
int cb_adamw_step(float* master, float* grad, float* exp_avg, float* exp_avg_sq, void* packed_bf16, const int64_t* chunks,
                  int nchunks, const float* hyper, const float* scales, const float* grad_sumsq, float max_norm, int zero_grad,
                  void* stream);

#ifdef __cplusplus
}
#endif
#endif
```

Before: 3986.

## Use TMA im2col loads so 3x3 convs compute only interior pixels

Adds an im2col TMA tensor-map path for the 3x3 conv forward, dgrad and wgrad GEMMs. The GEMM M (or wgrad K) dimension now covers only interior pixels instead of the whole zero-bordered padded image, so the border rows are no longer computed and discarded. Tap offsets are expressed as im2col offsets, and residual and aux inputs use matching im2col maps. The cost is per-tile pixel decode arithmetic and a dependence on im2col TMA box semantics being correct for tiles that cross image boundaries.

```diff
diff --git a/clipbert_b200/_lib.py b/clipbert_b200/_lib.py
--- a/clipbert_b200/_lib.py
+++ b/clipbert_b200/_lib.py
@@ -30,6 +30,7 @@
         ("dropout_p", ctypes.c_float), ("dropout_seed", ctypes.c_uint64),
         ("block_n", ctypes.c_int32), ("reserved", ctypes.c_int32),
         ("workspace", ctypes.c_void_p), ("workspace_bytes", ctypes.c_int64),
+        ("tap_mode", ctypes.c_int32),
     ]
 
 
diff --git a/clipbert_b200/csrc/api.cu b/clipbert_b200/csrc/api.cu
--- a/clipbert_b200/csrc/api.cu
+++ b/clipbert_b200/csrc/api.cu
@@ -154,6 +154,64 @@
   return true;
 }
 
+typedef CUresult (*EncodeIm2colFn)(CUtensorMap*, CUtensorMapDataType, cuuint32_t, void*, const cuuint64_t*, const cuuint64_t*,
+                                   const int*, const int*, cuuint32_t, cuuint32_t, const cuuint32_t*, CUtensorMapInterleave,
+                                   CUtensorMapSwizzle, CUtensorMapL2promotion, CUtensorMapFloatOOBfill);
+
+static EncodeIm2colFn get_encode_im2col_fn() {
+  static EncodeIm2colFn fn = nullptr;
+  static std::once_flag once;
+  std::call_once(once, [] {
+    void* p = nullptr;
+    cudaDriverEntryPointQueryResult q;
+    cudaError_t e = cudaGetDriverEntryPoint("cuTensorMapEncodeIm2col", &p, cudaEnableDefault, &q);
+    if (e == cudaSuccess && q == cudaDriverEntryPointSuccess) fn = reinterpret_cast<EncodeIm2colFn>(p);
+  });
+  return fn;
+}
+
+bool get_tmap_im2col(CUtensorMap* out, const void* base, uint64_t channels, uint64_t ld, uint64_t wp, uint64_t hp, uint64_t n,
+                     uint32_t pixels) {
+  static std::mutex mu;
+  static std::unordered_map<TmapKey, CUtensorMap, TmapKeyHash> cache;
+  TmapKey key{reinterpret_cast<uint64_t>(base), channels, n, ld, static_cast<uint32_t>(wp << 16 | hp), pixels};
+  std::lock_guard<std::mutex> lock(mu);
+  auto it = cache.find(key);
+  if (it != cache.end()) {
+    *out = it->second;
+    return true;
+  }
+  EncodeIm2colFn enc = get_encode_im2col_fn();
+  if (!enc) {
+    set_error("cuTensorMapEncodeIm2col driver entry point not available");
+    return false;
+  }
+  if ((reinterpret_cast<uint64_t>(base) & 15) != 0 || ((ld * 2) & 15) != 0 || (channels & 63) != 0 || wp < 3 || hp < 3 ||
+      wp >= 65536 || hp >= 65536) {
+    set_error("im2col tensor map: base %p, pixel pitch %llu, channels %llu (a multiple of 64), %llu x %llu padded", base,
+              (unsigned long long)ld, (unsigned long long)channels, (unsigned long long)hp, (unsigned long long)wp);
+    return false;
+  }
+  alignas(64) CUtensorMap tm;
+  cuuint64_t dims[4] = {channels, wp, hp, n};
+  cuuint64_t strides[3] = {ld * 2, ld * 2 * wp, ld * 2 * wp * hp};
+  const int lower[2] = {0, 0}, upper[2] = {-2, -2};
+  cuuint32_t estr[4] = {1, 1, 1, 1};
+  CUresult r = enc(&tm, CU_TENSOR_MAP_DATA_TYPE_BFLOAT16, 4, const_cast<void*>(base), dims, strides, lower, upper, 64, pixels, estr,
+                   CU_TENSOR_MAP_INTERLEAVE_NONE, CU_TENSOR_MAP_SWIZZLE_128B, CU_TENSOR_MAP_L2_PROMOTION_L2_256B,
+                   CU_TENSOR_MAP_FLOAT_OOB_FILL_NONE);
+  if (r != CUDA_SUCCESS) {
+    set_error("cuTensorMapEncodeIm2col failed (%d) channels=%llu w=%llu h=%llu n=%llu ld=%llu pixels=%u", (int)r,
+              (unsigned long long)channels, (unsigned long long)wp, (unsigned long long)hp, (unsigned long long)n,
+              (unsigned long long)ld, pixels);
+    return false;
+  }
+  if (cache.size() > 65536) cache.clear();
+  cache.emplace(key, tm);
+  *out = tm;
+  return true;
+}
+
 }
 
 extern "C" {
diff --git a/clipbert_b200/csrc/common.cuh b/clipbert_b200/csrc/common.cuh
--- a/clipbert_b200/csrc/common.cuh
+++ b/clipbert_b200/csrc/common.cuh
@@ -94,6 +94,16 @@
       "cp.async.bulk.tensor.3d.shared::cluster.global.mbarrier::complete_tx::bytes "
       "[%0], [%1, {%3, %4, %5}], [%2];" ::"r"(smem_u32(smem_dst)),
       "l"(map), "r"(smem_u32(bar)), "r"(c0), "r"(c1), "r"(c2)
+      : "memory");
+}
+
+__device__ __forceinline__ void tma_load_im2col(void* smem_dst, const CUtensorMap* map, uint64_t* bar, int c, int w, int h, int n,
+                                                int off_w, int off_h) {
+  asm volatile(
+      "cp.async.bulk.tensor.4d.shared::cluster.global.im2col.mbarrier::complete_tx::bytes "
+      "[%0], [%1, {%3, %4, %5, %6}], [%2], {%7, %8};" ::"r"(smem_u32(smem_dst)),
+      "l"(map), "r"(smem_u32(bar)), "r"(c), "r"(w), "r"(h), "r"(n), "h"(static_cast<uint16_t>(off_w)),
+      "h"(static_cast<uint16_t>(off_h))
       : "memory");
 }
 
diff --git a/clipbert_b200/csrc/gemm.cu b/clipbert_b200/csrc/gemm.cu
--- a/clipbert_b200/csrc/gemm.cu
+++ b/clipbert_b200/csrc/gemm.cu
@@ -38,6 +38,7 @@
   uint64_t seed;
   const uint64_t* seed_off;
   int mn3d;
+  int im2col;
   long long* dbg;
 };
 
@@ -231,6 +232,19 @@
 struct TileInfo {
   int m0, n0;
 };
+
+struct Pix {
+  int x, y, img;
+};
+__device__ __forceinline__ Pix decode_pixel(int q, int H, int W) {
+  Pix p;
+  const int hw = H * W;
+  p.img = q / hw;
+  const int r = q - p.img * hw;
+  p.y = r / W;
+  p.x = r - p.y * W;
+  return p;
+}
 
 template <int BN>
 __device__ __forceinline__ TileInfo decode_tile(int tile, int tiles_m, int tiles_n) {
@@ -423,14 +437,21 @@
           if (++s == STAGES) { s = 0; ph ^= 1; }
         }
         mbar_expect_tx(bar, in_bytes);
+        const Pix q = epi.im2col ? decode_pixel(t.m0, epi.H, epi.W) : Pix{0, 0, 0};
         if (has_res) {
 #pragma unroll
-          for (int j = 0; j < BN / 64; ++j) tma_load_2d(dst + j * IN_BOX_BYTES, &tmR, bar, t.n0 + j * 64, t.m0);
+          for (int j = 0; j < BN / 64; ++j) {
+            if (epi.im2col) tma_load_im2col(dst + j * IN_BOX_BYTES, &tmR, bar, t.n0 + j * 64, q.x, q.y, q.img, 1, 1);
+            else tma_load_2d(dst + j * IN_BOX_BYTES, &tmR, bar, t.n0 + j * 64, t.m0);
+          }
           dst += IN_TILE_BYTES;
         }
         if (has_aux) {
 #pragma unroll
-          for (int j = 0; j < BN / 64; ++j) tma_load_2d(dst + j * IN_BOX_BYTES, &tmX, bar, t.n0 + j * 64, t.m0);
+          for (int j = 0; j < BN / 64; ++j) {
+            if (epi.im2col) tma_load_im2col(dst + j * IN_BOX_BYTES, &tmX, bar, t.n0 + j * 64, q.x, q.y, q.img, 1, 1);
+            else tma_load_2d(dst + j * IN_BOX_BYTES, &tmX, bar, t.n0 + j * 64, t.m0);
+          }
         }
       };
       int pend = -1;
@@ -438,6 +459,7 @@
         const TileInfo t = decode_tile<BN>(tile, tiles_m, tiles_n);
         const bool inputs_first = tile < unit + N_IN * n_units;
         if (in_bytes && N_IN && inputs_first) load_inputs(tile);
+        const Pix q = epi.im2col ? decode_pixel(t.m0, epi.H, epi.W) : Pix{0, 0, 0};
         for (int i = 0; i < n_iters; i += KCH) {
           const int nch = min(KCH, n_iters - i);
           mbar_wait(&empty_bar[s], ph ^ 1);
@@ -447,10 +469,14 @@
           for (int ch = 0; ch < nch; ++ch) {
             uint8_t* sa = smem + s * stage_bytes + ch * Cfg::STAGE_BYTES;
             uint8_t* sb = sa + Cfg::A_BYTES;
-            int shift = 0;
-            if (ntaps == 9) shift = tap_sign * ((tp / 3 - 1) * tap_w + (tp % 3 - 1));
-            else if (ntaps > 1) shift = tap_sign * tp * tap_w;
-            tma_load_2d(sa, &tmA, &full_bar[s], kc * BK, t.m0 + shift);
+            if (epi.im2col) {
+              tma_load_im2col(sa, &tmA, &full_bar[s], kc * BK, q.x, q.y, q.img, 1 + tap_sign * (tp % 3 - 1), 1 + tap_sign * (tp / 3 - 1));
+            } else {
+              int shift = 0;
+              if (ntaps == 9) shift = tap_sign * ((tp / 3 - 1) * tap_w + (tp % 3 - 1));
+              else if (ntaps > 1) shift = tap_sign * tp * tap_w;
+              tma_load_2d(sa, &tmA, &full_bar[s], kc * BK, t.m0 + shift);
+            }
             if (MODE == 0) {
               tma_load_2d(sb, &tmB, &full_bar[s], tp * K + kc * BK, t.n0);
             } else if (epi.mn3d) {
@@ -755,7 +781,9 @@
   const int tiles_m = ceil_div(d.m, BM), tiles_n = ceil_div(d.n, BN);
   const int total = tiles_m * tiles_n;
   const int kiters = ceil_div(d.k, BK) * d.ntaps;
-  bool ok = get_tmap_2d(&ta, d.a, d.k, d.a_rows, d.a_ld, BK, BM);
+  const bool im2col = d.tap_mode == CB_TAPS_INTERIOR;
+  const uint64_t wp = d.map_w + 2, hp = d.map_h + 2, nimg = im2col ? d.a_rows / (wp * hp) : 0;
+  bool ok = im2col ? get_tmap_im2col(&ta, d.a, d.k, d.a_ld, wp, hp, nimg, BM) : get_tmap_2d(&ta, d.a, d.k, d.a_rows, d.a_ld, BK, BM);
   if (MODE == 0) {
     ok = ok && get_tmap_2d(&tb, d.b, static_cast<uint64_t>(d.k) * d.ntaps, d.b_rows, d.b_ld, BK, BN);
   } else {
@@ -765,10 +793,13 @@
   }
   tr = ta;
   tx = ta;
-  if (d.residual) ok = ok && get_tmap_2d(&tr, d.residual, d.n, d.m, d.res_ld, 64, BM);
-  if (d.aux) ok = ok && get_tmap_2d(&tx, d.aux, d.n, d.m, d.aux_ld, 64, BM);
+  if (d.residual)
+    ok = ok && (im2col ? get_tmap_im2col(&tr, d.residual, d.n, d.res_ld, wp, hp, nimg, BM) : get_tmap_2d(&tr, d.residual, d.n, d.m, d.res_ld, 64, BM));
+  if (d.aux)
+    ok = ok && (im2col ? get_tmap_im2col(&tx, d.aux, d.n, d.aux_ld, wp, hp, nimg, BM) : get_tmap_2d(&tx, d.aux, d.n, d.m, d.aux_ld, 64, BM));
   if (!ok) return CB_ERR_CUDA;
   epi.mn3d = mn3d ? 1 : 0;
+  epi.im2col = im2col ? 1 : 0;
   const int units = sm_count();
   const int grid = total < units ? total : units;
   const int in_bytes = epi_in_bytes(d, BN);
@@ -841,6 +872,7 @@
   int iters_per_split, tiles_m, tiles_n;
   int tile_begin;
   int mn3d;
+  int im2col, H, W;
 };
 struct WgradGroup {
   int nprob, total_tiles;
@@ -910,6 +942,7 @@
         const int n0 = t.n0 * BN;
         int shift = 0;
         if (P.ntaps == 9) shift = P.tap_sign * ((t.tap / 3 - 1) * P.tap_w + (t.tap % 3 - 1));
+        const int ox = 1 + P.tap_sign * (t.tap % 3 - 1), oy = 1 + P.tap_sign * (t.tap / 3 - 1);
         for (int i = 0; i < t.n_iters; i += KCH) {
           const int nch = min(KCH, t.n_iters - i);
           mbar_wait(&empty_bar[s], ph ^ 1);
@@ -919,7 +952,13 @@
             uint8_t* sa = smem + s * stage_bytes + ch * Cfg::STAGE_BYTES;
             uint8_t* sb = sa + Cfg::A_BYTES;
             const int p = kit * BK;
-            if (P.mn3d) {
+            if (P.im2col) {
+              const Pix q = decode_pixel(p, P.H, P.W);
+#pragma unroll
+              for (int j = 0; j < BM / 64; ++j) tma_load_im2col(sa + j * (BK * 128), &P.tmA, &full_bar[s], t.m0 + j * 64, q.x, q.y, q.img, 1, 1);
+#pragma unroll
+              for (int j = 0; j < BN / 64; ++j) tma_load_im2col(sb + j * (BK * 128), &P.tmB, &full_bar[s], n0 + j * 64, q.x, q.y, q.img, ox, oy);
+            } else if (P.mn3d) {
               tma_load_3d(sa, &P.tmA, &full_bar[s], 0, p, t.m0 >> 6);
               tma_load_3d(sb, &P.tmB, &full_bar[s], 0, p + shift, n0 >> 6);
             } else {
@@ -977,11 +1016,21 @@
   for (int i = 0; i < n; ++i) {
     const cb_gemm_desc& d = descs[i];
     WgradProblem& P = g.p[i];
-    const bool mn3d = g_mn3d && d.m % 64 == 0 && d.n % 64 == 0 && get_tmap_3d_mn(&P.tmA, d.a, d.m, d.a_rows, d.a_ld, BK, BM / 64) &&
-                      get_tmap_3d_mn(&P.tmB, d.b, d.n, d.b_rows, d.b_ld, BK, BN / 64);
-    if (!mn3d && !(get_tmap_2d(&P.tmA, d.a, d.m, d.a_rows, d.a_ld, 64, BK) && get_tmap_2d(&P.tmB, d.b, d.n, d.b_rows, d.b_ld, 64, BK)))
-      return CB_ERR_CUDA;
-    P.mn3d = mn3d ? 1 : 0;
+    P.im2col = d.tap_mode == CB_TAPS_INTERIOR;
+    P.H = d.map_h;
+    P.W = d.map_w;
+    if (P.im2col) {
+      const uint64_t wp = d.map_w + 2, hp = d.map_h + 2, nimg = d.a_rows / (wp * hp);
+      if (!(get_tmap_im2col(&P.tmA, d.a, d.m, d.a_ld, wp, hp, nimg, BK) && get_tmap_im2col(&P.tmB, d.b, d.n, d.b_ld, wp, hp, nimg, BK)))
+        return CB_ERR_CUDA;
+      P.mn3d = 0;
+    } else {
+      const bool mn3d = g_mn3d && d.m % 64 == 0 && d.n % 64 == 0 && get_tmap_3d_mn(&P.tmA, d.a, d.m, d.a_rows, d.a_ld, BK, BM / 64) &&
+                        get_tmap_3d_mn(&P.tmB, d.b, d.n, d.b_rows, d.b_ld, BK, BN / 64);
+      if (!mn3d && !(get_tmap_2d(&P.tmA, d.a, d.m, d.a_rows, d.a_ld, 64, BK) && get_tmap_2d(&P.tmB, d.b, d.n, d.b_rows, d.b_ld, 64, BK)))
+        return CB_ERR_CUDA;
+      P.mn3d = mn3d ? 1 : 0;
+    }
     P.out = static_cast<float*>(d.out);
     P.scale = d.scale;
     P.out_ld = d.out_ld;
@@ -1049,15 +1098,55 @@
 static int64_t wgrad_ws_bytes(const cb_gemm_desc& d, int splits) {
   return splits > 1 ? static_cast<int64_t>(splits) * d.m * d.ntaps * d.n * 4 : 0;
 }
+static cb_gemm_desc interior_view(const cb_gemm_desc& d);
 static int64_t group_ws_bytes(const cb_gemm_desc* descs, int n) {
-  const GroupPlan gp = group_plan(descs, n, sm_count_device());
+  cb_gemm_desc es[WG_MAX_PROBLEMS];
+  for (int i = 0; i < n && i < WG_MAX_PROBLEMS; ++i) es[i] = interior_view(descs[i]);
+  const GroupPlan gp = n <= WG_MAX_PROBLEMS ? group_plan(es, n, sm_count_device()) : GroupPlan{false, 64, 1};
   int64_t bytes = 0;
   for (int i = 0; i < n; ++i) {
-    const int64_t b = gp.groupable ? wgrad_ws_bytes(descs[i], real_splits(ceil_div(descs[i].k, BK), gp.split))
-                                   : wgrad_ws_bytes(descs[i], choose_config(descs[i], sm_count_device()).splits);
+    const cb_gemm_desc e = interior_view(descs[i]);
+    const int64_t b = gp.groupable ? wgrad_ws_bytes(e, real_splits(ceil_div(e.k, BK), gp.split))
+                                   : wgrad_ws_bytes(e, choose_config(e, sm_count_device()).splits);
     bytes = gp.groupable ? bytes + b : std::max(bytes, b);
   }
   return bytes;
+}
+
+static int check_taps_desc(const cb_gemm_desc& d, const char* who) {
+  CB_REQUIRE(d.tap_mode == CB_TAPS_ALL || d.tap_mode == CB_TAPS_INTERIOR, "%s: bad tap_mode %d", who, d.tap_mode);
+  if (d.tap_mode == CB_TAPS_ALL) return CB_OK;
+  CB_REQUIRE(d.ntaps == 9 && (d.tap_sign == 1 || d.tap_sign == -1), "%s: CB_TAPS_INTERIOR needs ntaps = 9 and tap_sign = +-1", who);
+  CB_REQUIRE(d.map_h > 0 && d.map_w > 0 && d.map_h < 65534 && d.map_w < 65534 && d.tap_w == d.map_w + 2,
+             "%s: CB_TAPS_INTERIOR needs map_h / map_w and tap_w = map_w + 2 (got %d, %d, %d)", who, d.map_h, d.map_w, d.tap_w);
+  const int64_t phw = static_cast<int64_t>(d.map_h + 2) * (d.map_w + 2);
+  CB_REQUIRE(d.a_rows > 0 && d.a_rows % phw == 0, "%s: CB_TAPS_INTERIOR: a_rows %lld is not a whole number of %d x %d zero-bordered images",
+             who, static_cast<long long>(d.a_rows), d.map_h + 2, d.map_w + 2);
+  if (d.mode == CB_GEMM_WGRAD) {
+    CB_REQUIRE(d.k == d.a_rows && d.b_rows == d.a_rows, "%s: CB_TAPS_INTERIOR: k, a_rows and b_rows must be the same padded pixel count", who);
+    CB_REQUIRE(d.m % 64 == 0 && d.n % 64 == 0, "%s: CB_TAPS_INTERIOR: m, n must be multiples of 64 (got %d, %d)", who, d.m, d.n);
+    CB_REQUIRE(d.a_ld % 8 == 0 && d.b_ld % 8 == 0 && d.a_ld >= d.m && d.b_ld >= d.n, "%s: CB_TAPS_INTERIOR: bad a_ld / b_ld", who);
+  } else {
+    CB_REQUIRE(d.m == d.a_rows, "%s: CB_TAPS_INTERIOR: m must be a_rows (got %d, %lld)", who, d.m, static_cast<long long>(d.a_rows));
+    CB_REQUIRE(d.rowmap == CB_ROWMAP_UNPAD, "%s: CB_TAPS_INTERIOR needs CB_ROWMAP_UNPAD (only interior rows are written)", who);
+    CB_REQUIRE(d.k % 64 == 0 && d.a_ld % 8 == 0 && d.a_ld >= d.k, "%s: CB_TAPS_INTERIOR: k must be a multiple of 64 (got %d), a_ld >= k", who, d.k);
+    CB_REQUIRE((!d.residual && !d.aux) || d.n % 64 == 0, "%s: CB_TAPS_INTERIOR with residual / aux: n must be a multiple of 64 (got %d)", who,
+               d.n);
+  }
+  return CB_OK;
+}
+
+static cb_gemm_desc interior_view(const cb_gemm_desc& d) {
+  cb_gemm_desc e = d;
+  if (d.tap_mode != CB_TAPS_INTERIOR || d.map_h <= 0 || d.map_w <= 0) return e;
+  const int64_t pixels = d.a_rows / (static_cast<int64_t>(d.map_h + 2) * (d.map_w + 2)) * d.map_h * d.map_w;
+  if (d.mode == CB_GEMM_WGRAD) {
+    e.k = static_cast<int32_t>(pixels);
+  } else {
+    e.m = static_cast<int32_t>(pixels);
+    e.rowmap = CB_ROWMAP_NONE;
+  }
+  return e;
 }
 
 static int check_wgrad_desc(const cb_gemm_desc& d, const char* who) {
@@ -1069,7 +1158,7 @@
   CB_REQUIRE((reinterpret_cast<uintptr_t>(d.a) & 15) == 0 && (reinterpret_cast<uintptr_t>(d.b) & 15) == 0,
              "%s: a and b must be 16-byte aligned (TMA)", who);
   CB_REQUIRE(d.ntaps == 1 || d.ntaps == 9, "%s: ntaps must be 1 or 9 (got %d)", who, d.ntaps);
-  return CB_OK;
+  return check_taps_desc(d, who);
 }
 
 static int launch_wgrad(const cb_gemm_desc* descs, int n, int bn, int splits, cudaStream_t stream, const char* what) {
@@ -1129,6 +1218,7 @@
   epi.seed = d.dropout_seed;
   epi.dbg = g_gemm_timeline;
   epi.mn3d = 0;
+  epi.im2col = 0;
   {
     const DropCfg dc = make_drop(d.dropout_p, d.dropout_seed);
     epi.drop_thresh = dc.thresh;
@@ -1153,19 +1243,26 @@
     CB_REQUIRE(!(d.out2 && d.out_fp32), "cb_gemm(TN): out2 requires a bf16 primary output");
     CB_REQUIRE(d.rowmap == CB_ROWMAP_NONE || (d.map_h > 0 && d.map_w > 0), "cb_gemm: rowmap needs map_h/map_w");
     CB_REQUIRE(d.ntaps == 1 || d.tap_w > 2, "cb_gemm: tap modes need tap_w (padded row pitch in pixels)");
+    {
+      const int rc = check_taps_desc(d, "cb_gemm(TN)");
+      if (rc != CB_OK) return rc;
+    }
     CB_REQUIRE(d.block_n == 0 || d.block_n == 64 || d.block_n == 128 || d.block_n == 256, "cb_gemm: block_n must be 0, 64, 128 or 256 (got %d)",
                d.block_n);
-    const LaunchCfg lc = choose_config(d, sm_count());
+    const cb_gemm_desc e = interior_view(d);
+    epi.rowmap = e.rowmap;
+    const LaunchCfg lc = choose_config(e, sm_count());
     switch (lc.bn) {
-      case 64: return nn ? launch_gemm<64, 2>(d, epi, stream) : launch_gemm<64, 0>(d, epi, stream);
-      case 128: return nn ? launch_gemm<128, 2>(d, epi, stream) : launch_gemm<128, 0>(d, epi, stream);
+      case 64: return nn ? launch_gemm<64, 2>(e, epi, stream) : launch_gemm<64, 0>(e, epi, stream);
+      case 128: return nn ? launch_gemm<128, 2>(e, epi, stream) : launch_gemm<128, 0>(e, epi, stream);
       default: CB_REQUIRE(false, "cb_gemm: no tile width for block_n %d", d.block_n);
     }
   } else {
     const int rc = check_wgrad_desc(d, "cb_gemm(WGRAD)");
     if (rc != CB_OK) return rc;
-    const LaunchCfg lc = choose_config(d, plan_sm_count());
-    return launch_wgrad(&d, 1, lc.bn, lc.splits, stream, "cb_gemm");
+    const cb_gemm_desc e = interior_view(d);
+    const LaunchCfg lc = choose_config(e, plan_sm_count());
+    return launch_wgrad(&e, 1, lc.bn, lc.splits, stream, "cb_gemm");
   }
   return CB_ERR_INVALID;
 }
@@ -1179,7 +1276,9 @@
     const int rc = check_wgrad_desc(descs[i], who);
     if (rc != CB_OK) return rc;
   }
-  const GroupPlan gp = group_plan(descs, n, plan_sm_count());
+  cb_gemm_desc es[WG_MAX_PROBLEMS];
+  for (int i = 0; i < n && i < WG_MAX_PROBLEMS; ++i) es[i] = interior_view(descs[i]);
+  const GroupPlan gp = group_plan(es, n, plan_sm_count());
   if (!gp.groupable) {
     for (int i = 0; i < n; ++i) {
       cb_gemm_desc d = descs[i];
@@ -1190,13 +1289,14 @@
     }
     return CB_OK;
   }
-  return launch_wgrad(descs, n, gp.bn, gp.split, static_cast<cudaStream_t>(stream_v), "cb_gemm_wgrad_group");
+  return launch_wgrad(es, n, gp.bn, gp.split, static_cast<cudaStream_t>(stream_v), "cb_gemm_wgrad_group");
 }
 
 extern "C" int64_t cb_gemm_workspace_bytes(const cb_gemm_desc* d) {
   using namespace cb;
   if (d == nullptr || d->mode != CB_GEMM_WGRAD || d->m <= 0 || d->n <= 0 || d->k <= 0) return 0;
-  return wgrad_ws_bytes(*d, choose_config(*d, sm_count_device()).splits);
+  const cb_gemm_desc e = interior_view(*d);
+  return wgrad_ws_bytes(e, choose_config(e, sm_count_device()).splits);
 }
 
 extern "C" int64_t cb_gemm_wgrad_group_workspace_bytes(const cb_gemm_desc* descs, int n) {
diff --git a/clipbert_b200/csrc/host_util.h b/clipbert_b200/csrc/host_util.h
--- a/clipbert_b200/csrc/host_util.h
+++ b/clipbert_b200/csrc/host_util.h
@@ -59,6 +59,9 @@
 
 bool get_tmap_3d_mn(CUtensorMap* out, const void* base, uint64_t cols, uint64_t rows, uint64_t ld, uint32_t box_rows, uint32_t nblk);
 
+bool get_tmap_im2col(CUtensorMap* out, const void* base, uint64_t channels, uint64_t ld, uint64_t wp, uint64_t hp, uint64_t n,
+                     uint32_t pixels);
+
 #define CB_REQUIRE(cond, ...)        \
   do {                               \
     if (!(cond)) {                   \
diff --git a/clipbert_b200/grid_feat.py b/clipbert_b200/grid_feat.py
--- a/clipbert_b200/grid_feat.py
+++ b/clipbert_b200/grid_feat.py
@@ -304,7 +304,7 @@
         out = torch.empty(n * h * w, m.cout, dtype=torch.bfloat16, device=x_pad.device)
         ops.gemm(mode=ops.CB_GEMM_TN, m=p, n=m.cout, k=m.cin, a=x_pad, a_rows=p, a_ld=m.cin, b=m._w, b_rows=m.cout,
                  b_ld=9 * m.cin, ntaps=9, tap_w=w + 2, tap_sign=1, shift=m._shift, act=act, out=out, out_ld=m.cout,
-                 rowmap=ops.ROWMAP_UNPAD, map_h=h, map_w=w)
+                 rowmap=ops.ROWMAP_UNPAD, map_h=h, map_w=w, tap_mode=ops.TAPS_INTERIOR)
         return out
 
     def _forward_impl(self, images, need_backward):
@@ -407,12 +407,15 @@
                 self._capture["stash"] = stash
         return grid, stash
 
-    def _wgrad_kw(self, m, dy, x, p, ntaps=1, tap_w=0):
-        return dict(mode=ops.CB_GEMM_WGRAD, m=m.cout, n=m.cin, k=p, a=dy, a_rows=p, a_ld=m.cout, b=x, b_rows=p, b_ld=m.cin,
-                    ntaps=ntaps, tap_w=tap_w, tap_sign=1, scale=m._scale, out=m._gw, out_ld=ntaps * m.cin, out_fp32=1)
-
-    def _wgrad(self, m, dy, x, p, ntaps=1, tap_w=0):
-        ops.gemm(**self._wgrad_kw(m, dy, x, p, ntaps, tap_w))
+    def _wgrad_kw(self, m, dy, x, p, ntaps=1, tap_w=0, map_h=0):
+        kw = dict(mode=ops.CB_GEMM_WGRAD, m=m.cout, n=m.cin, k=p, a=dy, a_rows=p, a_ld=m.cout, b=x, b_rows=p, b_ld=m.cin,
+                  ntaps=ntaps, tap_w=tap_w, tap_sign=1, scale=m._scale, out=m._gw, out_ld=ntaps * m.cin, out_fp32=1)
+        if ntaps == 9:
+            kw.update(tap_mode=ops.TAPS_INTERIOR, map_h=map_h, map_w=tap_w - 2)
+        return kw
+
+    def _wgrad(self, m, dy, x, p, ntaps=1, tap_w=0, map_h=0):
+        ops.gemm(**self._wgrad_kw(m, dy, x, p, ntaps, tap_w, map_h))
 
     def _dgrad1x1(self, m, dy, rows, residual=None, aux=None, rowmap=ops.ROWMAP_NONE, hw=None, out=None):
         if out is None:
@@ -433,7 +436,7 @@
         out = torch.empty(n * h * w, m.cin, dtype=torch.bfloat16, device=dy_pad.device)
         ops.gemm(mode=ops.CB_GEMM_NN, m=p, n=m.cin, k=m.cout, a=dy_pad, a_rows=p, a_ld=m.cout, b=m._w, b_rows=m.cout,
                  b_ld=9 * m.cin, ntaps=9, tap_w=w + 2, tap_sign=-1, aux=aux_pad, aux_ld=m.cin, aux_mode=ops.AUX_RELU_MASK,
-                 out=out, out_ld=m.cin, rowmap=ops.ROWMAP_UNPAD, map_h=h, map_w=w)
+                 out=out, out_ld=m.cin, rowmap=ops.ROWMAP_UNPAD, map_h=h, map_w=w, tap_mode=ops.TAPS_INTERIOR)
         return out
 
     def _backward_impl(self, stash, dgrid, last=True):
@@ -451,7 +454,7 @@
         res5_pad = stash["res5_pad"]
         recycle.append(res5_pad)
         if ge.weight.requires_grad:
-            sq.run(lambda: self._wgrad(ge, dg_pad, res5_pad, p, ntaps=9, tap_w=w + 2), dg_pad, res5_pad)
+            sq.run(lambda: self._wgrad(ge, dg_pad, res5_pad, p, ntaps=9, tap_w=w + 2, map_h=h), dg_pad, res5_pad)
         blocks = stash["blocks"]
         if blocks:
             g = self._dgrad3x3(ge, dg_pad, n, h, w, res5_pad)
@@ -464,7 +467,7 @@
             db_pad = self._pad_get(pp, blk.mid, dev)
             recycle += [db_pad, st["a_pad"]]
             self._dgrad1x1(blk.conv3, g, rows, aux=st["b"], rowmap=ops.ROWMAP_PAD, hw=(hh, ww), out=db_pad)
-            wg.append(self._wgrad_kw(blk.conv2, db_pad, st["a_pad"], pp, ntaps=9, tap_w=ww + 2))
+            wg.append(self._wgrad_kw(blk.conv2, db_pad, st["a_pad"], pp, ntaps=9, tap_w=ww + 2, map_h=hh))
             da = self._dgrad3x3(blk.conv2, db_pad, n, hh, ww, st["a_pad"])
             wg.append(self._wgrad_kw(blk.conv1, da, st["xs"], rows))
             if blk.has_shortcut:
diff --git a/clipbert_b200/ops.py b/clipbert_b200/ops.py
--- a/clipbert_b200/ops.py
+++ b/clipbert_b200/ops.py
@@ -7,6 +7,7 @@
                    AUX_RELU_MASK, AUX_TANH_GRAD, CB_GEMM_TN, CB_GEMM_WGRAD, ROWMAP_NONE, ROWMAP_PAD, ROWMAP_UNPAD)
 
 CB_GEMM_NN = 2
+TAPS_ALL, TAPS_INTERIOR = 0, 1
 _c = ctypes
 _vp, _i, _i64, _f, _u64 = _c.c_void_p, _c.c_int, _c.c_int64, _c.c_float, _c.c_uint64
 
diff --git a/include/clipbert_b200.h b/include/clipbert_b200.h
--- a/include/clipbert_b200.h
+++ b/include/clipbert_b200.h
@@ -73,7 +73,10 @@
   int32_t reserved;
   void* workspace;
   int64_t workspace_bytes;
+  int32_t tap_mode;
 } cb_gemm_desc;
+
+enum { CB_TAPS_ALL = 0, CB_TAPS_INTERIOR = 1 };
 
 int cb_gemm(const cb_gemm_desc* desc, void* stream);
 int64_t cb_gemm_workspace_bytes(const cb_gemm_desc* desc);
```

Result: faster. 4225, median of 6 (+6.0%).
